# ilovepose/fast-human-pose-estimation.pytorch

Measured on AMD Instinct MI355X. Metric: images/sec FPD train step (4-stack HG student, 8-stack teacher) 256x256, higher is better.
Workload: dtype bf16; 1 GPU; configs[1]: hourglass student S=4 F=128 + teacher S=8 F=256, 256x256, batch 32/GPU, fused FPD step incl. Adam, teacher forward one batch ahead on a 2nd stream; global_batch=32, parallelism=dp1, backend=mfma, launch=one native plan call per phase, kernels launched eagerly on 3 streams, ranks=1, finite=True

## Files before the change

### fast-human-pose-estimation.pytorch_amd/csrc/api.hip

```cpp
#include <cstdarg>
#include <cstdio>
#include <cstdlib>
#include <cstring>
#include <string>
#include <vector>

#include "conv_dispatch.h"

int g_fpd_backend = FPD_BACKEND_MFMA;
static thread_local char g_err[512] = "";

static FILE* g_launch_log_file = nullptr;
static bool launch_log_open() {
    const char* path = getenv("FPD_LAUNCH_LOG");
    if (path == nullptr || path[0] == 0) return false;
    g_launch_log_file = fopen(path, "w");
    if (g_launch_log_file == nullptr) fprintf(stderr, "[fpd_amd] FPD_LAUNCH_LOG: cannot open %s\n", path);
    return g_launch_log_file != nullptr;
}
bool g_fpd_launch_log = launch_log_open();
static thread_local char g_op_tag[256] = "-";
void fpd_log_launch(const char* kernel, const dim3& grid, const dim3& block) {
    if (g_launch_log_file == nullptr) return;
    fprintf(g_launch_log_file, "%s\t%u\t%u\t%s\n", kernel, grid.x * grid.y * grid.z, block.x * block.y * block.z, g_op_tag);
    fflush(g_launch_log_file);
}

int fpd_fail(int code, const char* fmt, ...) {
    va_list ap;
    va_start(ap, fmt);
    vsnprintf(g_err, sizeof(g_err), fmt, ap);
    va_end(ap);
    return code;
}

static int check_launch() {
    hipError_t e = hipGetLastError();
    if (e != hipSuccess) return fpd_fail(-100 - (int)e, "kernel launch failed: %s", hipGetErrorString(e));
    return 0;
}

static int validate_conv_dims(int N, int H, int W, int C, int K, int R, int S, int stride, int pad, int P, int Q) {
    FPD_REQUIRE(N > 0 && H > 0 && W > 0 && C > 0 && K > 0 && R > 0 && S > 0 && stride > 0 && pad >= 0,
                "conv: non-positive dimension");
    FPD_REQUIRE(P == (H + 2 * pad - R) / stride + 1 && Q == (W + 2 * pad - S) / stride + 1,
                "conv: output %dx%d inconsistent with input %dx%d k=%dx%d stride=%d pad=%d", P, Q, H, W, R, S, stride, pad);
    FPD_REQUIRE((int64_t)N * H * W * C < (1ll << 31) && (int64_t)N * P * Q * K < (1ll << 31), "conv: tensor too large for 32-bit indexing");
    return 0;
}

int fpd_bneck_blocks_option(int value);
int fpd_head_blocks_option(int value);

extern "C" {

const char* fpd_last_error(void) { return g_err; }
int fpd_abi_version(void) { return FPD_ABI_VERSION; }
int64_t fpd_stats_words(int32_t channels) { return FPD_STATS_WORDS(channels); }
int fpd_set_backend(int32_t backend) {
    const int prev = g_fpd_backend;
    if (backend == FPD_BACKEND_MFMA || backend == FPD_BACKEND_NAIVE || backend == FPD_BACKEND_MFMA_GENERIC) g_fpd_backend = backend;
    return prev;
}

static int g_wgrad_tile_only = 0;

int fpd_set_option(const char* name, int32_t value) {
    FPD_REQUIRE(name, "set_option: null name");
    if (!strcmp(name, "conv_pp")) return fpd_conv_pp_option(0, value);
    if (!strcmp(name, "conv_pp_blocks")) return fpd_conv_pp_option(1, value);
    if (!strcmp(name, "conv_c1")) return fpd_conv_c1_option(0, value);
    if (!strcmp(name, "conv_c1_blocks")) return fpd_conv_c1_option(1, value);
    if (!strcmp(name, "conv_c1_launches")) return fpd_conv_c1_option(2, value);
    if (!strcmp(name, "conv_skip")) return fpd_conv_c1_option(3, value);
    if (!strcmp(name, "stem_act")) return fpd_stem_s2d_option(0, value);
    if (!strcmp(name, "ew_merge")) return fpd_ew_merge_option(value < 0 ? 0 : value);
    if (!strcmp(name, "ew_merge_blocks")) return fpd_ew_merge_blocks_option(value);
    if (!strcmp(name, "conv_c3")) return fpd_conv_c3_option(0, value);
    if (!strcmp(name, "conv_c3_blocks")) return fpd_conv_c3_option(1, value);
    if (!strcmp(name, "conv_c3_launches")) return fpd_conv_c3_option(2, value);
    if (!strcmp(name, "bneck_blocks")) return fpd_bneck_blocks_option(value);
    if (!strcmp(name, "head_blocks")) return fpd_head_blocks_option(value);
    if (!strcmp(name, "wgrad_tile_only")) { g_wgrad_tile_only = value; return 0; }
    return fpd_fail(-2, "set_option: unknown option '%s'", name);
}

int fpd_abi_sizeof(const char* n) {
#define SZ(T) if (!strcmp(n, #T)) return (int)sizeof(T)
    SZ(fpd_bn_t); SZ(fpd_conv_t); SZ(fpd_wgrad_t); SZ(fpd_stem_t); SZ(fpd_ew_t); SZ(fpd_loss_t); SZ(fpd_adam_t);
    SZ(fpd_wprep_entry_t); SZ(fpd_bnupd_entry_t); SZ(fpd_memset_t); SZ(fpd_table_t); SZ(fpd_wreduce_entry_t); SZ(fpd_bneck_t); SZ(fpd_conv_pair_t); SZ(fpd_bneck_pair_t); SZ(fpd_ew_pair_t); SZ(fpd_pck_t); SZ(fpd_head_t); SZ(fpd_affsum_t); SZ(fpd_layout_t);
    SZ(fpd_conv_f8_t); SZ(fpd_wquant_entry_t); SZ(fpd_flipmerge_t); SZ(fpd_finalpreds_t); SZ(fpd_targets_t); SZ(fpd_warp_src_t); SZ(fpd_warp_t);
    SZ(fpd_loss_ohkm_t); SZ(fpd_sgd_t); SZ(fpd_ew_merge_t);
    SZ(fpd_aug_img_t); SZ(fpd_aug_db_t); SZ(fpd_aug_crop_t); SZ(fpd_augment_t); SZ(fpd_warp_aug_t); SZ(fpd_targets_w_t);
    SZ(fpd_oks_nms_t); SZ(fpd_coco_match_t); SZ(fpd_coco_accum_t);
#undef SZ
    return -1;
}

static int validate_conv(const fpd_conv_t* a) {
    FPD_REQUIRE(a && a->x && a->w && a->y, "conv: null pointer");
    int rc = validate_conv_dims(a->N, a->H, a->W, a->C, a->K, a->R, a->S, a->stride, a->pad, a->P, a->Q);
    if (rc) return rc;
    FPD_REQUIRE(a->dtype == FPD_F32 || a->dtype == FPD_BF16, "conv: bad dtype %d", a->dtype);
    FPD_REQUIRE(a->bn.mode == FPD_BN_NONE || (a->bn.gamma && a->bn.beta), "conv: BN prologue without gamma/beta");
    FPD_REQUIRE(a->bn.mode != FPD_BN_TRAIN || a->bn.stats, "conv: train-mode BN without statistics");
    FPD_REQUIRE(a->bn.mode != FPD_BN_EVAL || (a->bn.running_mean && a->bn.running_var), "conv: eval-mode BN without running stats");
    FPD_REQUIRE(a->epi == FPD_EPI_PLAIN || (a->epi_x && a->epi_stats && a->epi_bn.mode == FPD_BN_TRAIN && a->epi_bn.stats),
                "conv: BNRELU_BWD epilogue needs epi_x, epi_stats and a train-mode epi_bn");
    FPD_REQUIRE(a->x2 == nullptr || (a->w2 != nullptr && a->C2 > 0), "conv: a second source (x2) needs w2 and C2");
    FPD_REQUIRE(a->x2 == nullptr || a->residual == nullptr, "conv: a second source (x2) and a residual exclude each other");
    return 0;
}

constexpr unsigned ON_MFMA = 1u << FPD_BACKEND_MFMA, ON_GENERIC = ON_MFMA | 1u << FPD_BACKEND_MFMA_GENERIC, ON_ANY = ON_GENERIC | 1u << FPD_BACKEND_NAIVE;
struct ConvBackend {
    const char* name;
    unsigned backends;
    int (*route)(const fpd_conv_t& a, const fpd_conv_t* b, ConvAsk ask, ConvRoute& r);
    int (*launch)(const fpd_conv_t& a, const fpd_conv_t* b, hipStream_t st);
};
static const ConvBackend g_conv_backends[] = {
    {"conv_c1", ON_MFMA, fpd_conv_c1_route, fpd_conv_c1_launch},
    {"conv_c3", ON_MFMA, fpd_conv_c3_route, fpd_conv_c3_launch},
    {"conv_pp", ON_MFMA, fpd_conv_pp_route, fpd_conv_pp_launch},
    {"conv_tile", ON_MFMA, fpd_conv_tile_route, fpd_conv_tile_launch},
    {"conv_mfma", ON_GENERIC, nullptr, [](const fpd_conv_t& a, const fpd_conv_t*, hipStream_t st) { return fpd_conv_mfma_launch(a, st); }},
    {"conv_smallc", ON_GENERIC, nullptr, [](const fpd_conv_t& a, const fpd_conv_t*, hipStream_t st) { return fpd_conv_smallc_launch(a, st); }},
    {"conv_naive", ON_ANY, nullptr, [](const fpd_conv_t& a, const fpd_conv_t*, hipStream_t st) { return fpd_conv_naive_launch(a, st); }},
};
static bool eligible(unsigned backends) { return (backends >> g_fpd_backend & 1u) != 0; }

static const ConvBackend* route_conv(const fpd_conv_t& a, const fpd_conv_t* b, ConvAsk ask, ConvRoute& r) {
    r = ConvRoute{false, 0, 0, false};
    for (const ConvBackend& e : g_conv_backends) {
        if (!eligible(e.backends)) continue;
        if (e.route == nullptr ? b == nullptr : e.route(a, b, ask, r) == 0) return &e;
    }
    return nullptr;
}

static int launch_conv(const fpd_conv_t& a, const fpd_conv_t* b, hipStream_t st) {
    ConvRoute r;
    const ConvBackend* e = route_conv(a, b, fpd_conv_ask(a, b), r);
    if (e == nullptr) {
        const int rc = launch_conv(a, nullptr, st);
        return rc ? rc : launch_conv(*b, nullptr, st);
    }
    FPD_REQUIRE(!(a.wg_partial != nullptr && r.slabs_a == 0) && !(b != nullptr && b->wg_partial != nullptr && r.slabs_b == 0),
                "conv: the launch asks for a fused weight gradient (wg_partial), which its route (%s) does not offer; %s() reports 0 for it",
                e->name, b ? "fpd_conv_pair_fused_wgrad_partials" : "fpd_conv_fused_wgrad_partials");
    FPD_REQUIRE(r.folds || (a.fold_x == nullptr && (b == nullptr || b->fold_x == nullptr)),
                "conv: the launch asks for a folded BN-backward apply (fold_x), which its route (%s) does not offer; %s() reports 0 for it",
                e->name, b ? "fpd_conv_pair_fold_supported" : "fpd_conv_fold_supported");
    FPD_REQUIRE(r.skips || (a.x2 == nullptr && (b == nullptr || b->x2 == nullptr)),
                "conv: the launch carries a second 1x1 source (x2), which its route (%s) does not offer; fpd_conv_skip_supported() reports 0 for it", e->name);
    int rc = e->launch(a, b, st);
    for (++e; rc == 1 && e != std::end(g_conv_backends); ++e)
        if (e->route == nullptr && eligible(e->backends)) rc = e->launch(a, b, st);
    return rc;
}

int fpd_conv_forward(const fpd_conv_t* a, fpd_stream_t stream) {
    int rc = validate_conv(a);
    if (rc) return rc;
    rc = launch_conv(*a, nullptr, (hipStream_t)stream);
    return rc ? rc : check_launch();
}

int fpd_conv_fold_supported(const fpd_conv_t* a) {
    ConvRoute r;
    if (!a || validate_conv(a) != 0) return 0;
    route_conv(*a, nullptr, ConvAsk{true, a->wg_partial != nullptr, a->x2 != nullptr}, r);
    return r.folds ? 1 : 0;
}
int fpd_conv_pair_fold_supported(const fpd_conv_pair_t* p) {
    ConvRoute r;
    if (!p || validate_conv(&p->a) != 0 || validate_conv(&p->b) != 0) return 0;
    if (route_conv(p->a, &p->b, ConvAsk{true, fpd_conv_ask(p->a, &p->b).wg, fpd_conv_ask(p->a, &p->b).skip}, r) != nullptr) return r.folds ? 1 : 0;
    return (fpd_conv_fold_supported(&p->a) && fpd_conv_fold_supported(&p->b)) ? 1 : 0;
}

int fpd_conv_skip_supported(const fpd_conv_t* a) {
    ConvRoute r;
    if (!a || validate_conv(a) != 0) return 0;
    route_conv(*a, nullptr, ConvAsk{a->fold_x != nullptr, a->wg_partial != nullptr, true}, r);
    return r.skips ? 1 : 0;
}

int fpd_conv_fused_wgrad_partials(const fpd_conv_t* a) {
    ConvRoute r;
    if (!a || validate_conv(a) != 0) return 0;
    route_conv(*a, nullptr, ConvAsk{a->fold_x != nullptr, true, a->x2 != nullptr}, r);
    return r.slabs_a;
}
int fpd_conv_pair_fused_wgrad_partials(const fpd_conv_pair_t* p, int32_t* n_a, int32_t* n_b) {
    FPD_REQUIRE(p && n_a && n_b, "conv_pair_fused_wgrad_partials: null pointer");
    *n_a = *n_b = 0;
    if (validate_conv(&p->a) != 0 || validate_conv(&p->b) != 0) return 0;
    ConvRoute r;
    route_conv(p->a, &p->b, ConvAsk{fpd_conv_ask(p->a, &p->b).fold, true, fpd_conv_ask(p->a, &p->b).skip}, r);
    *n_a = r.slabs_a; *n_b = r.slabs_b;
    return 0;
}

int fpd_conv_f8_in_domain(const fpd_conv_t* c) { return (c && fpd_conv_f8_domain(*c)) ? 1 : 0; }

int fpd_conv_forward_f8(const fpd_conv_f8_t* a, fpd_stream_t stream) {
    FPD_REQUIRE(a, "conv_f8: null pointer");
    int rc = validate_conv(&a->c);
    if (rc) return rc;
    FPD_REQUIRE(a->w8 && a->w8_scale, "conv_f8: null fp8 weights / scales");
    FPD_REQUIRE(((uintptr_t)a->w8 & 15) == 0, "conv_f8: w8 must be 16-byte aligned");
    rc = 1;
    if (g_fpd_backend == FPD_BACKEND_MFMA) rc = fpd_conv_tile_f8_launch(a->c, a->w8, a->w8_scale, (hipStream_t)stream);
    if (rc == 1) rc = launch_conv(a->c, nullptr, (hipStream_t)stream);
    return rc ? rc : check_launch();
}

int fpd_weight_quant_f8(const fpd_wquant_entry_t* t, int32_t n, fpd_stream_t stream) {
    FPD_REQUIRE(n == 0 || t != nullptr, "weight_quant_f8: null table");
    int rc = fpd_weight_quant_f8_launch(t, n, (hipStream_t)stream);
    return rc ? rc : check_launch();
}

int fpd_conv_forward_pair(const fpd_conv_pair_t* p, fpd_stream_t stream) {
    FPD_REQUIRE(p, "conv_pair: null pointer");
    int rc = validate_conv(&p->a);
    if (rc) return rc;
    rc = validate_conv(&p->b);
    if (rc) return rc;
    FPD_REQUIRE(p->a.x2 == nullptr && p->b.x2 == nullptr, "conv_pair: a pair launch takes no second source (x2)");
    rc = launch_conv(p->a, &p->b, (hipStream_t)stream);
    return rc ? rc : check_launch();
}

static int validate_bneck_bns(const fpd_bneck_t* a) {
    const fpd_bn_t* bns[3] = {&a->bn1, &a->bn2, &a->bn3};
    for (int i = 0; i < 3; ++i)
        FPD_REQUIRE(bns[i]->mode == FPD_BN_EVAL && bns[i]->relu && bns[i]->gamma && bns[i]->beta && bns[i]->running_mean &&
                    bns[i]->running_var, "bottleneck: bn%d must be an eval-mode BN+ReLU with running statistics", i + 1);
    return 0;
}

int fpd_bottleneck_fold(const fpd_bneck_t* a, fpd_stream_t stream) {
    FPD_REQUIRE(a && a->folded, "bottleneck_fold: null pointer");
    int rc = validate_bneck_bns(a);
    if (rc) return rc;
    rc = fpd_bneck_fold_launch(*a, const_cast<float*>(a->folded), (hipStream_t)stream);
    if (rc == 1) return fpd_fail(-3, "bottleneck_fold: C=%d P=%d is outside the fused kernel's domain", a->C, a->P);
    return rc ? rc : check_launch();
}

int fpd_bottleneck_forward_pair(const fpd_bneck_pair_t* p, fpd_stream_t stream) {
    FPD_REQUIRE(p, "bottleneck_pair: null pointer");
    const fpd_bneck_t* ab[2] = {&p->a, &p->b};
    for (const fpd_bneck_t* a : ab) {
        FPD_REQUIRE(a->x && a->y && a->w1 && a->w2 && a->w3 && a->x != a->y, "bottleneck_pair: null pointer or y aliases x");
        FPD_REQUIRE((int64_t)a->N * a->H * a->W * a->C < ((int64_t)1 << 31), "bottleneck_pair: tensor too large for 32-bit indexing");
        int rc = validate_bneck_bns(a);
        if (rc) return rc;
    }
    int rc = fpd_bneck_fused_pair_launch(p->a, p->b, (hipStream_t)stream);
    if (rc == 1) {
        rc = fpd_bottleneck_forward(&p->a, stream);
        return rc ? rc : fpd_bottleneck_forward(&p->b, stream);
    }
    return rc ? rc : check_launch();
}

int fpd_bottleneck_forward(const fpd_bneck_t* a, fpd_stream_t stream) {
    FPD_REQUIRE(a && a->x && a->y && a->w1 && a->w2 && a->w3, "bottleneck: null pointer");
    FPD_REQUIRE(a->x != a->y, "bottleneck: y must not alias x");
    FPD_REQUIRE(a->N > 0 && a->H > 0 && a->W > 0 && a->C > 0 && a->P > 0, "bottleneck: bad dims");
    FPD_REQUIRE((int64_t)a->N * a->H * a->W * a->C < ((int64_t)1 << 31), "bottleneck: tensor too large for 32-bit indexing");
    int rc = validate_bneck_bns(a);
    if (rc) return rc;
    rc = fpd_bneck_fused_launch(*a, (hipStream_t)stream);
    if (rc == 1)
        return fpd_fail(-3, "bottleneck: shape N=%d H=%d W=%d C=%d P=%d dtype=%d is outside the fused kernel's domain",
                        a->N, a->H, a->W, a->C, a->P, a->dtype);
    return rc ? rc : check_launch();
}

struct WgradBackend {
    unsigned backends;
    int (*partials)(const fpd_wgrad_t& a);
    int (*launch)(const fpd_wgrad_t& a, hipStream_t st);
};
static const WgradBackend g_wgrad_backends[] = {
    {ON_MFMA, fpd_wgrad_tile_partials, fpd_wgrad_tile_launch},
    {ON_GENERIC, fpd_wgrad_mfma_partials, fpd_wgrad_mfma_launch},
    {ON_GENERIC, fpd_wgrad_smallc_partials, fpd_wgrad_smallc_launch},
    {ON_ANY, fpd_wgrad_naive_partials, fpd_wgrad_naive_launch},
};

int fpd_conv_wgrad(const fpd_wgrad_t* a, fpd_stream_t stream) {
    FPD_REQUIRE(a && a->x && a->dy && a->dw, "wgrad: null pointer");
    int rc = validate_conv_dims(a->N, a->H, a->W, a->C, a->K, a->R, a->S, a->stride, a->pad, a->P, a->Q);
    if (rc) return rc;
    FPD_REQUIRE(a->dtype == FPD_F32 || a->dtype == FPD_BF16, "wgrad: bad dtype %d", a->dtype);
    FPD_REQUIRE(a->partial == nullptr || a->partial_stride >= (int64_t)a->K * a->R * a->S * a->C + a->K,
                "wgrad: partial_stride %lld smaller than weight + bias", (long long)a->partial_stride);
    rc = 1;
    for (const WgradBackend& e : g_wgrad_backends) {
        FPD_REQUIRE(!(g_wgrad_tile_only && &e != g_wgrad_backends), "wgrad: option wgrad_tile_only is set and the halo-tile kernel declines N=%d H=%d W=%d C=%d K=%d R=%d", a->N, a->H, a->W, a->C, a->K, a->R);
        if (eligible(e.backends)) rc = e.launch(*a, (hipStream_t)stream);
        if (rc != 1) break;
    }
    return rc ? rc : check_launch();
}

int fpd_wgrad_num_partials(const fpd_wgrad_t* a) {
    int n = 0;
    for (const WgradBackend& e : g_wgrad_backends)
        if (a && n == 0 && eligible(e.backends)) n = e.partials(*a);
    return n;
}

struct StemBackend {
    unsigned backends;
    bool (*takes_act)(const fpd_stem_t& a);
    int (*forward)(const fpd_stem_t& a, hipStream_t st);
    int (*wgrad_partials)(const fpd_stem_t& a);
    int (*wgrad)(const fpd_stem_t& a, hipStream_t st);
};
static const StemBackend g_stem_backends[] = {
    {ON_MFMA, fpd_stem_forward_s2d_takes_act, fpd_stem_forward_s2d_launch, fpd_stem_wgrad_s2d_partials, fpd_stem_wgrad_s2d_launch},
    {ON_MFMA, nullptr, fpd_stem_forward_mfma_launch, fpd_stem_wgrad_mfma_partials, fpd_stem_wgrad_mfma_launch},
    {ON_ANY, nullptr, fpd_stem_forward_launch, fpd_stem_wgrad_partials, fpd_stem_wgrad_launch},
};

int fpd_stem_wgrad_num_partials(const fpd_stem_t* a) {
    int n = 0;
    for (const StemBackend& e : g_stem_backends)
        if (a && n == 0 && eligible(e.backends)) n = e.wgrad_partials(*a);
    return n;
}

int fpd_wgrad_reduce(const fpd_wreduce_entry_t* t, int32_t n, int64_t max_elems, fpd_stream_t stream) {
    int rc = fpd_wreduce_launch(t, n, max_elems, (hipStream_t)stream);
    return rc ? rc : check_launch();
}

int fpd_stem_act_supported(const fpd_stem_t* a) {
    if (!a || a->act.mode != FPD_BN_EVAL || !a->act.gamma || !a->act.beta || !a->act.running_mean || !a->act.running_var || a->out_stats != nullptr) return 0;
    for (const StemBackend& e : g_stem_backends)
        if (eligible(e.backends)) return (e.takes_act != nullptr && e.takes_act(*a)) ? 1 : 0;
    return 0;
}

int fpd_stem_forward(const fpd_stem_t* a, fpd_stream_t stream) {
    FPD_REQUIRE(a && a->x && a->w && a->bias && a->y, "stem: null pointer");
    FPD_REQUIRE(a->P == (a->H + 6 - 7) / 2 + 1 && a->Q == (a->W + 6 - 7) / 2 + 1, "stem: bad output size");
    FPD_REQUIRE(a->act.mode == FPD_BN_NONE || fpd_stem_act_supported(a) == 1,
                "stem: the launch asks for BN + ReLU in its epilogue (act), which is not offered for it; fpd_stem_act_supported() reports 0");
    int rc = 1;
    for (const StemBackend& e : g_stem_backends)
        if (rc == 1 && eligible(e.backends)) rc = e.forward(*a, (hipStream_t)stream);
    return rc ? rc : check_launch();
}

int fpd_stem_wgrad(const fpd_stem_t* a, fpd_stream_t stream) {
    FPD_REQUIRE(a && a->x && a->dy && a->dw, "stem wgrad: null pointer");
    FPD_REQUIRE(a->partial == nullptr || a->partial_stride >= (int64_t)a->K * 148, "stem wgrad: partial_stride %lld smaller than weight + bias",
                (long long)a->partial_stride);
    int rc = 1;
    for (const StemBackend& e : g_stem_backends)
        if (rc == 1 && eligible(e.backends)) rc = e.wgrad(*a, (hipStream_t)stream);
    return rc ? rc : check_launch();
}

int fpd_affsum(const fpd_affsum_t* a, fpd_stream_t stream) {
    FPD_REQUIRE(a && a->y, "affsum: null pointer");
    FPD_REQUIRE(a->nterms >= 1 && a->nterms <= FPD_AFFSUM_MAX, "affsum: %d terms (1..%d supported)", a->nterms, FPD_AFFSUM_MAX);
    FPD_REQUIRE(a->dtype == FPD_F32 || a->dtype == FPD_BF16, "affsum: bad dtype %d", a->dtype);
    for (int j = 0; j < a->nterms; ++j) {
        const int up = a->t[j].up;
        FPD_REQUIRE(a->t[j].x, "affsum: term %d has no input", j);
        FPD_REQUIRE((up == 1 || up == 2 || up == 4 || up == 8) && a->H % up == 0 && a->W % up == 0,
                    "affsum: term %d: up-sampling factor %d does not divide %dx%d", j, up, a->H, a->W);
        const fpd_bn_t& bn = a->t[j].bn;
        FPD_REQUIRE(bn.mode == FPD_BN_NONE || (bn.gamma && bn.beta), "affsum: term %d: BN without gamma/beta", j);
        FPD_REQUIRE(bn.mode != FPD_BN_TRAIN || bn.stats, "affsum: term %d: train-mode BN without statistics", j);
        FPD_REQUIRE(bn.mode != FPD_BN_EVAL || (bn.running_mean && bn.running_var), "affsum: term %d: eval-mode BN without running stats", j);
    }
    int rc = fpd_affsum_launch(*a, (hipStream_t)stream);
    return rc ? rc : check_launch();
}

int fpd_elementwise(const fpd_ew_t* a, fpd_stream_t stream) {
    FPD_REQUIRE(a && (a->y || a->op == FPD_EW_BNRELU_BWD_R), "elementwise: null pointer");
    int rc = fpd_elementwise_launch(*a, (hipStream_t)stream);
    return rc ? rc : check_launch();
}

int fpd_ew_merge_supported(const fpd_ew_merge_t* a) { return (a && fpd_ew_merge_why_not(*a) == nullptr) ? 1 : 0; }
int fpd_ew_merge(const fpd_ew_merge_t* a, fpd_stream_t stream) {
    FPD_REQUIRE(a, "ew_merge: null pointer");
    int rc = fpd_ew_merge_launch(*a, (hipStream_t)stream);
    return rc ? rc : check_launch();
}

static int validate_head(const fpd_head_t* a) {
    FPD_REQUIRE(a && a->y0 && a->score && a->w_fc && a->w_score, "head: null pointer");
    FPD_REQUIRE(a->next == nullptr || (a->x && a->w_fc2 && a->w_score2 && a->next != a->x && a->next != a->y0),
                "head: next needs x, w_fc2, w_score2 and must not alias an input");
    FPD_REQUIRE(a->N > 0 && a->H > 0 && a->W > 0 && (int64_t)a->N * a->H * a->W * a->C < ((int64_t)1 << 31), "head: bad dims");
    FPD_REQUIRE(a->bn.mode == FPD_BN_EVAL && a->bn.relu && a->bn.gamma && a->bn.beta && a->bn.running_mean && a->bn.running_var,
                "head: bn must be an eval-mode BN+ReLU with running statistics");
    return 0;
}
int fpd_head_forward(const fpd_head_t* a, fpd_stream_t stream) {
    int rc = validate_head(a);
    if (rc) return rc;
    rc = fpd_head_fused_launch(*a, (hipStream_t)stream);
    if (rc == 1) return fpd_fail(-3, "head: C=%d J=%d dtype=%d is outside the fused kernel's domain", a->C, a->J, a->dtype);
    return rc ? rc : check_launch();
}
int fpd_head_fold(const fpd_head_t* a, fpd_stream_t stream) {
    FPD_REQUIRE(a && a->folded, "head_fold: null pointer");
    FPD_REQUIRE(a->bn.mode == FPD_BN_EVAL && a->bn.gamma && a->bn.beta && a->bn.running_mean && a->bn.running_var, "head_fold: bn");
    int rc = fpd_head_fold_launch(*a, const_cast<float*>(a->folded), (hipStream_t)stream);
    if (rc == 1) return fpd_fail(-3, "head_fold: C=%d is outside the fused kernel's domain", a->C);
    return rc ? rc : check_launch();
}

int fpd_pck(const fpd_pck_t* a, fpd_stream_t stream) {
    FPD_REQUIRE(a && a->out && a->target && a->counts && a->log && a->cursor, "pck: null pointer");
    FPD_REQUIRE(a->B > 0 && a->J > 0 && a->H > 0 && a->W > 0 && a->log_slots > 0, "pck: bad dims");
    FPD_REQUIRE(a->dtype == FPD_F32 || a->dtype == FPD_BF16, "pck: bad dtype %d", a->dtype);
    int rc = fpd_pck_launch(*a, (hipStream_t)stream);
    return rc ? rc : check_launch();
}

int fpd_flip_w(const float* x, float* y, int64_t rows, int32_t W, fpd_stream_t stream) {
// ... 156 lines not shown

int fpd_sgd(const fpd_sgd_t* a, fpd_stream_t stream) {
    FPD_REQUIRE(a && a->param && a->grad, "sgd: null pointer");
    FPD_REQUIRE(a->n >= 0, "sgd: n = %lld is negative", (long long)a->n);
    FPD_REQUIRE(a->momentum >= 0.f, "sgd: invalid momentum value %g", (double)a->momentum);
    FPD_REQUIRE(a->weight_decay >= 0.f, "sgd: invalid weight_decay value %g", (double)a->weight_decay);
    FPD_REQUIRE(a->momentum == 0.f || a->buf, "sgd: momentum %g needs a momentum buffer (buf is null)", (double)a->momentum);
    FPD_REQUIRE(!a->nesterov || a->momentum != 0.f, "sgd: nesterov momentum requires a momentum (and zero dampening)");
    int rc = fpd_sgd_launch(*a, (hipStream_t)stream);
    return rc ? rc : check_launch();
}

int fpd_weight_prep(const fpd_wprep_entry_t* t, int32_t n, int64_t max_elems, int32_t dtype, fpd_stream_t stream) {
    int rc = fpd_weight_prep_launch(t, n, max_elems, dtype, (hipStream_t)stream);
    return rc ? rc : check_launch();
}
int fpd_bn_update_running(const fpd_bnupd_entry_t* t, int32_t n, fpd_stream_t stream) {
    int rc = fpd_bn_update_running_launch(t, n, (hipStream_t)stream);
    return rc ? rc : check_launch();
}
int fpd_cast(const void* src, void* dst, int64_t n, int32_t sd, int32_t dd, fpd_stream_t stream) {
    int rc = fpd_cast_launch(src, dst, n, sd, dd, (hipStream_t)stream);
    return rc ? rc : check_launch();
}
int fpd_nchw_to_nhwc(const float* src, void* dst, int32_t N, int32_t C, int32_t H, int32_t W, int32_t dtype, fpd_stream_t stream) {
    int rc = fpd_nchw_to_nhwc_launch(src, dst, N, C, H, W, dtype, (hipStream_t)stream);
    return rc ? rc : check_launch();
}
int fpd_nhwc_to_nchw(const void* src, float* dst, int32_t N, int32_t C, int32_t H, int32_t W, int32_t dtype, fpd_stream_t stream) {
    int rc = fpd_nhwc_to_nchw_launch(src, dst, N, C, H, W, dtype, (hipStream_t)stream);
    return rc ? rc : check_launch();
}

struct fpd_op {
    int32_t type;
    union {
        fpd_affsum_t affsum; fpd_layout_t layout; fpd_conv_f8_t conv8; fpd_conv_t conv; fpd_conv_pair_t pair; fpd_bneck_t bneck; fpd_bneck_pair_t bpair; fpd_ew_pair_t epair; fpd_pck_t pck; fpd_head_t head; fpd_wgrad_t wgrad; fpd_stem_t stem; fpd_ew_t ew; fpd_loss_t loss; fpd_loss_ohkm_t lossk; fpd_adam_t adam; fpd_sgd_t sgd; fpd_ew_merge_t ewm;
        fpd_memset_t mset; fpd_table_t table;
    } u;
};
struct fpd_sched {
    int32_t lane = 0;
    bool record = false;
    hipEvent_t done = nullptr;
    std::vector<int32_t> waits;
};
struct fpd_plan {
    std::vector<fpd_op> ops;
    std::vector<fpd_sched> sched;
    std::vector<hipGraphExec_t> graphs;
    std::vector<hipGraph_t> graph_defs;
    hipStream_t lanes[FPD_MAX_LANES] = {};
    hipEvent_t lane_done[FPD_MAX_LANES] = {};
    hipEvent_t fork = nullptr;
};

fpd_plan* fpd_plan_create(void) { return new fpd_plan(); }
void fpd_plan_destroy(fpd_plan* p) {
    if (!p) return;
    for (auto g : p->graphs) (void)hipGraphExecDestroy(g);
    for (auto g : p->graph_defs) (void)hipGraphDestroy(g);
    for (auto& s : p->sched) if (s.done) (void)hipEventDestroy(s.done);
    for (int l = 0; l < FPD_MAX_LANES; ++l) {
        if (p->lanes[l]) (void)hipStreamDestroy(p->lanes[l]);
        if (p->lane_done[l]) (void)hipEventDestroy(p->lane_done[l]);
    }
    if (p->fork) (void)hipEventDestroy(p->fork);
    delete p;
}
int fpd_plan_size(const fpd_plan* p) { return p ? (int)p->ops.size() : -1; }

int fpd_plan_add(fpd_plan* p, int32_t op, const void* args, int64_t bytes) {
    FPD_REQUIRE(p && args, "plan_add: null");
    fpd_op o;
    memset(&o, 0, sizeof(o));
    o.type = op;
    size_t want = 0;
    switch (op) {
        case FPD_OP_CONV: want = sizeof(fpd_conv_t); break;
        case FPD_OP_CONV_F8: want = sizeof(fpd_conv_f8_t); break;
        case FPD_OP_WGRAD: want = sizeof(fpd_wgrad_t); break;
        case FPD_OP_CONV_PAIR: want = sizeof(fpd_conv_pair_t); break;
        case FPD_OP_BNECK_PAIR: want = sizeof(fpd_bneck_pair_t); break;
        case FPD_OP_EW_PAIR: want = sizeof(fpd_ew_pair_t); break;
        case FPD_OP_PCK: want = sizeof(fpd_pck_t); break;
        case FPD_OP_HEAD: case FPD_OP_HEAD_FOLD: want = sizeof(fpd_head_t); break;
        case FPD_OP_BNECK: case FPD_OP_BNECK_FOLD: want = sizeof(fpd_bneck_t); break;
        case FPD_OP_STEM_FWD: case FPD_OP_STEM_WGRAD: want = sizeof(fpd_stem_t); break;
        case FPD_OP_EW: want = sizeof(fpd_ew_t); break;
        case FPD_OP_EW_MERGE: want = sizeof(fpd_ew_merge_t); break;
        case FPD_OP_LOSS: want = sizeof(fpd_loss_t); break;
        case FPD_OP_LOSS_OHKM: want = sizeof(fpd_loss_ohkm_t); break;
        case FPD_OP_ADAM: want = sizeof(fpd_adam_t); break;
        case FPD_OP_SGD: want = sizeof(fpd_sgd_t); break;
        case FPD_OP_MEMSET: case FPD_OP_NOP: want = sizeof(fpd_memset_t); break;
        case FPD_OP_AFFSUM: want = sizeof(fpd_affsum_t); break;
        case FPD_OP_NCHW2NHWC: want = sizeof(fpd_layout_t); break;
        case FPD_OP_WPREP: case FPD_OP_BNUPD: case FPD_OP_WREDUCE: case FPD_OP_WQUANT: want = sizeof(fpd_table_t); break;
        default: return fpd_fail(-2, "plan_add: unknown op %d", op);
    }
    FPD_REQUIRE((size_t)bytes == want, "plan_add: op %d expects %zu bytes of args, got %lld", op, want, (long long)bytes);
    memcpy(&o.u, args, want);
    p->ops.push_back(o);
    p->sched.emplace_back();
    return (int)p->ops.size() - 1;
}

int fpd_plan_set_schedule(fpd_plan* p, int32_t op, int32_t lane, const int32_t* wait_ops, int32_t n_waits) {
    FPD_REQUIRE(p && op >= 0 && op < (int)p->ops.size(), "plan_set_schedule: bad op index %d", op);
    FPD_REQUIRE(lane >= 0 && lane < FPD_MAX_LANES, "plan_set_schedule: lane %d outside [0,%d)", lane, FPD_MAX_LANES);
    FPD_REQUIRE(n_waits >= 0 && (n_waits == 0 || wait_ops != nullptr), "plan_set_schedule: bad wait list");
    for (int i = 0; i < n_waits; ++i)
        FPD_REQUIRE(wait_ops[i] >= 0 && wait_ops[i] < op, "plan_set_schedule: op %d may only wait for earlier ops (got %d)", op, wait_ops[i]);
    fpd_sched& s = p->sched[op];
    s.lane = lane;
    s.waits.assign(wait_ops, wait_ops + n_waits);
    for (int i = 0; i < n_waits; ++i) p->sched[wait_ops[i]].record = true;
    return 0;
}

int fpd_plan_mark_event(fpd_plan* p, int32_t op) {
    FPD_REQUIRE(p && op >= 0 && op < (int)p->ops.size(), "plan_mark_event: bad op index %d", op);
    p->sched[op].record = true;
    return 0;
}

int fpd_plan_wait_op(fpd_plan* p, int32_t op, fpd_stream_t stream) {
    FPD_REQUIRE(p && op >= 0 && op < (int)p->ops.size(), "plan_wait_op: bad op index %d", op);
    FPD_REQUIRE(p->sched[op].record && p->sched[op].done, "plan_wait_op: op %d has no recorded event (mark it, then run its range)", op);
    FPD_CHECK_HIP(hipStreamWaitEvent((hipStream_t)stream, p->sched[op].done, 0));
    return 0;
}

static void conv_tag(char* p, size_t n, const char* what, const fpd_conv_t& c) {
    snprintf(p, n, "%s N=%d H=%d W=%d C=%d K=%d R=%d s=%d %s%s%s%s%s", what, c.N, c.H, c.W, c.C, c.K, c.R, c.stride,
             c.epi == FPD_EPI_BNRELU_BWD ? "dgrad" : "fwd", c.bn.mode == FPD_BN_EVAL ? " evalbn" : "", c.wg_partial ? " +wgrad" : "", c.fold_x ? " +fold" : "",
             c.x2 ? " +skip" : "");
}
static void set_op_tag(int idx, const fpd_op& o) {
    char t[200] = "";
    static const char* ew_names[] = {"bnrelu_fwd", "bnrelu_bwd_r", "bn_bwd_apply", "maxpool_fwd", "maxpool_bwd", "upadd_fwd", "sumpool", "add", "relu_mask", "dilate2"};
    auto ewn = [&](int op) { return (op >= 0 && op < 10) ? ew_names[op] : "ew"; };
    switch (o.type) {
        case FPD_OP_CONV: conv_tag(t, sizeof(t), "conv", o.u.conv); break;
        case FPD_OP_CONV_F8: conv_tag(t, sizeof(t), "conv_f8", o.u.conv8.c); break;
        case FPD_OP_CONV_PAIR: {
            char a[90], b[90];
            conv_tag(a, sizeof(a), "conv2", o.u.pair.a);
            snprintf(b, sizeof(b), " | H=%d W=%d", o.u.pair.b.H, o.u.pair.b.W);
            snprintf(t, sizeof(t), "%s%s", a, b);
            break;
        }
        case FPD_OP_WGRAD: snprintf(t, sizeof(t), "wgrad N=%d H=%d W=%d C=%d K=%d R=%d s=%d", o.u.wgrad.N, o.u.wgrad.H, o.u.wgrad.W, o.u.wgrad.C, o.u.wgrad.K, o.u.wgrad.R, o.u.wgrad.stride); break;
        case FPD_OP_BNECK: snprintf(t, sizeof(t), "bneck N=%d H=%d W=%d C=%d P=%d", o.u.bneck.N, o.u.bneck.H, o.u.bneck.W, o.u.bneck.C, o.u.bneck.P); break;
        case FPD_OP_BNECK_PAIR: snprintf(t, sizeof(t), "bneck2 N=%d H=%d W=%d C=%d P=%d | H=%d W=%d", o.u.bpair.a.N, o.u.bpair.a.H, o.u.bpair.a.W, o.u.bpair.a.C, o.u.bpair.a.P, o.u.bpair.b.H, o.u.bpair.b.W); break;
        case FPD_OP_HEAD: snprintf(t, sizeof(t), "head N=%d H=%d W=%d C=%d J=%d", o.u.head.N, o.u.head.H, o.u.head.W, o.u.head.C, o.u.head.J); break;
        case FPD_OP_EW: snprintf(t, sizeof(t), "ew %s N=%d H=%d W=%d C=%d", ewn(o.u.ew.op), o.u.ew.N, o.u.ew.H, o.u.ew.W, o.u.ew.C); break;
        case FPD_OP_EW_PAIR: snprintf(t, sizeof(t), "ew2 %s N=%d H=%d W=%d C=%d | H=%d W=%d", ewn(o.u.epair.a.op), o.u.epair.a.N, o.u.epair.a.H, o.u.epair.a.W, o.u.epair.a.C, o.u.epair.b.H, o.u.epair.b.W); break;
        case FPD_OP_EW_MERGE: {
            const fpd_ew_merge_t& m = o.u.ewm;
            const bool pb = m.kind == FPD_EWM_MAXPOOL_BWD;
            snprintf(t, sizeof(t), "ewm %s N=%d H=%d W=%d C=%d", pb ? (m.has_full ? "apply2+maxpool_bwd" : "apply+maxpool_bwd") : "apply+sumpool", m.pool.N, m.pool.H, m.pool.W, m.pool.C);
            break;
        }
        case FPD_OP_STEM_FWD: case FPD_OP_STEM_WGRAD: snprintf(t, sizeof(t), "%s N=%d H=%d W=%d K=%d%s", o.type == FPD_OP_STEM_FWD ? "stem_fwd" : "stem_wgrad", o.u.stem.N, o.u.stem.H, o.u.stem.W, o.u.stem.K,
                                                              (o.type == FPD_OP_STEM_FWD && o.u.stem.act.mode != FPD_BN_NONE) ? " +act" : ""); break;
        case FPD_OP_AFFSUM: snprintf(t, sizeof(t), "affsum N=%d H=%d W=%d C=%d terms=%d", o.u.affsum.N, o.u.affsum.H, o.u.affsum.W, o.u.affsum.C, o.u.affsum.nterms); break;
        case FPD_OP_LOSS: snprintf(t, sizeof(t), "loss B=%d J=%d H=%d W=%d S=%d", o.u.loss.B, o.u.loss.J, o.u.loss.H, o.u.loss.W, o.u.loss.S); break;
        case FPD_OP_LOSS_OHKM: snprintf(t, sizeof(t), "loss_ohkm B=%d J=%d H=%d W=%d S=%d k=%d,%d", o.u.lossk.base.B, o.u.lossk.base.J, o.u.lossk.base.H, o.u.lossk.base.W, o.u.lossk.base.S, o.u.lossk.topk_pose, o.u.lossk.topk_kd); break;
        case FPD_OP_ADAM: snprintf(t, sizeof(t), "adam n=%lld", (long long)o.u.adam.n); break;
        case FPD_OP_SGD: snprintf(t, sizeof(t), "sgd n=%lld momentum=%g wd=%g%s", (long long)o.u.sgd.n, (double)o.u.sgd.momentum, (double)o.u.sgd.weight_decay, o.u.sgd.nesterov ? " nesterov" : ""); break;
        case FPD_OP_WREDUCE: snprintf(t, sizeof(t), "wreduce entries=%d", o.u.table.n); break;
        case FPD_OP_WPREP: snprintf(t, sizeof(t), "wprep entries=%d", o.u.table.n); break;
        case FPD_OP_BNUPD: snprintf(t, sizeof(t), "bnupd entries=%d", o.u.table.n); break;
        default: snprintf(t, sizeof(t), "op%d", o.type); break;
    }
    snprintf(g_op_tag, sizeof(g_op_tag), "%d\t%s", idx, t);
}

static int run_op(const fpd_op& o, fpd_stream_t s) {
    switch (o.type) {
        case FPD_OP_CONV: return fpd_conv_forward(&o.u.conv, s);
        case FPD_OP_CONV_F8: return fpd_conv_forward_f8(&o.u.conv8, s);
        case FPD_OP_WQUANT: return fpd_weight_quant_f8((const fpd_wquant_entry_t*)o.u.table.table, o.u.table.n, s);
        case FPD_OP_WGRAD: return fpd_conv_wgrad(&o.u.wgrad, s);
        case FPD_OP_CONV_PAIR: return fpd_conv_forward_pair(&o.u.pair, s);
        case FPD_OP_BNECK_PAIR: return fpd_bottleneck_forward_pair(&o.u.bpair, s);
        case FPD_OP_EW_PAIR: return fpd_elementwise_pair(&o.u.epair, s);
        case FPD_OP_PCK: return fpd_pck(&o.u.pck, s);
        case FPD_OP_HEAD: return fpd_head_forward(&o.u.head, s);
        case FPD_OP_HEAD_FOLD: return fpd_head_fold(&o.u.head, s);
        case FPD_OP_BNECK: return fpd_bottleneck_forward(&o.u.bneck, s);
        case FPD_OP_BNECK_FOLD: return fpd_bottleneck_fold(&o.u.bneck, s);
        case FPD_OP_STEM_FWD: return fpd_stem_forward(&o.u.stem, s);
        case FPD_OP_STEM_WGRAD: return fpd_stem_wgrad(&o.u.stem, s);
        case FPD_OP_EW: return fpd_elementwise(&o.u.ew, s);
        case FPD_OP_EW_MERGE: return fpd_ew_merge(&o.u.ewm, s);
        case FPD_OP_LOSS: return fpd_loss(&o.u.loss, s);
        case FPD_OP_LOSS_OHKM: return fpd_loss_ohkm(&o.u.lossk, s);
        case FPD_OP_ADAM: return fpd_adam(&o.u.adam, s);
        case FPD_OP_SGD: return fpd_sgd(&o.u.sgd, s);
        case FPD_OP_MEMSET: {
            FPD_CHECK_HIP(hipMemsetAsync(o.u.mset.ptr, 0, (size_t)o.u.mset.bytes, (hipStream_t)s));
            return 0;
        }
        case FPD_OP_NOP: return 0;
        case FPD_OP_AFFSUM: return fpd_affsum(&o.u.affsum, s);
        case FPD_OP_NCHW2NHWC:
            return fpd_nchw_to_nhwc(o.u.layout.src, o.u.layout.dst, o.u.layout.N, o.u.layout.C, o.u.layout.H, o.u.layout.W, o.u.layout.dtype, s);
        case FPD_OP_WPREP:
            return fpd_weight_prep((const fpd_wprep_entry_t*)o.u.table.table, o.u.table.n, o.u.table.max_elems, o.u.table.dtype, s);
        case FPD_OP_BNUPD: return fpd_bn_update_running((const fpd_bnupd_entry_t*)o.u.table.table, o.u.table.n, s);
        case FPD_OP_WREDUCE: return fpd_wgrad_reduce((const fpd_wreduce_entry_t*)o.u.table.table, o.u.table.n, o.u.table.max_elems, s);
    }
    return fpd_fail(-2, "run_op: unknown op %d", o.type);
}

static int lane_priority() { return 0; }

static int side_streams() { return FPD_MAX_LANES; }

int fpd_plan_run(fpd_plan* p, int32_t begin, int32_t end, fpd_stream_t stream) {
    FPD_REQUIRE(p && begin >= 0 && end <= (int)p->ops.size() && begin <= end, "plan_run: bad range [%d,%d)", begin, end);
    hipStream_t main_s = (hipStream_t)stream;
    bool multi = false;
    for (int i = begin; i < end; ++i) multi |= p->sched[i].lane != 0;
    bool used[FPD_MAX_LANES] = {};
    if (multi) {
        if (!p->fork) FPD_CHECK_HIP(hipEventCreateWithFlags(&p->fork, hipEventDisableTiming));
        FPD_CHECK_HIP(hipEventRecord(p->fork, main_s));
    }
    int rc = 0;
    for (int i = begin; i < end && rc == 0; ++i) {
        fpd_sched& sc = p->sched[i];
        hipStream_t st = main_s;
        if (sc.lane != 0) {
            const int l = 1 + (sc.lane - 1) % side_streams();
            if (!p->lanes[l]) {
                FPD_CHECK_HIP(hipStreamCreateWithPriority(&p->lanes[l], hipStreamNonBlocking, lane_priority()));
                FPD_CHECK_HIP(hipEventCreateWithFlags(&p->lane_done[l], hipEventDisableTiming));
            }
            st = p->lanes[l];
            if (!used[l]) {
                FPD_CHECK_HIP(hipStreamWaitEvent(st, p->fork, 0));
                used[l] = true;
            }
        }
        for (int32_t w : sc.waits)
            if (w >= begin && w < end) FPD_CHECK_HIP(hipStreamWaitEvent(st, p->sched[w].done, 0));
        if (g_fpd_launch_log) set_op_tag(i, p->ops[i]);
        rc = run_op(p->ops[i], (fpd_stream_t)st);
        if (rc) {
            char tmp[400];
            snprintf(tmp, sizeof(tmp), "%s", g_err);
            rc = fpd_fail(rc, "plan op %d (type %d): %s", i, p->ops[i].type, tmp);
            break;
        }
        if (sc.record) {
            if (!sc.done) FPD_CHECK_HIP(hipEventCreateWithFlags(&sc.done, hipEventDisableTiming));
            FPD_CHECK_HIP(hipEventRecord(sc.done, st));
        }
    }
    for (int l = 1; l < FPD_MAX_LANES; ++l)
        if (used[l]) {
            FPD_CHECK_HIP(hipEventRecord(p->lane_done[l], p->lanes[l]));
            FPD_CHECK_HIP(hipStreamWaitEvent(main_s, p->lane_done[l], 0));
        }
    return rc;
}

int fpd_plan_run_op(fpd_plan* p, int32_t op, fpd_stream_t stream) {
    FPD_REQUIRE(p && op >= 0 && op < (int)p->ops.size(), "plan_run_op: bad op index %d", op);
    if (g_fpd_launch_log) set_op_tag(op, p->ops[op]);
    return run_op(p->ops[op], stream);
}

int fpd_plan_capture(fpd_plan* p, int32_t begin, int32_t end, fpd_stream_t stream) {
    FPD_REQUIRE(p, "plan_capture: null");
    FPD_REQUIRE(!g_fpd_launch_log, "plan_capture: FPD_LAUNCH_LOG is set -- the launch log keys a kernel trace 1:1 and cannot follow hipGraph replays; unset one of them");
    hipStream_t st = (hipStream_t)stream;
    FPD_CHECK_HIP(hipStreamBeginCapture(st, hipStreamCaptureModeThreadLocal));
    int rc = fpd_plan_run(p, begin, end, stream);
    hipGraph_t g = nullptr;
    hipError_t e = hipStreamEndCapture(st, &g);
    if (rc) { if (g) (void)hipGraphDestroy(g); return rc; }
    if (e != hipSuccess) return fpd_fail(-100 - (int)e, "hipStreamEndCapture: %s", hipGetErrorString(e));
    hipGraphExec_t ge = nullptr;
    FPD_CHECK_HIP(hipGraphInstantiate(&ge, g, nullptr, nullptr, 0));
    p->graph_defs.push_back(g);
    p->graphs.push_back(ge);
    return (int)p->graphs.size() - 1;
}

int fpd_plan_replay(fpd_plan* p, int32_t gid, fpd_stream_t stream) {
    FPD_REQUIRE(p && gid >= 0 && gid < (int)p->graphs.size(), "plan_replay: bad graph id %d", gid);
    FPD_CHECK_HIP(hipGraphLaunch(p->graphs[gid], (hipStream_t)stream));
    return 0;
}

void* fpd_event_create(void) {
    hipEvent_t e = nullptr;
    if (hipEventCreate(&e) != hipSuccess) return nullptr;
    return (void*)e;
}
int fpd_event_record(void* ev, fpd_stream_t stream) {
    FPD_CHECK_HIP(hipEventRecord((hipEvent_t)ev, (hipStream_t)stream));
    return 0;
// ... 11 lines not shown
```

### fast-human-pose-estimation.pytorch_amd/csrc/bneck_fused.hip

```cpp
#include <algorithm>
#include <atomic>
#include <cstdlib>
#include <type_traits>

#include "common.h"

namespace {

typedef unsigned int u32x4 __attribute__((ext_vector_type(4)));

#ifdef FPD_BNECK_TIMING
#define STAMP(i) do { if (tid == 0 && bid_in == 0) stamps[i] = clock64(); } while (0)
#else
#define STAMP(i) do { } while (0)
#endif

template <int P>
__device__ __forceinline__ void bneck_fold_tables(const fpd_bneck_t& a, float* out, int tid, int nthreads) {
    constexpr int C = 2 * P;
    for (int c = tid; c < C; c += nthreads) {
        float sc, sh;
        bn_coef_eval(a.bn1, c, sc, sh);
        out[c] = sc;
        out[C + c] = sh;
        out[2 * C + 4 * P + c] = a.b3 ? a.b3[c] : 0.f;
    }
    for (int c = tid; c < 2 * P; c += nthreads) {
        const bool second = c >= P;
        const int cc = second ? c - P : c;
        float sc, sh;
        bn_coef_eval(second ? a.bn3 : a.bn2, cc, sc, sh);
        const float* bias = second ? a.b2 : a.b1;
        out[2 * C + (second ? 2 * P : 0) + cc] = sc;
        out[2 * C + (second ? 2 * P : 0) + P + cc] = fmaf(sc, bias ? bias[cc] : 0.f, sh);
    }
}

template <int P>
__global__ void bneck_fold_kernel(const fpd_bneck_t a, float* out) { bneck_fold_tables<P>(a, out, threadIdx.x, blockDim.x); }

template <int P, bool DMA>
__device__ __forceinline__ void bneck_eval_body(const fpd_bneck_t& a, const int logW, const int swz, const int bid_in,
                                                const int nblk, const int ntiles) {
    constexpr int C = 2 * P;
    constexpr int LDW = DMA ? P : P + 8;
    constexpr int LDX = 64 + 8;
    constexpr int LD2 = P + 8;
    constexpr int TNH = P / 64;
    constexpr int CW = 32 * TNH;
    constexpr int NSTEP = 9 + 2;
    constexpr int VPR2 = P / 8;
    constexpr int WV = P * VPR2 / 512;
    constexpr int W1V = P * 8 / 512;
    constexpr int NCH = C / 64;
    constexpr int ASTG = (128 + P) * LDX;
    extern __shared__ __attribute__((aligned(16))) unsigned char smem[];

    const int tid = threadIdx.x, lane = tid & 63, wave = tid >> 6;
#ifdef FPD_BNECK_TIMING
    long long stamps[8];
    long long astamp[10];
    int acnt = 0;
#define ASTAMP() do { if (tid == 0 && bid_in == 0 && acnt < 10) astamp[acnt++] = clock64(); } while (0)
#else
#define ASTAMP() do { } while (0)
#endif
    STAMP(0);
    const int q = wave & 3, hC = wave >> 2;
    const int koff = 8 * (lane >> 5);
    const int H = a.H, W = a.W;
    const int M = a.N * H * W, GR = a.N * H;
    const int nrows = 128 >> logW, hrows = nrows + 2, WP = W + 2;
    const int rrows = 2 * nrows;
    const bool whole = (128 % (H * W)) == 0;
    const int irows = whole ? hrows : rrows;
    const int zero_px = irows * WP;
    int m0 = 0, g0 = 0;
    int vrow0 = 0;

    float* s_sc1 = reinterpret_cast<float*>(smem);
    float* s_sh1 = s_sc1 + C;
    float* s_sc2 = s_sh1 + C;
    float* s_sh2 = s_sc2 + P;
    float* s_sc3 = s_sh2 + P;
    float* s_sh3 = s_sc3 + P;
    float* s_b3 = s_sh3 + P;
    bf16_t* sA2 = reinterpret_cast<bf16_t*>(s_b3 + C);
    bf16_t* sR2 = sA2 + (zero_px + 3) * LD2;
    const bf16_t* __restrict__ x = reinterpret_cast<const bf16_t*>(a.x);
    const bf16_t* __restrict__ w1 = reinterpret_cast<const bf16_t*>(a.w1);
    const bf16_t* __restrict__ w2 = reinterpret_cast<const bf16_t*>(a.w2);
    const bf16_t* __restrict__ w3 = reinterpret_cast<const bf16_t*>(a.w3);

    int hp0 = whole ? W : 0;
    int npass = whole ? 1 : ((hrows * W + 127) >> 7);
    const int xpx = tid >> 3, xcv = (tid & 7) * 8;
    int xo[2];
    bool xok[2];
    auto pass_addr = [&](int p) __attribute__((always_inline)) {
#pragma unroll
        for (int i = 0; i < 2; ++i) {
            const int hp = hp0 + 128 * p + xpx + 64 * i;
            const int hr = hp >> logW, j = hp & (W - 1);
            const int g = g0 - 1 + hr;
            xok[i] = hr < hrows && (unsigned)g < (unsigned)GR;
            xo[i] = xok[i] ? (g * W + j) * C + xcv : 0;
        }
    };
    int w1o[W1V], w1l[W1V];
#pragma unroll
    for (int i = 0; i < W1V; ++i) {
        const int v = tid + i * 512;
        w1o[i] = (v >> 3) * C + (v & 7) * 8;
        w1l[i] = 128 * LDX + (v >> 3) * LDX + (v & 7) * 8;
    }
    const int xl = xpx * LDX + xcv;

    u32x4 rx[NCH][2], rw[NCH][W1V];
    auto a_load = [&](auto kcc) __attribute__((always_inline)) {
        constexpr int kc = decltype(kcc)::value;
        static_for<2>([&](auto ic) {
            constexpr int i = decltype(ic)::value;
            const u32x4 z = {0u, 0u, 0u, 0u};
            rx[kc][i] = z;
            if (xok[i]) rx[kc][i] = *reinterpret_cast<const u32x4*>(x + (xo[i] + kc * 64));
        });
        static_for<W1V>([&](auto ic) {
            constexpr int i = decltype(ic)::value;
            rw[kc][i] = *reinterpret_cast<const u32x4*>(w1 + (w1o[i] + kc * 64));
        });
    };
    constexpr int NSL = 2 + W1V;
    auto a_store_slice = [&](auto kcc, auto slc) __attribute__((always_inline)) {
        constexpr int kc = decltype(kcc)::value, sl = decltype(slc)::value;
        bf16_t* dst = sR2 + (kc & 1) * ASTG;
        if constexpr (sl < 2) {
            f32x4 sc[2], sh[2];
            sc[0] = *reinterpret_cast<const f32x4*>(s_sc1 + kc * 64 + xcv);
            sc[1] = *reinterpret_cast<const f32x4*>(s_sc1 + kc * 64 + xcv + 4);
            sh[0] = *reinterpret_cast<const f32x4*>(s_sh1 + kc * 64 + xcv);
            sh[1] = *reinterpret_cast<const f32x4*>(s_sh1 + kc * 64 + xcv + 4);
            float f[8];
            const u32x4 r = rx[kc][sl];
            DT<bf16_t>::unpack(make_uint4(r[0], r[1], r[2], r[3]), f);
#pragma unroll
            for (int e = 0; e < 8; ++e) f[e] = fmaxf(fmaf(f[e], sc[e >> 2][e & 3], sh[e >> 2][e & 3]), 0.f);
            *reinterpret_cast<uint4*>(dst + xl + 64 * sl * LDX) = DT<bf16_t>::pack(f);
        } else if constexpr (sl < NSL) {
            *reinterpret_cast<u32x4*>(dst + w1l[sl - 2]) = rw[kc][sl - 2];
        }
    };
    auto a_store = [&](auto kcc) __attribute__((always_inline)) {
        static_for<NSL>([&](auto slc) { a_store_slice(kcc, slc); });
    };
    int t2o[WV], t3o[WV], tlo[WV];
#pragma unroll
    for (int i = 0; i < WV; ++i) {
        const int v = tid + i * 512;
        const int row = v / VPR2, col = (v - row * VPR2) * 8;
        t2o[i] = row * 9 * P + col;
        t3o[i] = row * P + col;
        tlo[i] = row * LD2 + col;
    }
    u32x4 rb[DMA ? 1 : 2][DMA ? 1 : WV];
    auto t_load = [&](auto sc_) __attribute__((always_inline)) {
        constexpr int s = decltype(sc_)::value;
        if constexpr (!DMA) {
            static_for<WV>([&](auto ic) {
                constexpr int i = decltype(ic)::value;
                const bf16_t* src = s < 9 ? w2 + (t2o[i] + s * P) : w3 + (t3o[i] + (s - 9) * P * P);
                rb[s & 1][i] = *reinterpret_cast<const u32x4*>(src);
            });
        }
    };
    auto t_store = [&](auto sc_) __attribute__((always_inline)) {
        constexpr int s = decltype(sc_)::value;
        if constexpr (!DMA) {
            bf16_t* dst = sR2 + (s & 1) * P * LDW;
            static_for<WV>([&](auto ic) {
                constexpr int i = decltype(ic)::value;
                *reinterpret_cast<u32x4*>(dst + tlo[i]) = rb[s & 1][i];
            });
        }
    };
    constexpr int CPR = P / 8;
    constexpr int RPI = 64 / CPR;
    constexpr int DPW = P / RPI / 8;
    unsigned dma2[DMA ? DPW : 1], dma3[DMA ? DPW : 1];
    if constexpr (DMA) {
#pragma unroll
        for (int j = 0; j < DPW; ++j) {
            const int row = wave * DPW * RPI + j * RPI + lane / CPR;
            const int sw = (P == 128) ? (row & 15) : ((row >> 1) & 7);
            const int c8 = ((lane % CPR) ^ sw) * 8;
            dma2[j] = (unsigned)(row * 9 * P + c8) * 2u;
            dma3[j] = (unsigned)(row * P + c8) * 2u;
        }
    }
    auto t_dma = [&](auto sc_) __attribute__((always_inline)) {
        constexpr int s = decltype(sc_)::value;
        if constexpr (DMA) {
            unsigned char* ring = reinterpret_cast<unsigned char*>(sR2) + (s & 1) * P * P * 2 + wave * DPW * 1024;
            const char* gbase = s < 9 ? reinterpret_cast<const char*>(w2) + s * P * 2
                                      : reinterpret_cast<const char*>(w3) + (s - 9) * P * P * 2;
            static_for<DPW>([&](auto jc) {
                constexpr int j = decltype(jc)::value;
                unsigned off = s < 9 ? dma2[j] : dma3[j];
                asm volatile("" : "+v"(off));
                __builtin_amdgcn_global_load_lds((const __attribute__((address_space(1))) void*)(gbase + off),
                                                 (__attribute__((address_space(3))) void*)(ring + j * 1024), 16, 0, 0);
            });
        }
    };

    if (a.folded != nullptr) {
        for (int v = tid; v < (3 * C + 4 * P) / 4; v += 512)
            reinterpret_cast<f32x4*>(s_sc1)[v] = reinterpret_cast<const f32x4*>(a.folded)[v];
    } else {
        bneck_fold_tables<P>(a, s_sc1, tid, 512);
    }

    const int t_beg = fpd_cut(bid_in, ntiles, nblk), t_end = fpd_cut(bid_in + 1, ntiles, nblk);
    (void)swz;
    for (int tile = t_beg; tile < t_end; ++tile) {
    {
        m0 = tile * 128;
        g0 = m0 >> logW;
        vrow0 = (tile * nrows) % rrows;
        if (!whole) {
            const bool incr = tile > t_beg && (g0 % H) != 0;
            hp0 = incr ? 2 * W : 0;
            npass = incr ? 1 : ((hrows * W + 127) >> 7);
        }
    }
    pass_addr(0);
    static_for<NCH>([&](auto kcc) { a_load(kcc); });
    if (npass > 1) pass_addr(1);
    __syncthreads();
    {
        constexpr int VR = LD2 / 8;
        const uint4 z = make_uint4(0, 0, 0, 0);
        for (int v = tid; v < (2 * irows + 3) * VR; v += 512) {
            const int pz = v / VR, cv = (v - pz * VR) * 8;
            const int px = pz < 2 * irows ? ((pz >> 1) * WP + ((pz & 1) ? WP - 1 : 0)) : zero_px + (pz - 2 * irows);
            *reinterpret_cast<uint4*>(sA2 + px * LD2 + cv) = z;
        }
    }
    STAMP(1);

    auto refill = [&](auto kcc, int pp) __attribute__((always_inline)) {
        constexpr int kc = decltype(kcc)::value;
        if (pp + 1 < npass) a_load(kcc);
        else if constexpr (kc < 2) t_load(kcc);
    };
#ifdef FPD_BNECK_TIMING
    acnt = 0;
#endif
    ASTAMP();
    a_store(std::integral_constant<int, 0>{});
    refill(std::integral_constant<int, 0>{}, 0);
    __syncthreads();
    ASTAMP();
    for (int p = 0; p < npass; ++p) {
        f32x16 acc[TNH];
#pragma unroll
        for (int tn = 0; tn < TNH; ++tn)
#pragma unroll
            for (int i = 0; i < 16; ++i) acc[tn][i] = 0.f;
        static_for<NCH>([&](auto kcc) {
            constexpr int kc = decltype(kcc)::value;
            auto stage_slice = [&](auto slc) __attribute__((always_inline)) {
                constexpr int sl = decltype(slc)::value;
                if constexpr (kc + 1 < NCH) {
                    a_store_slice(std::integral_constant<int, (kc + 1) % NCH>{}, slc);
                    if constexpr (sl == NSL - 1) refill(std::integral_constant<int, (kc + 1) % NCH>{}, p);
                } else {
                    if (p + 1 < npass) {
                        a_store_slice(std::integral_constant<int, 0>{}, slc);
                        if constexpr (sl == NSL - 1) {
                            if (p + 2 < npass) pass_addr(p + 2);
                            refill(std::integral_constant<int, 0>{}, p + 1);
                        }
                    }
                }
            };
            const bf16_t* xrow = sR2 + (kc & 1) * ASTG + (q * 32 + (lane & 31)) * LDX + koff;
            const bf16_t* wrow = sR2 + (kc & 1) * ASTG + 128 * LDX + (hC * CW + (lane & 31)) * LDX + koff;
            static_for<4>([&](auto kkc) {
                constexpr int kk = decltype(kkc)::value;
                const bf16x8 px = *reinterpret_cast<const bf16x8*>(xrow + kk * 16);
#pragma unroll
                for (int tn = 0; tn < TNH; ++tn) {
                    const bf16x8 wf = *reinterpret_cast<const bf16x8*>(wrow + tn * 32 * LDX + kk * 16);
                    acc[tn] = __builtin_amdgcn_mfma_f32_32x32x16_bf16(wf, px, acc[tn], 0, 0, 0);
                }
                stage_slice(kkc);
            });
            __syncthreads();
            ASTAMP();
        });
        if (p + 1 == npass) {
            t_dma(std::integral_constant<int, 0>{});
            t_dma(std::integral_constant<int, 1>{});
        }
        const int hp = hp0 + 128 * p + q * 32 + (lane & 31);
        const int hr = hp >> logW, j = hp & (W - 1);
        if (hr < hrows) {
            const int rr = whole ? hr : ((vrow0 + hr) & (rrows - 1));
            bf16_t* dst = sA2 + (rr * WP + j + 1) * LD2;
#pragma unroll
            for (int tn = 0; tn < TNH; ++tn)
#pragma unroll
                for (int gi = 0; gi < 4; ++gi) {
                    const int c = hC * CW + tn * 32 + 8 * gi + 4 * (lane >> 5);
                    const f32x4 sc = *reinterpret_cast<const f32x4*>(s_sc2 + c);
                    const f32x4 sh = *reinterpret_cast<const f32x4*>(s_sh2 + c);
                    float v[4];
#pragma unroll
                    for (int e = 0; e < 4; ++e) v[e] = fmaxf(fmaf(acc[tn][4 * gi + e], sc[e], sh[e]), 0.f);
                    *reinterpret_cast<uint2*>(dst + c) = make_uint2(f2bf_pk(v[0], v[1]), f2bf_pk(v[2], v[3]));
                }
        }
    }

    const int ml = q * 32 + (lane & 31);
    const int a3px = whole ? 0 : vrow0 * WP;
    int ab[3];
    {
        const int ti = ml >> logW, tj = ml & (W - 1);
        const int g = g0 + ti;
        const int pr = g % H;
        const bool live = g < GR;
        const int r0 = whole ? ti : ((vrow0 + ti) & (rrows - 1)), r1 = whole ? ti + 1 : ((vrow0 + ti + 1) & (rrows - 1)),
                  r2 = whole ? ti + 2 : ((vrow0 + ti + 2) & (rrows - 1));
        ab[0] = (live && pr - 1 >= 0) ? (r0 * WP + tj) * LD2 : zero_px * LD2;
        ab[1] = live ? (r1 * WP + tj) * LD2 : zero_px * LD2;
        ab[2] = (live && pr + 1 < H) ? (r2 * WP + tj) * LD2 : zero_px * LD2;
    }
    STAMP(2);
    t_store(std::integral_constant<int, 0>{});
    t_load(std::integral_constant<int, 2>{});
    __syncthreads();
    STAMP(3);

    f32x16 accB[TNH], accC[2][TNH];
#pragma unroll
    for (int tn = 0; tn < TNH; ++tn)
#pragma unroll
        for (int i = 0; i < 16; ++i) accB[tn][i] = 0.f;

    const int wsw = (P == 128) ? (lane & 15) : ((lane >> 1) & 7);
    auto mma = [&](const bf16_t* arow, int buf, f32x16* acc) __attribute__((always_inline)) {
        const bf16_t* wbase = sR2 + buf * P * LDW + (hC * CW + (lane & 31)) * LDW;
#pragma unroll
        for (int kk = 0; kk < P / 16; ++kk) {
            const bf16x8 px = *reinterpret_cast<const bf16x8*>(arow + kk * 16);
            const int wo = DMA ? (((2 * kk + (lane >> 5)) ^ wsw) * 8) : (kk * 16 + koff);
#pragma unroll
            for (int tn = 0; tn < TNH; ++tn) {
                const bf16x8 wf = *reinterpret_cast<const bf16x8*>(wbase + tn * 32 * LDW + wo);
                acc[tn] = __builtin_amdgcn_mfma_f32_32x32x16_bf16(wf, px, acc[tn], 0, 0, 0);
            }
        }
    };

    constexpr int VW = CW / 8;
    constexpr int NIT = 32 * VW / 64;
    u32x4 rres[2][NIT];
    auto res_load = [&](auto stc) __attribute__((always_inline)) {
        constexpr int st = decltype(stc)::value;
        static_for<NIT>([&](auto itc) {
            constexpr int it = decltype(itc)::value;
            const int idx = lane + 64 * it;
            const int px = idx / VW, cv = (idx - px * VW) * 8;
            const int m = m0 + q * 32 + px;
            const u32x4 z = {0u, 0u, 0u, 0u};
            rres[st][it] = z;
            if (m < M) rres[st][it] = *reinterpret_cast<const u32x4*>(x + ((size_t)m * C + st * P + hC * CW + cv));
        });
    };

    static_for<NSTEP>([&](auto sc_) {
        constexpr int s = decltype(sc_)::value;
        if constexpr (DMA && s >= 1 && s + 1 < NSTEP) t_dma(std::integral_constant<int, (s + 1 < NSTEP ? s + 1 : 0)>{});
        if constexpr (s < 9) {
            mma(sA2 + ab[s / 3] + (s % 3) * LD2 + koff, s & 1, accB);
        } else {
#pragma unroll
            for (int tn = 0; tn < TNH; ++tn)
#pragma unroll
                for (int i = 0; i < 16; ++i) accC[s - 9][tn][i] = 0.f;
            mma(sA2 + (a3px + ml) * LD2 + koff, s & 1, accC[s - 9]);
        }
        if constexpr (s + 1 < NSTEP) {
            t_store(std::integral_constant<int, s + 1>{});
            if constexpr (s + 3 < NSTEP) t_load(std::integral_constant<int, (s + 3 < NSTEP ? s + 3 : 0)>{});
            if constexpr (s == 8) res_load(std::integral_constant<int, 0>{});
            if constexpr (s == 9) res_load(std::integral_constant<int, 1>{});
            __syncthreads();
        }
        if constexpr (s == 8) {
            STAMP(4);
            bf16_t* dst = sA2 + (a3px + ml) * LD2;
#pragma unroll
            for (int tn = 0; tn < TNH; ++tn)
#pragma unroll
                for (int gi = 0; gi < 4; ++gi) {
                    const int c = hC * CW + tn * 32 + 8 * gi + 4 * (lane >> 5);
                    const f32x4 sc = *reinterpret_cast<const f32x4*>(s_sc3 + c);
                    const f32x4 sh = *reinterpret_cast<const f32x4*>(s_sh3 + c);
                    float v[4];
#pragma unroll
                    for (int e = 0; e < 4; ++e) v[e] = fmaxf(fmaf(accB[tn][4 * gi + e], sc[e], sh[e]), 0.f);
                    *reinterpret_cast<uint2*>(dst + c) = make_uint2(f2bf_pk(v[0], v[1]), f2bf_pk(v[2], v[3]));
                }
            __syncthreads();
        }
    });

    STAMP(5);
    constexpr int LDS_ = CW + 4;
    float* stage = reinterpret_cast<float*>(sR2) + wave * 32 * LDS_;
    bf16_t* __restrict__ y = reinterpret_cast<bf16_t*>(a.y);
    static_for<2>([&](auto stc) {
        constexpr int st = decltype(stc)::value;
        __syncthreads();
#pragma unroll
        for (int tn = 0; tn < TNH; ++tn)
#pragma unroll
            for (int gi = 0; gi < 4; ++gi) {
                f32x4 v;
#pragma unroll
                for (int e = 0; e < 4; ++e) v[e] = accC[st][tn][4 * gi + e];
                *reinterpret_cast<f32x4*>(stage + (lane & 31) * LDS_ + tn * 32 + 8 * gi + 4 * (lane >> 5)) = v;
            }
        __syncthreads();
        static_for<NIT>([&](auto itc) {
            constexpr int it = decltype(itc)::value;
            const int idx = lane + 64 * it;
            const int px = idx / VW, cv = (idx - px * VW) * 8;
            const int m = m0 + q * 32 + px;
            if (m < M) {
                const int c = st * P + hC * CW + cv;
                const f32x4 v0 = *reinterpret_cast<const f32x4*>(stage + px * LDS_ + cv);
                const f32x4 v1 = *reinterpret_cast<const f32x4*>(stage + px * LDS_ + cv + 4);
                const f32x4 b0 = *reinterpret_cast<const f32x4*>(s_b3 + c);
                const f32x4 b1 = *reinterpret_cast<const f32x4*>(s_b3 + c + 4);
                float res[8], o[8];
                const u32x4 r = rres[st][it];
                DT<bf16_t>::unpack(make_uint4(r[0], r[1], r[2], r[3]), res);
#pragma unroll
                for (int e = 0; e < 4; ++e) {
                    o[e] = v0[e] + b0[e] + res[e];
                    o[4 + e] = v1[e] + b1[e] + res[4 + e];
                }
                *reinterpret_cast<uint4*>(y + ((size_t)m * C + c)) = DT<bf16_t>::pack(o);
            }
        });
    });
    }
#ifdef FPD_BNECK_TIMING
    STAMP(6);
    if (tid == 0 && bid_in == 0)
        printf("bneck W=%d: setup %lld | phaseA %lld | tile0 %lld | B(9 taps) %lld | a3+C %lld | epilogue %lld | total %lld cycles\n",
               W, stamps[1] - stamps[0], stamps[2] - stamps[1], stamps[3] - stamps[2], stamps[4] - stamps[3],
               stamps[5] - stamps[4], stamps[6] - stamps[5], stamps[6] - stamps[0]);
    if (tid == 0 && bid_in == 0 && acnt == 10)
        printf("  phase A steps: first-stage %lld | pass0 %lld %lld %lld %lld | pass1 %lld %lld %lld %lld | a2 write %lld\n",
               astamp[1] - astamp[0], astamp[2] - astamp[1], astamp[3] - astamp[2], astamp[4] - astamp[3], astamp[5] - astamp[4],
               astamp[6] - astamp[5], astamp[7] - astamp[6], astamp[8] - astamp[7], astamp[9] - astamp[8], stamps[2] - astamp[9]);
#endif
}

template <int P, bool DMA>
__global__ __launch_bounds__(512, 1) void bneck_eval_kernel(const fpd_bneck_t a, const int logW, const int ntiles) {
    bneck_eval_body<P, DMA>(a, logW, (ntiles & 7) == 0, blockIdx.x, gridDim.x, ntiles);
}

template <int P, bool DMA>
__global__ __launch_bounds__(512, 1) void bneck_eval_pair_kernel(const fpd_bneck_t a, const fpd_bneck_t b, const int logWa,
                                                                 const int logWb, const int nblk_a, const int ntiles_a,
                                                                 const int ntiles_b) {
    if ((int)blockIdx.x < nblk_a) bneck_eval_body<P, DMA>(a, logWa, (ntiles_a & 7) == 0, blockIdx.x, nblk_a, ntiles_a);
    else bneck_eval_body<P, DMA>(b, logWb, (ntiles_b & 7) == 0, (int)blockIdx.x - nblk_a, (int)gridDim.x - nblk_a, ntiles_b);
}


static std::atomic<int> g_bneck_cap{0};
static int bneck_block_cap() {
    int cap = g_bneck_cap.load(std::memory_order_relaxed);
    if (!cap) {
        const char* e = getenv("FPD_BNECK_BLOCKS");
        cap = e ? atoi(e) : 128;
        if (cap < 8) cap = 8;
        int unset = 0;
        if (!g_bneck_cap.compare_exchange_strong(unset, cap, std::memory_order_relaxed)) cap = unset;
    }
    return cap;
}
static int bneck_blocks(int tiles, int cap) {
    if (tiles <= cap) return tiles;
    const int rounds = cdiv(tiles, cap);
    return cdiv(tiles, rounds);
}

template <int P>
size_t bneck_lds_bytes(int H, int W) {
    constexpr int C = 2 * P, LD2 = P + 8, LDX = 72, CW = 32 * (P / 64);
    int logW = 0;
    while ((1 << logW) < W) ++logW;
    const int nrows = 128 >> logW, WP = W + 2;
    const bool whole = (128 % (H * W)) == 0;
    const int irows = whole ? nrows + 2 : 2 * nrows;
    const size_t r2 = std::max({(size_t)2 * P * LD2 * 2, (size_t)2 * (128 + P) * LDX * 2, (size_t)8 * 32 * (CW + 4) * 4});
    return (size_t)(3 * C + 4 * P) * sizeof(float) + (size_t)(irows * WP + 3) * LD2 * 2 + r2;
}

template <int P, bool DMA>
int launch_bneck_pair(const fpd_bneck_t& a, const fpd_bneck_t& b, hipStream_t st) {
    const size_t lds = std::max(bneck_lds_bytes<P>(a.H, a.W), bneck_lds_bytes<P>(b.H, b.W));
    static LdsAttr configured;
    if (int rc_ = configured.ensure(reinterpret_cast<const void*>(&bneck_eval_pair_kernel<P, DMA>), lds)) return rc_;
    int la = 0, lb = 0;
    while ((1 << la) < a.W) ++la;
    while ((1 << lb) < b.W) ++lb;
    const int ta = cdiv(a.N * a.H * a.W, 128), tb = cdiv(b.N * b.H * b.W, 128);
    int na = ta, nb = tb;
    const int cap = bneck_block_cap();
    if (ta + tb > cap) {
        const int capb = std::max(1, (int)((int64_t)cap * tb / (ta + tb)));
        nb = bneck_blocks(tb, capb);
        na = bneck_blocks(ta, std::max(1, cap - nb));
    }
    FPD_LAUNCH((bneck_eval_pair_kernel<P, DMA>), dim3(na + nb), dim3(512), lds, st, a, b, la, lb, na, ta, tb);
    return 0;
}

template <int P, bool DMA>
int launch_bneck(const fpd_bneck_t& a, int logW, hipStream_t st) {
    const size_t lds = bneck_lds_bytes<P>(a.H, a.W);
    static LdsAttr configured;
    if (int rc_ = configured.ensure(reinterpret_cast<const void*>(&bneck_eval_kernel<P, DMA>), lds)) return rc_;
    const int ntiles = cdiv(a.N * a.H * a.W, 128);
    FPD_LAUNCH((bneck_eval_kernel<P, DMA>), dim3(bneck_blocks(ntiles, bneck_block_cap())), dim3(512), lds, st, a, logW, ntiles);
    return 0;
}

}

int fpd_bneck_blocks_option(int value) {
    bneck_block_cap();
    return g_bneck_cap.exchange(value < 1 ? 1 : value, std::memory_order_relaxed);
}

static bool bneck_in_domain(const fpd_bneck_t& a) {
    if (a.dtype != FPD_BF16 || a.C != 2 * a.P || (a.P != 64 && a.P != 128)) return false;
    if (a.W < 4 || a.W > 64 || (a.W & (a.W - 1)) != 0) return false;
    const int hw = a.H * a.W;
    return hw % 128 == 0 || 128 % hw == 0;
}

int fpd_bneck_fused_launch(const fpd_bneck_t& a, hipStream_t st) {
    if (!bneck_in_domain(a)) return 1;
    int logW = 0;
    while ((1 << logW) < a.W) ++logW;
    return a.P == 128 ? launch_bneck<128, true>(a, logW, st) : launch_bneck<64, true>(a, logW, st);
}

int fpd_bneck_fused_pair_launch(const fpd_bneck_t& a, const fpd_bneck_t& b, hipStream_t st) {
    if (!bneck_in_domain(a) || !bneck_in_domain(b) || a.P != b.P) return 1;
    return a.P == 128 ? launch_bneck_pair<128, true>(a, b, st) : launch_bneck_pair<64, true>(a, b, st);
}

int fpd_bneck_fold_launch(const fpd_bneck_t& a, float* out, hipStream_t st) {
    if (a.C != 2 * a.P || (a.P != 64 && a.P != 128)) return 1;
    if (a.P == 128) FPD_LAUNCH((bneck_fold_kernel<128>), dim3(1), dim3(256), 0, st, a, out);
    else FPD_LAUNCH((bneck_fold_kernel<64>), dim3(1), dim3(256), 0, st, a, out);
    return 0;
}
```

### fast-human-pose-estimation.pytorch_amd/csrc/conv_dispatch.h

```cpp
#pragma once
#include <algorithm>
#include <climits>
#include <cstdlib>

#include "common.h"

struct EnvOpt {
    const char* env; int def, lo = INT_MIN, v = -1;
    int get() { if (v < 0) { const char* e = getenv(env); v = e ? atoi(e) : def; } return v < lo ? lo : v; }
    int set(int value) { const int prev = get(); v = value; return prev; }
};

inline bool fpd_split_blocks(int ua, int ub, bool pair, int cap, int& na, int& nb) {
    int total = std::max(1, std::min(cap, ua + ub));
    total = cdiv(ua + ub, cdiv(ua + ub, total));
    nb = 0;
    if (pair) {
        if (total < 2) return false;
        nb = std::max(1, std::min(total - 1, (int)((long long)total * ub / (ua + ub))));
    }
    na = total - nb;
    return true;
}

struct ConvAsk { bool fold, wg, skip; };
struct ConvRoute { bool folds; int slabs_a, slabs_b; bool skips; };
inline ConvAsk fpd_conv_ask(const fpd_conv_t& a, const fpd_conv_t* b) {
    return ConvAsk{a.fold_x != nullptr || (b != nullptr && b->fold_x != nullptr), a.wg_partial != nullptr || (b != nullptr && b->wg_partial != nullptr),
                   a.x2 != nullptr || (b != nullptr && b->x2 != nullptr)};
}
inline int fpd_conv_check_slabs(const fpd_conv_t& c, int slabs, const char* unit) {
    if (c.wg_partial == nullptr) return 0;
    FPD_REQUIRE(c.wg_stride >= (int64_t)c.C * c.K + c.C, "conv: wg_stride %lld smaller than weight + bias", (long long)c.wg_stride);
    FPD_REQUIRE(c.wg_count == slabs, "conv: the launch writes %d weight-gradient slabs but the caller sized its workspace for %d "
                "(fpd_conv_fused_wgrad_partials: has a %s option changed since?)", slabs, c.wg_count, unit);
    return 0;
}
int fpd_conv_c1_route(const fpd_conv_t& a, const fpd_conv_t* b, ConvAsk ask, ConvRoute& r);
int fpd_conv_c1_launch(const fpd_conv_t& a, const fpd_conv_t* b, hipStream_t st);
int fpd_conv_c3_route(const fpd_conv_t& a, const fpd_conv_t* b, ConvAsk ask, ConvRoute& r);
int fpd_conv_c3_launch(const fpd_conv_t& a, const fpd_conv_t* b, hipStream_t st);
int fpd_conv_pp_route(const fpd_conv_t& a, const fpd_conv_t* b, ConvAsk ask, ConvRoute& r);
int fpd_conv_pp_launch(const fpd_conv_t& a, const fpd_conv_t* b, hipStream_t st);
int fpd_conv_tile_route(const fpd_conv_t& a, const fpd_conv_t* b, ConvAsk ask, ConvRoute& r);
int fpd_conv_tile_launch(const fpd_conv_t& a, const fpd_conv_t* b, hipStream_t st);
int fpd_conv_c1_option(int which, int value);
int fpd_conv_c3_option(int which, int value);
int fpd_conv_pp_option(int which, int value);
int fpd_conv_mfma_launch(const fpd_conv_t& a, hipStream_t st);
int fpd_conv_smallc_launch(const fpd_conv_t& a, hipStream_t st);
int fpd_conv_naive_launch(const fpd_conv_t& a, hipStream_t st);
bool fpd_conv_f8_domain(const fpd_conv_t& a);
int fpd_conv_tile_f8_launch(const fpd_conv_t& a, const void* w8, const float* wscale, hipStream_t st);
int fpd_weight_quant_f8_launch(const fpd_wquant_entry_t* table, int n, hipStream_t st);

int fpd_wgrad_tile_partials(const fpd_wgrad_t& a);
int fpd_wgrad_tile_launch(const fpd_wgrad_t& a, hipStream_t st);
int fpd_wgrad_mfma_partials(const fpd_wgrad_t& a);
int fpd_wgrad_mfma_launch(const fpd_wgrad_t& a, hipStream_t st);
int fpd_wgrad_smallc_partials(const fpd_wgrad_t& a);
int fpd_wgrad_smallc_launch(const fpd_wgrad_t& a, hipStream_t st);
int fpd_wgrad_naive_partials(const fpd_wgrad_t& a);
int fpd_wgrad_naive_launch(const fpd_wgrad_t& a, hipStream_t st);
int fpd_wreduce_launch(const fpd_wreduce_entry_t* table, int n, int64_t max_elems, hipStream_t st);

int fpd_stem_forward_s2d_launch(const fpd_stem_t& a, hipStream_t st);
bool fpd_stem_forward_s2d_takes_act(const fpd_stem_t& a);
int fpd_stem_s2d_option(int which, int value);
int fpd_stem_wgrad_s2d_partials(const fpd_stem_t& a);
int fpd_stem_wgrad_s2d_launch(const fpd_stem_t& a, hipStream_t st);
int fpd_stem_forward_mfma_launch(const fpd_stem_t& a, hipStream_t st);
int fpd_stem_wgrad_mfma_partials(const fpd_stem_t& a);
int fpd_stem_wgrad_mfma_launch(const fpd_stem_t& a, hipStream_t st);
int fpd_stem_forward_launch(const fpd_stem_t& a, hipStream_t st);
int fpd_stem_wgrad_partials(const fpd_stem_t& a);
int fpd_stem_wgrad_launch(const fpd_stem_t& a, hipStream_t st);

int fpd_bneck_fused_launch(const fpd_bneck_t& a, hipStream_t st);
int fpd_bneck_fused_pair_launch(const fpd_bneck_t& a, const fpd_bneck_t& b, hipStream_t st);
int fpd_bneck_fold_launch(const fpd_bneck_t& a, float* out, hipStream_t st);
int fpd_head_fused_launch(const fpd_head_t& a, hipStream_t st);
int fpd_head_fold_launch(const fpd_head_t& a, float* out, hipStream_t st);
int fpd_pck_launch(const fpd_pck_t& a, hipStream_t st);
int fpd_flip_w_launch(const float* x, float* y, int64_t rows, int W, hipStream_t st);
int fpd_flip_merge_launch(const fpd_flipmerge_t& p, hipStream_t st);
int fpd_final_preds_launch(const fpd_finalpreds_t& p, hipStream_t st);
int fpd_render_targets_launch(const fpd_targets_t& a, hipStream_t st);
int fpd_warp_affine_launch(const fpd_warp_t& a, hipStream_t st);
int fpd_render_targets_w_launch(const fpd_targets_w_t& a, hipStream_t st);
int fpd_warp_affine_aug_launch(const fpd_warp_aug_t& a, hipStream_t st);
int fpd_augment_params_launch(const fpd_augment_t& a, hipStream_t st);
int fpd_oks_nms_launch(const fpd_oks_nms_t& a, hipStream_t st);
int fpd_coco_match_launch(const fpd_coco_match_t& a, hipStream_t st);
int fpd_coco_accumulate_launch(const fpd_coco_accum_t& a, hipStream_t st);
int fpd_elementwise_launch(const fpd_ew_t& a, hipStream_t st);
int fpd_elementwise_pair_launch(const fpd_ew_t& a, const fpd_ew_t& b, hipStream_t st);
int fpd_affsum_launch(const fpd_affsum_t& a, hipStream_t st);
const char* fpd_ew_merge_why_not(const fpd_ew_merge_t& m);
int fpd_ew_merge_launch(const fpd_ew_merge_t& m, hipStream_t st);
int fpd_ew_merge_option(int value);
int fpd_ew_merge_blocks_option(int value);
int fpd_loss_launch(const fpd_loss_t& a, hipStream_t st);
int fpd_loss_ohkm_launch(const fpd_loss_ohkm_t& a, hipStream_t st);
int64_t fpd_loss_ohkm_scratch_size(const fpd_loss_t& a);
int fpd_adam_launch(const fpd_adam_t& a, hipStream_t st);
int fpd_sgd_launch(const fpd_sgd_t& a, hipStream_t st);
int fpd_weight_prep_launch(const fpd_wprep_entry_t* table, int n, int64_t max_elems, int dtype, hipStream_t st);
int fpd_bn_update_running_launch(const fpd_bnupd_entry_t* table, int n, hipStream_t st);
int fpd_cast_launch(const void* src, void* dst, int64_t n, int sd, int dd, hipStream_t st);
int fpd_nchw_to_nhwc_launch(const float* src, void* dst, int N, int C, int H, int W, int dtype, hipStream_t st);
int fpd_nhwc_to_nchw_launch(const void* src, float* dst, int N, int C, int H, int W, int dtype, hipStream_t st);
```

### fast-human-pose-estimation.pytorch_amd/executor.py

```python
import ctypes as C
import os

import torch

from . import graph as G
from . import runtime as R
from .schedule import PhaseSchedule

_EW = {'bnrelu_fwd': R.EW_BNRELU_FWD, 'bnrelu_bwd_r': R.EW_BNRELU_BWD_R, 'bn_bwd_apply': R.EW_BN_BWD_APPLY,
       'maxpool_fwd': R.EW_MAXPOOL_FWD, 'maxpool_bwd': R.EW_MAXPOOL_BWD, 'upadd_fwd': R.EW_UPADD_FWD,
       'sumpool': R.EW_SUMPOOL, 'add': R.EW_ADD, 'relu_mask': R.EW_RELU_MASK, 'dilate2': R.EW_DILATE2}
_ARENA_DTYPE = {'param': torch.float32, 'grad': torch.float32, 'rstat': torch.float32, 'nbt': torch.int64,
                'stats': torch.int64, 'losses': torch.float64, 'image': torch.float32, 'target': torch.float32,
                'weight': torch.float32, 'adam_m': torch.float32, 'adam_v': torch.float32, 'fold': torch.float32,
                'w8': torch.uint8, 'w8s': torch.float32, 'ohkm_scratch': torch.float64, 'ohkm_masks': torch.int32}


def act_torch_dtype(dtype):
    return torch.bfloat16 if dtype == R.BF16 else torch.float32


_STAT_HI, _STAT_LO = float(2 ** 20), float(2 ** 60)


# ... 154 lines not shown
                    for o in members_of(top):
                        if id(o) in own or not any(_abuf(t) is y for t in o.acts_in()):
                            continue
                        if j < i:
                            early = True
                        m.fold_other_readers = True
            if early:
                continue
            if op.kind == 'conv2':
                ps = R.ConvPairT()
                ps.a, ps.b = self.conv(op.a, plain=True)[1], self.conv(op.b, plain=True)[1]
                ok = l.fpd_conv_pair_fold_supported(C.byref(ps)) == 1
            else:
                ok = l.fpd_conv_fold_supported(C.byref(self.conv(op, plain=True)[1])) == 1
            if ok:
                for m in cands:
                    m.fold_active = True
                    m.fold_apply.folded = True

    def plan_ew_merge(self, ops):
        if os.environ.get('FPD_EW_MERGE', '1') == '0':
            return
        l = R.lib()
        members_of = lambda top: [m for m in ((top.a, top.b) if top.kind in ('conv2', 'ew2', 'bneck2') else (top,)) if m is not None]
        iv = lambda b: (b.arena, b.off, b.off + b.numel)
        hit = lambda p, q: p[0] == q[0] and p[1] < q[2] and q[1] < p[2]
        is_apply = lambda m: (m is not None and m.kind == 'ew' and m.op == 'bn_bwd_apply' and not getattr(m, 'folded', False)
                              and not getattr(m, 'ewm_absorbed', False))
        lane0 = [i for i, op in enumerate(ops) if op is not None and (op.lane or 0) == 0]
        for k in range(1, len(lane0)):
            i, j = lane0[k - 1], lane0[k]
            prev, op = ops[i], ops[j]
            if op.kind != 'ew' or op.op not in ('maxpool_bwd', 'sumpool') or getattr(op, 'ewm_kind', None) is not None:
                continue
            full = half = None
            if op.op == 'maxpool_bwd':
                cands = [m for m in members_of(prev) if is_apply(m)] if prev.kind in ('ew', 'ew2') else []
                if len(cands) != len(members_of(prev)):
                    continue
                half = next((m for m in cands if _abuf(m.y) is _abuf(op.dy)), None)
                full = next((m for m in cands if m is not half), None)
                n, h, w, c = op.dims
                if half is None or tuple(half.dims) != (n, h // 2, w // 2, c):
                    continue
                if full is not None and not (_abuf(op.add) is _abuf(full.y) and _abuf(op.x) is _abuf(full.x) and tuple(full.dims) == tuple(op.dims)):
                    continue
                hidden = [m.y for m in (full, half) if m is not None]
                if any(o is not op and any(_abuf(t) is _abuf(y) for t in o.acts_in() for y in hidden)
                       for top in ops if top is not None for o in members_of(top)):
                    continue
            else:
                if prev.kind != 'ew' or not is_apply(prev) or _abuf(prev.y) is not _abuf(op.x) or tuple(prev.dims) != tuple(op.dims):
                    continue
                full = prev
                if any(any(_abuf(t) is _abuf(full.y) for t in o.acts_in()) for top in ops[i + 1:j] if top is not None for o in members_of(top)):
                    continue
            group = [m for m in (full, half) if m is not None]
            if not self._ew_merge_intervals_ok(op, full, half, ops[i + 1:j], iv, hit):
                continue
            op.ewm_kind, op.ewm_full, op.ewm_half = op.op, full, half
            if l.fpd_ew_merge_supported(C.byref(self.ew_merge(op)[1])) == 1:
                for m in group:
                    m.ewm_absorbed = True
            else:
                op.ewm_kind = op.ewm_full = op.ewm_half = None

    @staticmethod
    def _ew_merge_intervals_ok(op, full, half, between, iv, hit):
        group = [m for m in (full, half) if m is not None]
        pool_bwd = op.op == 'maxpool_bwd'
        moved_rd, moved_wr = [], []
        for m in group:
            r, w = m.accesses()
            moved_rd += r + [m.bstats]
            moved_wr += [b for b in w if b is not m.bstats and not (pool_bwd and b is _abuf(m.y))]
        ins = moved_rd + [_abuf(t) for t in ((op.x, op.add if full is None else None) if pool_bwd else (op.add,)) if t is not None]
        outs = moved_wr + [_abuf(op.y)]
        if any(hit(iv(o), iv(b)) for o in outs for b in ins):
            return False
        if any(hit(iv(a), iv(b)) for x, a in enumerate(outs) for b in outs[x + 1:]):
            return False
        for top in between:
            if top is None:
                continue
            acc = top.accesses()
            if acc is None:
                return False
            r, w = acc
            if any(hit(iv(a), iv(b)) for a in w for b in moved_rd + moved_wr) or any(hit(iv(a), iv(b)) for a in r for b in moved_wr):
                return False
        return True

    def ew_merge(self, op):
        s = R.EwMergeT()
        s.kind = R.EWM_MAXPOOL_BWD if op.ewm_kind == 'maxpool_bwd' else R.EWM_SUMPOOL
        s.has_full = 1 if op.ewm_full is not None else 0
        if op.ewm_full is not None:
            s.full = self.ew(op.ewm_full, plain=True)[1]
        if op.ewm_half is not None:
            s.half = self.ew(op.ewm_half, plain=True)[1]
        s.pool = self.ew(op, plain=True)[1]
        return R.OP_EW_MERGE, s

    def _fill_skip(self, op, s):
        sc, p = op.skip_conv, self.A.ptr
        assert _abuf(sc.y) is _abuf(op.residual) and sc.bn is None, 'skip: the downsample convolution must produce exactly this residual'
        s.x2, s.w2, s.bias2, s.C2 = p(_abuf(sc.x)), p(sc.w), p(sc.bias), sc.dims[3]
        s.residual = None

    def plan_skips(self, ops, readers=None):
        if os.environ.get('FPD_FUSE_SKIP', '1') == '0':
            return
        l = R.lib()
        readers = ops if readers is None else readers
        members_of = lambda top: [m for m in ((top.a, top.b) if top.kind in ('conv2', 'ew2', 'bneck2') else (top,)) if m is not None]
        for op in ops:
            sc = getattr(op, 'skip_conv', None) if op is not None and op.kind == 'conv' else None
            if sc is None or not any(o is sc for o in ops) or (op.lane or 0) != (sc.lane or 0):
                continue
            if getattr(op, 'w8', None) is not None or getattr(sc, 'w8', None) is not None or sc.bn is not None:
                continue
            if _abuf(sc.y) is not _abuf(op.residual) or sc.out_stats is not None:
                continue
            y = _abuf(sc.y)
            if any(o is not op and any(_abuf(t) is y for t in o.acts_in()) for top in readers if top is not None for o in members_of(top)):
                continue
            s = self.conv(op, plain=True)[1]
            self._fill_skip(op, s)
            if l.fpd_conv_skip_supported(C.byref(s)) == 1:
                op.skip_active = True
                sc.skip_fused = True

    def plan_stem_act(self, ops, readers=None):
        if os.environ.get('FPD_STEM_ACT', '1') == '0':
            return
        readers = ops if readers is None else readers
        members_of = lambda top: [m for m in ((top.a, top.b) if top.kind in ('conv2', 'ew2', 'bneck2') else (top,)) if m is not None]
        for op in ops:
            ae = getattr(op, 'act_ew', None) if op is not None and op.kind == 'stem_fwd' else None
            if ae is None or not any(o is ae for o in ops) or (op.lane or 0) != (ae.lane or 0):
                continue
            if ae.op != 'bnrelu_fwd' or ae.bn is None or ae.bn.mode != 'eval' or _abuf(ae.x) is not _abuf(op.y):
                continue
            if op.out_stats is not None or ae.out_stats is not None:
                continue
            y = _abuf(op.y)
            if any(o is not ae and any(_abuf(t) is y for t in o.acts_in()) for top in readers if top is not None for o in members_of(top)):
                continue
            op.act_active = True
            ok = R.lib().fpd_stem_act_supported(C.byref(self.stem(op)[1])) == 1
            op.act_active = ok
            ae.stem_fused = ok

    def _fill_fold(self, op, s):
        if not getattr(op, 'fold_active', False):
            return
        ap, p = op.fold_apply, self.A.ptr
        assert ap.add is None and _abuf(ap.y) is _abuf(op.x), 'fold: the apply must produce exactly this operand'
        s.x = p(_abuf(ap.dy))
        s.fold_x, s.fold_bn, s.fold_stats = p(_abuf(ap.x)), self.bn(ap.bn), p(ap.bstats)
        s.fold_dgamma, s.fold_dbeta = p(ap.dgamma), p(ap.dbeta)
        skip = getattr(op, 'fused_active', False) and not getattr(op, 'fold_other_readers', False)
        s.fold_out = None if skip else p(_abuf(ap.y))

    def _fuse_wgrad(self, op, s, n):
        fw = op.fused_wgrad
        numel = fw.dw.numel
        assert numel == s.C * s.K, (numel, s.C, s.K)
        stride = (numel + s.C + 63) // 64 * 64
        self.partials[id(fw)] = [s, fw.dw, numel, stride, n, self.partial_elems, fw.dbias, s.C]
        self.partial_elems += n * stride
        s.wg_bias = 1 if fw.dbias is not None else 0
        s.wg_count = n
        self.fused.add(id(fw))
        op.fused_active = True

    def wquant(self, entries):
        ents = []
        for w, q, sc in entries:
            e = R.WquantEntryT()
            e.w, e.w8, e.scale = self.A.ptr(w), self.A.ptr(q), self.A.ptr(sc)
            e.K, e.RSC = w.shape[0], w.numel // w.shape[0]
            ents.append(e)
        s = R.TableT()
        s.table, s.n, s.dtype, s.max_elems = self._table(ents, R.WquantEntryT), len(ents), self.dtype, 0
        return R.OP_WQUANT, s

    def bneck(self, op):
        s = R.BneckT()
        (s.N, s.H, s.W, s.C, s.P) = op.dims
        s.dtype = self.dtype
        p = self.A.ptr
        s.x, s.y = p(_abuf(op.x)), p(_abuf(op.y))
        s.w1, s.b1, s.w2, s.b2, s.w3, s.b3 = p(op.w1), p(op.b1), p(op.w2), p(op.b2), p(op.w3), p(op.b3)
        s.bn1, s.bn2, s.bn3 = self.bn(op.bn1), self.bn(op.bn2), self.bn(op.bn3)
        s.folded = p(getattr(op, 'folded', None))
        return R.OP_BNECK, s

    def head(self, op):
        s = R.HeadT()
        (s.N, s.H, s.W, s.C, s.J) = op.dims
        s.dtype = self.dtype
        p = self.A.ptr
        s.y0, s.x, s.score, s.next = p(_abuf(op.y0)), p(_abuf(op.x)), p(_abuf(op.score)), p(_abuf(op.next))
        s.w_fc, s.b_fc, s.w_score, s.b_score = p(op.w_fc), p(op.b_fc), p(op.w_score), p(op.b_score)
        s.w_fc2, s.b_fc2, s.w_score2, s.b_score2 = p(op.w_fc2), p(op.b_fc2), p(op.w_score2), p(op.b_score2)
        s.bn = self.bn(op.bn)
        s.folded = p(getattr(op, 'folded', None))
        return R.OP_HEAD, s

    def wgrad(self, op):
        if id(op) in self.fused:
            return R.OP_NOP, R.MemsetT()
        s = R.WgradT()
        (s.N, s.H, s.W, s.C, s.K, s.R, s.S, s.stride, s.pad, s.P, s.Q) = op.dims
        s.dtype = self.dtype
        p = self.A.ptr
        s.x, s.dy, s.dw, s.dbias = p(_abuf(op.x)), p(_abuf(op.dy)), p(op.dw), p(op.dbias)
        s.bn = self.bn(op.bn)
        s.partial, s.partial_stride = None, 0
        if self.use_partials:
            n = R.lib().fpd_wgrad_num_partials(C.byref(s))
            if n > 0:
                numel = op.dw.numel
                stride = (numel + s.K + 63) // 64 * 64
                self.partials[id(op)] = [s, op.dw, numel, stride, n, self.partial_elems, op.dbias, s.K]
                self.partial_elems += n * stride
        return R.OP_WGRAD, s

    def wreduce(self, op):
        if not any(id(w) in self.partials for w in op.wgrads):
            return R.OP_NOP, R.MemsetT()
        t = R.TableT()
        self.reduces.append((op, t))
        return R.OP_WREDUCE, t

    def finish_partials(self):
        if not self.partials:
            return
        ws = torch.empty(self.partial_elems, dtype=torch.float32, device=self.A.device)
        self.keep.append(ws)
        for s, dw, numel, stride, n, off, dbias, nbias in self.partials.values():
            if isinstance(s, R.ConvT):
                s.wg_partial, s.wg_stride = ws.data_ptr() + 4 * off, stride
            else:
                s.partial, s.partial_stride = ws.data_ptr() + 4 * off, stride
        for op, t in self.reduces:
            ents, mx = [], 0
            for w in op.wgrads:
                rec = self.partials.get(id(w))
                if rec is None:
                    continue
                s, dw, numel, stride, n, off, dbias, nbias = rec
                base = ws.data_ptr() + 4 * off
                e = R.WreduceEntryT()
                e.partial, e.dw, e.n, e.stride, e.count = base, self.A.ptr(dw), numel, stride, n
                ents.append(e)
                if dbias is not None:
                    e = R.WreduceEntryT()
                    e.partial, e.dw, e.n, e.stride, e.count = base + 4 * numel, self.A.ptr(dbias), nbias, stride, n
                    ents.append(e)
                mx = max(mx, numel)
            t.table, t.n, t.dtype, t.max_elems = self._table(ents, R.WreduceEntryT), len(ents), self.dtype, mx

    def stem(self, op):
        s = R.StemT()
        (s.N, s.H, s.W, s.K, s.P, s.Q) = op.dims
        s.dtype = self.dtype
        p = self.A.ptr
        s.x = p(op.image)
        if op.kind == 'stem_fwd':
            s.w, s.bias, s.y, s.out_stats = p(op.w), p(op.bias), p(_abuf(op.y)), p(op.out_stats)
            if getattr(op, 'act_active', False):
                s.act, s.y = self.bn(op.act_ew.bn), p(_abuf(op.act_ew.y))
            return R.OP_STEM_FWD, s
        s.dy, s.dw, s.dbias = p(_abuf(op.dy)), p(op.dw), p(op.dbias)
        s.partial, s.partial_stride = None, 0
        if self.use_partials:
            n = R.lib().fpd_stem_wgrad_num_partials(C.byref(s))
            if n > 0:
                numel = op.dw.numel
                stride = (numel + s.K + 63) // 64 * 64
                self.partials[id(op)] = [s, op.dw, numel, stride, n, self.partial_elems, op.dbias, s.K]
                self.partial_elems += n * stride
        return R.OP_STEM_WGRAD, s

    def ew(self, op, plain=False):
        if not plain and getattr(op, 'ewm_absorbed', False):
            return R.OP_NOP, R.MemsetT()
        if not plain and getattr(op, 'ewm_kind', None) is not None:
            return self.ew_merge(op)
        if getattr(op, 'folded', False):
            return R.OP_NOP, R.MemsetT()
        if getattr(op, 'stem_fused', False):
            return R.OP_NOP, R.MemsetT()
        s = R.EwT()
        s.op, s.dtype = _EW[op.op], self.dtype
        (s.N, s.H, s.W, s.C) = op.dims
        p = self.A.ptr
        s.x, s.x2, s.dy, s.add, s.y = p(_abuf(op.x)), p(_abuf(op.x2)), p(_abuf(op.dy)), p(_abuf(op.add)), p(_abuf(op.y))
        s.out_stats, s.bstats, s.dgamma, s.dbeta = p(op.out_stats), p(op.bstats), p(op.dgamma), p(op.dbeta)
        s.bn = self.bn(op.bn)
        return R.OP_EW, s

    def _table(self, entries, cls):
        arr = (cls * len(entries))(*entries)
        raw = torch.frombuffer(bytearray(bytes(arr)), dtype=torch.uint8).to(self.A.device)
        self.keep.append(raw)
        return raw.data_ptr()

    def bnupd(self, op):
        ents = []
        for bn in op.bns:
            e = R.BnupdEntryT()
            e.stats, e.running_mean, e.running_var = self.A.ptr(bn.stats), self.A.ptr(bn.rmean), self.A.ptr(bn.rvar)
            e.num_batches_tracked = self.A.ptr(bn.nbt)
            e.count, e.momentum, e.C = float(bn.count), G.BN_MOMENTUM, bn.C
            ents.append(e)
        s = R.TableT()
        s.table, s.n, s.dtype, s.max_elems = self._table(ents, R.BnupdEntryT), len(ents), self.dtype, 0
        return R.OP_BNUPD, s

    def wprep(self, entries):
        ents, mx = [], 0
        for w, wf, wb in entries:
            e = R.WprepEntryT()
            e.w, e.w_fwd, e.w_bwd = self.A.ptr(w), self.A.ptr(wf), self.A.ptr(wb)
            (e.K, e.R, e.S, e.C) = w.shape
            mx = max(mx, w.numel)
            ents.append(e)
        s = R.TableT()
        s.table, s.n, s.dtype, s.max_elems = self._table(ents, R.WprepEntryT), len(ents), self.dtype, mx
        return R.OP_WPREP, s

    def memset(self, arena_name, off=0, n=None):
        t = self.A.tensor(arena_name)
        n = t.numel() - off if n is None else n
        s = R.MemsetT()
        s.ptr, s.bytes = t.data_ptr() + off * t.element_size(), n * t.element_size()
        return R.OP_MEMSET, s

    def op(self, op):
        if _WHATIF and _whatif_drop(op, getattr(self, 'train', True)):
            return R.OP_NOP, R.MemsetT()
        if op.kind == 'conv2':
            s = R.ConvPairT()
            s.a, s.b = self.conv(op.a, plain=True)[1], self.conv(op.b, plain=True)[1]
            if (self.use_partials and getattr(op.a, 'fused_wgrad', None) is not None and
                    getattr(op.b, 'fused_wgrad', None) is not None):
                na, nb = C.c_int32(0), C.c_int32(0)
                R.check(R.lib().fpd_conv_pair_fused_wgrad_partials(C.byref(s), C.byref(na), C.byref(nb)), 'fpd_conv_pair_fused_wgrad_partials')
                if na.value > 0 and nb.value > 0:
                    self._fuse_wgrad(op.a, s.a, na.value)
                    self._fuse_wgrad(op.b, s.b, nb.value)
            self._fill_fold(op.a, s.a)
            self._fill_fold(op.b, s.b)
            return R.OP_CONV_PAIR, s
        if op.kind == 'ew2':
            if getattr(op.a, 'ewm_absorbed', False) and getattr(op.b, 'ewm_absorbed', False):
                return R.OP_NOP, R.MemsetT()
            fa, fb = getattr(op.a, 'folded', False), getattr(op.b, 'folded', False)
            if fa or fb:
                return (R.OP_NOP, R.MemsetT()) if (fa and fb) else self.ew(op.b if fa else op.a)
            s = R.EwPairT()
            s.a, s.b = self.ew(op.a)[1], self.ew(op.b)[1]
            return R.OP_EW_PAIR, s
        if op.kind == 'bneck2':
            s = R.BneckPairT()
            s.a, s.b = self.bneck(op.a)[1], self.bneck(op.b)[1]
            return R.OP_BNECK_PAIR, s
        if op.kind == 'head':
            return self.head(op)
        if op.kind == 'head_fold':
            return R.OP_HEAD_FOLD, self.head(op.target)[1]
        if op.kind == 'bneck_fold':
            return R.OP_BNECK_FOLD, self.bneck(op.target)[1]
        if op.kind == 'affsum':
            s = R.AffsumT()
            (s.N, s.H, s.W, s.C) = op.dims
            s.dtype, s.relu, s.nterms = self.dtype, 1 if op.relu else 0, len(op.terms)
            assert len(op.terms) <= R.AFFSUM_MAX and op.out_stats is None
            for j, (t, bn, up) in enumerate(op.terms):
                s.t[j].x, s.t[j].bn, s.t[j].up = self.A.ptr(_abuf(t)), self.bn(bn), up
            s.y = self.A.ptr(_abuf(op.y))
            return R.OP_AFFSUM, s
        if op.kind == 'nchw2nhwc':
            s = R.LayoutT()
            (s.N, s.C, s.H, s.W) = op.dims
            s.src, s.dst, s.dtype = self.A.ptr(op.image), self.A.ptr(_abuf(op.y)), self.dtype
            return R.OP_NCHW2NHWC, s
        if op.kind == 'wreduce':
            return self.wreduce(op)
        if op.kind == 'grad_ready':
            return R.OP_NOP, R.MemsetT()
        return {'conv': self.conv, 'bneck': self.bneck, 'wgrad': self.wgrad, 'stem_fwd': self.stem, 'stem_wgrad': self.stem, 'ew': self.ew,
                'bnupd': self.bnupd}[op.kind](op)


class ModelState:

    def __init__(self, table, device, dtype):
        self.table, self.device, self.dtype = table, device, dtype
        self.A = Arenas(device, dtype)
        for name in ('param', 'rstat', 'nbt'):
            self.A.alloc(name, table.sizes[name])
        self.A.alloc('grad', table.sizes['param'])


class GraphInstance:

    def __init__(self, state, cfg, batch, height, width, train, image=None, share_weights_with=None):
        self.state, self.train = state, train
        self._wlp_owner = share_weights_with
        self.dtype = state.dtype
        env = os.environ.get
        if cfg.get('arch') == 'hrnet':
            self.g = G.HRNetGraph(state.table, cfg['extra'], cfg['J'], batch, height, width, train,
                                  wlp_is_master=(self.dtype == R.F32),
                                  wgrad_batch=int(env('FPD_WGRAD_BATCH')) if env('FPD_WGRAD_BATCH') else None,
                                  fp8=bool(cfg.get('fp8', False)))
        else:
            self.g = G.HourglassGraph(state.table, cfg['F'], cfg['S'], cfg['J'], batch, height, width, train,
                                      num_blocks=cfg.get('num_blocks', 1), wlp_is_master=(self.dtype == R.F32),
                                      fuse_bneck=(self.dtype == R.BF16 and not train and env('FPD_FUSE_BNECK', '1') != '0'),
                                      pair_branches=env('FPD_PAIR', '1') != '0', fuse_head=env('FPD_FUSE_HEAD', '1') != '0',
                                      fuse_skip=(self.dtype == R.BF16 and env('FPD_FUSE_SKIP', '1') != '0'),
                                      fuse_stem_act=(self.dtype == R.BF16 and env('FPD_STEM_ACT', '1') != '0'),
                                      wgrad_batch=int(env('FPD_WGRAD_BATCH')) if env('FPD_WGRAD_BATCH') else None)
        self.A = Arenas(state.device, self.dtype, parent=state.A)
        self.low = Lowering(self.A, self.dtype)
        self.low.train = train
        self.plan = R.Plan()
        self.rng = {}
        self.graphs = {}
        self._image_ext = image
        self._finalized = False
        self.mid_ops = []
        self.mid_native = []

    def _schedule(self, name, ir_ops):
        b, e = self.rng[name]
        assert e - b == len(ir_ops), (name, b, e, len(ir_ops))
        if not self.lanes_enabled or not any(o is not None and o.lane for o in ir_ops):
            return
        sch = PhaseSchedule([((o.lane or 0), o.accesses()) if o is not None else (0, None) for o in ir_ops], self.g.n_lanes)
        for k in range(len(ir_ops)):
            if sch.lanes[k] or sch.waits[k]:
                self.plan.set_schedule(b + k, sch.lanes[k], [b + w for w in sch.waits[k]])
        self.schedules[name] = sch

    def finalize(self):
        g = self.g
        ops = g.fwd + self.mid_ops + g.bwd
        self.lanes_enabled = os.environ.get('FPD_LANES', '1') != '0'
        self.schedules = {}
        delay = int(os.environ.get('FPD_REUSE_DELAY', '400')) if self.lanes_enabled else 0
        if not self.train:
            delay = 0
        act = G.plan_memory(ops, reuse_delay=delay)
        self.act_elems = act
        self.A.alloc('act', act)
        self.A.alloc('stats', g.stats_size)
        if self._wlp_owner is not None:
            o = self._wlp_owner
            assert o.g.wlp_size == g.wlp_size and o.g.fold_size == g.fold_size and not self.train
            self.A.t['wlp'] = o.A.t['wlp']
            self.A.t['fold'] = o.A.t['fold']
        else:
            self.A.alloc('wlp', g.wlp_size)
            self.A.alloc('fold', g.fold_size)
        if self._image_ext is not None:
            self.A.t['image'] = self._image_ext
        else:
            self.A.alloc('image', g.N * 3 * g.H * g.W)
        p = self.plan
        b = len(p)
        p.add(*self.low.memset('stats'))
        entries = []
        for k in self.state.table.conv_keys():
            if k in g.MASTER_ONLY:
                continue
            wf, wb = g.wfwd.get(k), g.wbwd.get(k)
            if wf is not None or wb is not None:
                entries.append((self.state.table[k], wf, wb))
        if entries:
            p.add(*self.low.wprep(entries))
        w8 = getattr(g, 'w8', None)
        if w8:
            self.A.alloc('w8', g.w8_size)
            self.A.alloc('w8s', g.w8s_size)
            p.add(*self.low.wquant([(self.state.table[k], q, sc) for k, (q, sc) in w8.items()]))
        for op in g.fwd:
            for sub in ((op.a, op.b) if op.kind == 'bneck2' else (op,)):
                if sub.kind == 'bneck' and getattr(sub, 'folded', None) is not None:
                    p.add(*self.low.op(G.Op('bneck_fold', target=sub)))
                if sub.kind == 'head' and getattr(sub, 'folded', None) is not None:
                    p.add(*self.low.op(G.Op('head_fold', target=sub)))
        self.rng['prep'] = (b, len(p))
        b = len(p)
        self.op_index = {}
        self.low.plan_skips(g.fwd, readers=ops)
        self.low.plan_stem_act(g.fwd, readers=ops)
        for op in g.fwd:
            self.op_index[id(op)] = p.add(*self.low.op(op))
        self.rng['fwd'] = (b, len(p))
        self._schedule('fwd', list(g.fwd))
        b = len(p)
        for fn in self.mid_native:
            fn(p)
        self.rng['mid'] = (b, len(p))
        if self.train:
            b = len(p)
            p.add(*self.low.memset('grad'))
            self.low.use_partials = True
            bwd_ir = [op for op in g.bwd if op.kind != 'seed']
            self.low.plan_folds(bwd_ir)
            if not isinstance(g, G.HRNetGraph):
                self.low.plan_ew_merge(bwd_ir)
            lowered = [self.low.op(op) for op in bwd_ir]
            self.low.finish_partials()
            self.bucket_ops = {}
            for ir, (code, st) in zip(bwd_ir, lowered):
                k = self.op_index[id(ir)] = p.add(code, st)
                if ir.kind == 'grad_ready':
                    self.bucket_ops[ir.bucket] = k
                    p.mark_event(k)
            self.rng['bwd'] = (b, len(p))
            self._schedule('bwd', [None] + bwd_ir)
        self._finalized = True
        return self

    def run(self, name, stream=None):
        gid = self.graphs.get(name)
        if gid is not None:
            self.plan.replay(gid, stream)
            return
        b, e = self.rng[name]
        self.plan.run(b, e, stream)

    def capture(self, names, cap_stream):
        torch.cuda.synchronize()
        with torch.cuda.stream(cap_stream):
            for n in names:
                b, e = self.rng[n]
                self.graphs[n] = self.plan.capture(b, e, C.c_void_p(cap_stream.cuda_stream))
        torch.cuda.synchronize()

    def image(self):
        return self.A.tensor('image').view(self.g.N, 3, self.g.H, self.g.W)

    def calibrate_running_stats(self):
        assert self.train
        torch.cuda.synchronize()
        for bn in self.g.bns:
            st = self.A.stats_read(bn.stats).sum(0)
            mean = st[0] / bn.count
            var = (st[1] / bn.count - mean * mean).clamp_min(0) * (bn.count / max(bn.count - 1, 1))
            self.A.view(bn.rmean).copy_(mean.float())
            self.A.view(bn.rvar).copy_(var.float())

    def output_view(self, i):
        return self.A.view(self.g.outputs[i].buf)

    def out_grad_view(self, i):
        return self.A.view(self.g.out_grads[i].buf)


class FusedFPDStep:

    def __init__(self, student_state, student_cfg, teacher_state, teacher_cfg, batch, height, width, alpha,
                 lr=2.5e-4, betas=(0.9, 0.999), eps=1e-8, world_size=1, adam=None, teacher_chunks=None,
                 use_target_weight=(True, True), ohkm=None, sgd=None):
        dev = student_state.device
        if adam is not None and sgd is not None:
            raise R.FpdError('FusedFPDStep: adam= and sgd= are mutually exclusive')
        self.use_w = (bool(use_target_weight[0]), bool(use_target_weight[1]))
        self.dtype = student_state.dtype
        self.alpha, self.world_size = alpha, world_size
        self.B, self.J = batch, student_cfg['J']
        self.ohkm = None
        if ohkm is not None:
            self.ohkm = tuple(self.J if k is None else int(k) for k in ohkm)
            if len(self.ohkm) != 2 or not all(1 <= k <= self.J for k in self.ohkm):
                raise R.FpdError('FusedFPDStep: ohkm=%r: topk must lie in [1, J=%d]' % (ohkm, self.J))
        self.teacher = None
        self.teachers = []
        self.tmap = [None, None]
        if teacher_state is not None:
            assert teacher_state.dtype == self.dtype
            if teacher_chunks is None:
                teacher_chunks = 1
            while batch % teacher_chunks:
                teacher_chunks -= 1
            cb = batch // teacher_chunks
            self.teacher = GraphInstance(teacher_state, teacher_cfg, cb, height, width, train=False).finalize()
            self.teachers = [self.teacher] + [
                GraphInstance(teacher_state, teacher_cfg, cb, height, width, train=False,
                              share_weights_with=self.teacher).finalize() for _ in range(1, teacher_chunks)]
            self.teacher.run('prep')
            nt = self.teacher.g.outputs[-1].numel * teacher_chunks
            self.tmap = [torch.zeros(nt, dtype=act_torch_dtype(self.dtype), device=dev) for _ in range(2)]
            self.t_streams = [torch.cuda.Stream(device=dev) for _ in range(teacher_chunks)]
            self.t_stream = self.t_streams[0]
            self.ev_t = [torch.cuda.Event(), torch.cuda.Event()]
            self.ev_chunk = [torch.cuda.Event() for _ in range(teacher_chunks)]
        self._k_t = self._k_s = 0
        self._late_teacher_wait = True
        self.student = GraphInstance(student_state, student_cfg, batch, height, width, train=True)
        g = self.student.g
        self.hh, self.hw = g.outputs[0].shape[1:3]
        A = self.student.A
# ... 239 lines not shown
```

### fast-human-pose-estimation.pytorch_amd/graph.py

```python
import os
from collections import OrderedDict

BN_EPS = 1e-5
BN_MOMENTUM = 0.1
STATS_REPLICAS = int(os.environ.get('FPD_STATS_REPLICAS', '4'))
WGRAD_LANES = 1
LANE_LEVELS = 0
FOLD_APPLY = os.environ.get('FPD_FOLD_APPLY', '1') != '0'
WREDUCE_MODE = os.environ.get('FPD_WREDUCE_MODE', 'lag')
WGRAD_BATCH = 8


class Buf:
    __slots__ = ('arena', 'off', 'shape', 'name')

    def __init__(self, arena, off, shape, name=''):
        self.arena, self.off, self.shape, self.name = arena, off, tuple(shape), name

    @property
    def numel(self):
        n = 1
        for s in self.shape:
            n *= s
        return n

    def __repr__(self):
        return 'Buf(%s+%s %s %s)' % (self.arena, self.off, self.shape, self.name)


class Act:
    __slots__ = ('shape', 'buf', 'stats', 'producer', 'grad', 'name', 'persistent', 'needs_grad', 'apply_op')

    def __init__(self, shape, name=''):
        self.shape = tuple(shape)
        self.buf = None
        self.stats = None
        self.producer = None
        self.grad = None
        self.name = name
        self.persistent = False
        self.needs_grad = True
        self.apply_op = None

    @property
    def numel(self):
        n, h, w, c = self.shape
        return n * h * w * c


class BN:
    __slots__ = ('name', 'mode', 'relu', 'C', 'gamma', 'beta', 'rmean', 'rvar', 'nbt', 'stats', 'count')

    def __init__(self, name, mode, C, gamma, beta, rmean, rvar, nbt, stats=None, relu=True):
        self.name, self.mode, self.C, self.relu = name, mode, C, relu
        self.gamma, self.beta, self.rmean, self.rvar, self.nbt, self.stats = gamma, beta, rmean, rvar, nbt, stats
        self.count = 0


def f8_conv_domain(dims):
    n, h, w, C, K, R, S, stride, pad, P, Q = dims
    if stride != 1 or R != S or R not in (1, 3) or pad != (R - 1) // 2 or w > 128 or w < 2:
        return False
    if C % 32 or K % 8 or C > 512:
        return False
    bk = 64 if C % 64 == 0 else 32
    return (max(1, 128 // w) + R - 1) * w * (bk // 8) <= 2048


class Op:

    def __init__(self, kind, **kw):
        self.kind = kind
        self.lane = None
        self.__dict__.update(kw)

    def accesses(self):
        def b(a):
            return a.buf if isinstance(a, Act) else a

        def bn_bufs(bn):
            if bn is None:
                return []
            return [bn.gamma, bn.beta] + ([bn.stats] if bn.mode == 'train' else [bn.rmean, bn.rvar])
        k = self.kind
        if k in ('conv2', 'bneck2', 'ew2'):
            (ra, wa), (rb, wb) = self.a.accesses(), self.b.accesses()
            return ra + rb, wa + wb
        if k == 'conv':
            rd = [b(self.x), self.w, self.bias, b(self.residual), b(self.epi_x)] + bn_bufs(self.bn) + bn_bufs(self.epi_bn)
            rd += [getattr(self, 'w8', None), getattr(self, 'w8s', None)]
            wr = [b(self.y), self.out_stats, self.epi_stats]
            fw = getattr(self, 'fused_wgrad', None)
            if fw is not None and getattr(self, 'fused_active', False):
                wr += [fw.dw, fw.dbias]
            fa = getattr(self, 'fold_apply', None)
            if fa is not None and getattr(self, 'fold_active', False):
                rd += [b(fa.x), b(fa.dy), fa.bstats] + bn_bufs(fa.bn)
                wr += [b(fa.y), fa.dgamma, fa.dbeta]
            sc = getattr(self, 'skip_conv', None)
            if sc is not None and getattr(self, 'skip_active', False):
                rd += [b(sc.x), sc.w, sc.bias]
        elif k == 'head':
            rd = [b(self.y0), b(self.x), self.w_fc, self.b_fc, self.w_score, self.b_score, self.w_fc2, self.b_fc2,
                  self.w_score2, self.b_score2] + bn_bufs(self.bn)
            wr = [b(self.score), b(self.next)]
        elif k == 'bneck':
            rd = [b(self.x), self.w1, self.b1, self.w2, self.b2, self.w3, self.b3] + bn_bufs(self.bn1) + \
                bn_bufs(self.bn2) + bn_bufs(self.bn3)
            wr = [b(self.y)]
        elif k == 'wgrad':
            rd = [b(self.x), b(self.dy)] + bn_bufs(self.bn)
            wr = [self.dw, self.dbias]
        elif k == 'affsum':
            rd = [b(t) for t, _, _ in self.terms]
            for _, bn, _ in self.terms:
                rd += bn_bufs(bn)
            wr = [b(self.y), self.out_stats]
        elif k == 'nchw2nhwc':
            rd, wr = [self.image], [b(self.y)]
        elif k == 'wreduce':
            rd, wr = list(self.bufs), list(self.bufs)
        elif k == 'grad_ready':
            rd, wr = [self.region], []
        elif k == 'stem_fwd':
            rd, wr = [self.image, self.w, self.bias], [b(self.y), self.out_stats]
            ae = getattr(self, 'act_ew', None)
            if ae is not None and getattr(self, 'act_active', False):
                rd += bn_bufs(ae.bn)
                wr += [b(ae.y)]
        elif k == 'stem_wgrad':
            rd, wr = [self.image, b(self.dy)], [self.dw, self.dbias]
        elif k == 'ew':
            rd = [b(self.x), b(self.x2), b(self.dy), b(self.add)] + bn_bufs(self.bn)
            wr = [b(self.y), self.out_stats, self.bstats, self.dgamma, self.dbeta]
            if getattr(self, 'ewm_kind', None) is not None:
                for m in (self.ewm_full, self.ewm_half):
                    if m is not None:
                        rd += [b(m.x), b(m.dy), b(m.add)] + bn_bufs(m.bn)
                        wr += [b(m.y), m.bstats, m.dgamma, m.dbeta]
        else:
            return None
        return [x for x in rd if x is not None], [x for x in wr if x is not None]

    def acts_in(self):
        if self.kind in ('conv2', 'bneck2', 'ew2'):
            return self.a.acts_in() + self.b.acts_in()
        if self.kind == 'head':
            return [t for t in (self.y0, self.x) if t is not None]
        fa = getattr(self, 'fold_apply', None)
        folded = [t for t in (fa.x, fa.dy) if isinstance(t, Act)] if fa is not None else []
        sc = getattr(self, 'skip_conv', None)
        if sc is not None and isinstance(sc.x, Act):
            folded = folded + [sc.x]
        return [getattr(self, f) for f in ('x', 'x2', 'dy', 'add', 'residual', 'epi_x') if
                isinstance(getattr(self, f, None), Act)] + [a for a in getattr(self, 'extra_in', []) if a is not None] + folded

    def acts_out(self):
        if self.kind in ('conv2', 'bneck2', 'ew2'):
            return self.a.acts_out() + self.b.acts_out()
        if self.kind == 'head':
            return [t for t in (self.score, self.next) if t is not None]
        ae = getattr(self, 'act_ew', None)
        return [getattr(self, f) for f in ('y',) if isinstance(getattr(self, f, None), Act)] + \
               [a for a in getattr(self, 'extra_out', []) if a is not None] + ([ae.y] if ae is not None else [])


class ParamTable:

    def __init__(self, keys, bucket_of=None):
        self.keys = list(keys)
        self.entries = OrderedDict()
        self.logical = dict(self.keys)
        self.sizes = {'param': 0, 'rstat': 0, 'nbt': 0}
        self.bucket = {k: (bucket_of(k) if bucket_of else 0) for k, _ in self.keys}
        placed = {}
        self.buckets = []
        for k, shp in sorted(self.keys, key=lambda ks: self.bucket[ks[0]]):
            if k.endswith('num_batches_tracked'):
                arena = 'nbt'
            elif k.endswith('running_mean') or k.endswith('running_var'):
                arena = 'rstat'
            else:
                arena = 'param'
            n = 1
            for s in shp:
                n *= s
            phys = (shp[0], shp[2], shp[3], shp[1]) if len(shp) == 4 else tuple(shp)
            off = self.sizes[arena]
            placed[k] = Buf(arena, off, phys, k)
            step = 4 if arena != 'nbt' else 2
            self.sizes[arena] = off + (n + step - 1) // step * step
            if arena == 'param':
                b = self.bucket[k]
                while len(self.buckets) <= b:
                    self.buckets.append([off, off])
                self.buckets[b][1] = self.sizes[arena]
        for k, _ in self.keys:
            self.entries[k] = placed[k]
        self.buckets = [tuple(b) for b in self.buckets]

    def __getitem__(self, k):
        return self.entries[k]

    def grad(self, k):
        b = self.entries[k]
        return Buf('grad', b.off, b.shape, 'grad:' + k)

    def conv_keys(self):
        return [k for k, shp in self.keys if len(shp) == 4]

    def trainable_keys(self):
        return [k for k, b in self.entries.items() if b.arena == 'param']

    def grad_bucket(self, b):
        lo, hi = self.buckets[b]
        return Buf('grad', lo, (hi - lo,), 'grad:bucket%d' % b)


def hourglass_bucket_of(num_stacks):
    def f(key):
        p = key.split('.')
        if p[0] in ('hg', 'res', 'fc', 'score', 'fc_', 'score_'):
            return num_stacks - 1 - int(p[1])
        return num_stacks - 1
    return f


def plan_memory(ops, align=64, reuse_delay=0):
    last = {}
    for i, op in enumerate(ops):
        for a in op.acts_in() + op.acts_out():
            last[id(a)] = i
    free = []
    limbo = []
    top = 0

    def alloc(n):
        nonlocal top
        n = (n + align - 1) // align * align
        best = None
        for j, (o, s) in enumerate(free):
            if s >= n and (best is None or s < free[best][1]):
                best = j
        if best is not None:
            o, s = free.pop(best)
            if s > n:
                free.append((o + n, s - n))
            return o, n
        o = top
        top += n
        return o, n

    def release(o, n):
        free.append((o, n))
        free.sort()
        merged = []
        for o2, s2 in free:
            if merged and merged[-1][0] + merged[-1][1] == o2:
                merged[-1] = (merged[-1][0], merged[-1][1] + s2)
            else:
                merged.append((o2, s2))
        free[:] = merged

    sizes = {}
    for i, op in enumerate(ops):
        while limbo and limbo[0][0] + reuse_delay <= i:
            _, o, n = limbo.pop(0)
            release(o, n)
        for a in op.acts_in() + op.acts_out():
            if a.buf is None:
                o, n = alloc(a.numel)
                a.buf = Buf('act', o, a.shape, a.name)
                sizes[id(a)] = n
        seen = set()
        for a in op.acts_in() + op.acts_out():
            if id(a) in seen:
                continue
            seen.add(id(a))
            if last[id(a)] == i and not a.persistent and id(a) in sizes:
                limbo.append((i, a.buf.off, sizes.pop(id(a))))
    return top


class _OpList(list):

    def __init__(self, owner):
        super().__init__()
        self.owner = owner

    def append(self, op):
        if op.lane is None:
            op.lane = self.owner._lane
        super().append(op)


class HourglassGraph:

    def __init__(self, params, num_feats, num_stacks, num_joints, batch, height, width, train, num_blocks=1,
                 depth=4, wlp_is_master=True, lane_levels=None, wgrad_batch=None, fuse_bneck=False, pair_branches=True, fuse_head=True,
                 fuse_skip=False, fuse_stem_act=False):
        self.p = params
        self.F, self.S, self.J = num_feats, num_stacks, num_joints
        self.N, self.H, self.W = batch, height, width
        self.train, self.num_blocks, self.depth = train, num_blocks, depth
        self.wlp_is_master = wlp_is_master
        self.fuse_bneck = fuse_bneck and not train
        self.fuse_head = fuse_head and self.fuse_bneck
        self.pair_branches = pair_branches
        self.fuse_skip, self.fuse_stem_act = fuse_skip, fuse_stem_act and not train
        self._pair_op = None
        self._pair_ew = None
        self.stats_size = 0
        self.fold_size = 0
        self.wlp_size = 0
# ... 635 lines not shown
```

### fast-human-pose-estimation.pytorch_amd/runtime.py

```python
import ctypes as C
import os

_HERE = os.path.dirname(os.path.abspath(__file__))
LIB_PATH = os.environ.get('FPD_AMD_LIB') or os.path.join(_HERE, 'csrc', 'libfpd_amd.so')

F32, BF16 = 0, 1
BN_NONE, BN_TRAIN, BN_EVAL = 0, 1, 2
EPI_PLAIN, EPI_BNRELU_BWD = 0, 1
BACKEND_MFMA, BACKEND_NAIVE, BACKEND_MFMA_GENERIC = 0, 1, 2
(EW_BNRELU_FWD, EW_BNRELU_BWD_R, EW_BN_BWD_APPLY, EW_MAXPOOL_FWD, EW_MAXPOOL_BWD, EW_UPADD_FWD, EW_SUMPOOL,
 EW_ADD, EW_RELU_MASK, EW_DILATE2) = range(10)
(OP_CONV, OP_WGRAD, OP_STEM_FWD, OP_STEM_WGRAD, OP_EW, OP_LOSS, OP_ADAM, OP_MEMSET, OP_WPREP, OP_BNUPD,
 OP_WREDUCE, OP_BNECK, OP_BNECK_FOLD, OP_CONV_PAIR, OP_BNECK_PAIR, OP_EW_PAIR, OP_PCK, OP_HEAD, OP_HEAD_FOLD,
 OP_NOP, OP_AFFSUM, OP_NCHW2NHWC, OP_CONV_F8, OP_WQUANT, OP_LOSS_OHKM, OP_SGD, OP_EW_MERGE) = range(27)
EWM_MAXPOOL_BWD, EWM_SUMPOOL = 0, 1
AFFSUM_MAX = 4
MAX_STACKS = 8
MAXC = 512

_i32, _i64, _f32, _f64, _vp = C.c_int32, C.c_int64, C.c_float, C.c_double, C.c_void_p


class BnT(C.Structure):
    _fields_ = [('mode', _i32), ('relu', _i32), ('eps', _f32), ('_pad', _i32), ('stats', _vp), ('gamma', _vp),
                ('beta', _vp), ('running_mean', _vp), ('running_var', _vp)]


class ConvT(C.Structure):
    _fields_ = [('N', _i32), ('H', _i32), ('W', _i32), ('C', _i32), ('K', _i32), ('R', _i32), ('S', _i32),
                ('stride', _i32), ('pad', _i32), ('P', _i32), ('Q', _i32), ('dtype', _i32), ('epi', _i32),
                ('_pad', _i32), ('x', _vp), ('w', _vp), ('bias', _vp), ('residual', _vp), ('y', _vp),
                ('out_stats', _vp), ('bn', BnT), ('epi_x', _vp), ('epi_bn', BnT), ('epi_stats', _vp),
                ('wg_partial', _vp), ('wg_stride', _i64), ('wg_bias', _i32), ('wg_count', _i32),
                ('fold_x', _vp), ('fold_bn', BnT), ('fold_stats', _vp), ('fold_out', _vp), ('fold_dgamma', _vp), ('fold_dbeta', _vp),
                ('x2', _vp), ('w2', _vp), ('bias2', _vp), ('C2', _i32), ('_pad2', _i32)]


class ConvF8T(C.Structure):
    _fields_ = [('c', ConvT), ('w8', _vp), ('w8_scale', _vp)]


class WquantEntryT(C.Structure):
    _fields_ = [('w', _vp), ('w8', _vp), ('scale', _vp), ('K', _i32), ('RSC', _i32)]


class ConvPairT(C.Structure):
    _fields_ = [('a', ConvT), ('b', ConvT)]


class BneckT(C.Structure):
    _fields_ = [('N', _i32), ('H', _i32), ('W', _i32), ('C', _i32), ('P', _i32), ('dtype', _i32), ('_pad', _i32 * 2),
                ('x', _vp), ('y', _vp), ('w1', _vp), ('b1', _vp), ('w2', _vp), ('b2', _vp), ('w3', _vp), ('b3', _vp),
                ('bn1', BnT), ('bn2', BnT), ('bn3', BnT), ('folded', _vp)]


class BneckPairT(C.Structure):
    _fields_ = [('a', BneckT), ('b', BneckT)]


class WgradT(C.Structure):
    _fields_ = [('N', _i32), ('H', _i32), ('W', _i32), ('C', _i32), ('K', _i32), ('R', _i32), ('S', _i32),
                ('stride', _i32), ('pad', _i32), ('P', _i32), ('Q', _i32), ('dtype', _i32), ('x', _vp), ('dy', _vp),
                ('dw', _vp), ('dbias', _vp), ('bn', BnT), ('partial', _vp), ('partial_stride', _i64)]


class StemT(C.Structure):
    _fields_ = [('N', _i32), ('H', _i32), ('W', _i32), ('K', _i32), ('P', _i32), ('Q', _i32), ('dtype', _i32),
                ('_pad', _i32), ('x', _vp), ('w', _vp), ('bias', _vp), ('y', _vp), ('out_stats', _vp), ('dy', _vp),
                ('dw', _vp), ('dbias', _vp), ('partial', _vp), ('partial_stride', _i64), ('act', BnT)]


class EwT(C.Structure):
    _fields_ = [('op', _i32), ('dtype', _i32), ('N', _i32), ('H', _i32), ('W', _i32), ('C', _i32), ('x', _vp),
                ('x2', _vp), ('dy', _vp), ('add', _vp), ('y', _vp), ('out_stats', _vp), ('bstats', _vp),
                ('dgamma', _vp), ('dbeta', _vp), ('bn', BnT)]


class EwPairT(C.Structure):
    _fields_ = [('a', EwT), ('b', EwT)]


class EwMergeT(C.Structure):
    _fields_ = [('kind', _i32), ('has_full', _i32), ('full', EwT), ('half', EwT), ('pool', EwT)]


class HeadT(C.Structure):
    _fields_ = [('N', _i32), ('H', _i32), ('W', _i32), ('C', _i32), ('J', _i32), ('dtype', _i32), ('_pad', _i32 * 2),
                ('y0', _vp), ('x', _vp), ('score', _vp), ('next', _vp), ('w_fc', _vp), ('b_fc', _vp), ('w_score', _vp),
                ('b_score', _vp), ('w_fc2', _vp), ('b_fc2', _vp), ('w_score2', _vp), ('b_score2', _vp), ('bn', BnT),
                ('folded', _vp)]


class AffTermT(C.Structure):
    _fields_ = [('x', _vp), ('bn', BnT), ('up', _i32), ('_pad', _i32)]


class AffsumT(C.Structure):
    _fields_ = [('N', _i32), ('H', _i32), ('W', _i32), ('C', _i32), ('dtype', _i32), ('relu', _i32), ('nterms', _i32),
                ('_pad', _i32), ('t', AffTermT * 4), ('y', _vp)]


class LayoutT(C.Structure):
    _fields_ = [('src', _vp), ('dst', _vp), ('N', _i32), ('C', _i32), ('H', _i32), ('W', _i32), ('dtype', _i32), ('_pad', _i32)]


class PckT(C.Structure):
    _fields_ = [('B', _i32), ('J', _i32), ('H', _i32), ('W', _i32), ('dtype', _i32), ('log_slots', _i32), ('thr', C.c_float),
                ('_pad', _i32), ('out', _vp), ('target', _vp), ('counts', _vp), ('log', _vp), ('cursor', _vp), ('losses', _vp)]


class FlipMergeT(C.Structure):
    _fields_ = [('N', _i32), ('J', _i32), ('H', _i32), ('W', _i32), ('shift', _i32), ('_pad', _i32), ('a', _vp), ('b', _vp),
                ('y', _vp), ('src', _i32 * 32)]


class FinalPredsT(C.Structure):
    _fields_ = [('N', _i32), ('J', _i32), ('H', _i32), ('W', _i32), ('post_process', _i32), ('_pad', _i32), ('hm', _vp),
                ('trans', _vp), ('coords', _vp), ('preds', _vp), ('maxvals', _vp)]


class TargetsT(C.Structure):
    _fields_ = [('B', _i32), ('J', _i32), ('H', _i32), ('W', _i32), ('patch', _i32), ('_pad', _i32), ('stride_x', _f64),
                ('stride_y', _f64), ('joints', _vp), ('vis', _vp), ('g', _vp), ('target', _vp), ('weight', _vp)]


class WarpSrcT(C.Structure):
    _fields_ = [('img', _vp), ('h', _i32), ('w', _i32), ('row_bytes', _i64), ('minv', _f64 * 6)]


class WarpT(C.Structure):
    _fields_ = [('B', _i32), ('H', _i32), ('W', _i32), ('_pad', _i32), ('src', _vp), ('mean', _f32 * 3), ('std', _f32 * 3),
                ('out', _vp)]


class AugImgT(C.Structure):
    _fields_ = [('img', _vp), ('h', _i32), ('w', _i32), ('row_bytes', _i64)]


class AugDbT(C.Structure):
    _fields_ = [('N', _i32), ('J', _i32), ('box_f32', _i32), ('_pad', _i32), ('images', _vp), ('joints', _vp), ('vis', _vp),
                ('center', _vp), ('scale', _vp), ('flip_src', _vp), ('upper', _vp), ('aspect_ratio', _f64), ('pixel_std', _f64)]


class AugCropT(C.Structure):
    _fields_ = [('src', _i32), ('flip', _i32), ('minv', _f64 * 6)]


class AugmentT(C.Structure):
    _fields_ = [('db', AugDbT), ('B', _i32), ('is_train', _i32), ('flip', _i32), ('num_joints_half_body', _i32),
                ('idx_stride', _i32), ('draw_stride', _i32), ('out_w', _i32), ('out_h', _i32), ('sf', _f64), ('rf', _f64),
                ('prob_half_body', _f64), ('idx', _vp), ('draws', _vp), ('crop', _vp), ('trans', _vp), ('joints', _vp),
                ('vis', _vp), ('center', _vp), ('scale', _vp), ('rotation', _vp), ('flipped', _vp)]


class WarpAugT(C.Structure):
    _fields_ = [('B', _i32), ('H', _i32), ('W', _i32), ('N', _i32), ('images', _vp), ('crop', _vp), ('mean', _f32 * 3),
                ('std', _f32 * 3), ('out', _vp)]


class TargetsWT(C.Structure):
    _fields_ = [('t', TargetsT), ('joints_weight', _vp)]


class OksNmsT(C.Structure):
    _fields_ = [('P_total', _i32), ('n_img', _i32), ('J', _i32), ('soft', _i32), ('rescore', _i32), ('grid', _i32),
                ('in_vis_thre', _f64), ('oks_thre', _f64), ('kpts', _vp), ('area', _vp), ('box_score', _vp), ('offsets', _vp),
                ('sigmas', _vp), ('score', _vp), ('work', _vp), ('keep', _vp), ('n_keep', _vp), ('oks_first', _vp)]


class CocoMatchT(C.Structure):
    _fields_ = [('n_img', _i32), ('J', _i32), ('G_total', _i32), ('D_total', _i32), ('grid', _i32), ('_pad', _i32),
                ('oks_total', _i64), ('area_lo', _f64 * 3), ('area_hi', _f64 * 3), ('oks_thrs', _f64 * 10), ('gt_kpts', _vp),
                ('gt_area', _vp), ('gt_bbox', _vp), ('gt_flags', _vp), ('dt_kpts', _vp), ('gt_offsets', _vp), ('dt_offsets', _vp),
                ('oks_offsets', _vp), ('sigmas', _vp), ('oks', _vp), ('scratch', _vp), ('matched', _vp), ('dt_ignored', _vp),
                ('gt_counted', _vp), ('dt_area', _vp), ('status', _vp)]


class CocoAccumT(C.Structure):
    _fields_ = [('D_total', _i32), ('n_rec', _i32), ('matched', _vp), ('dt_ignored', _vp), ('order', _vp), ('npig', _vp),
                ('rec_thrs', _vp), ('tp', _vp), ('env', _vp), ('precision', _vp), ('recall', _vp), ('status', _vp)]


class LossT(C.Structure):
    _fields_ = [('B', _i32), ('J', _i32), ('H', _i32), ('W', _i32), ('S', _i32), ('dtype', _i32),
                ('target_nchw', _i32), ('alpha', _f32), ('out', _vp * MAX_STACKS), ('dout', _vp * MAX_STACKS),
                ('teacher', _vp), ('target', _vp), ('weight', _vp), ('losses', _vp), ('grad_scale', _f32),
                ('_pad', _i32), ('weight_kd', _vp)]


class LossOhkmT(C.Structure):
    _fields_ = [('base', LossT), ('topk_pose', _i32), ('topk_kd', _i32), ('scratch', _vp), ('scratch_bytes', _i64),
                ('masks', _vp)]


class AdamT(C.Structure):
    _fields_ = [('n', _i64), ('param', _vp), ('grad', _vp), ('m', _vp), ('v', _vp), ('param_lp', _vp),
                ('lr', _f32), ('beta1', _f32), ('beta2', _f32), ('eps', _f32), ('bias_corr1', _f32),
                ('bias_corr2', _f32), ('grad_scale', _f32), ('_pad', _i32), ('lr_dev', _vp), ('step_dev', _vp)]


class SgdT(C.Structure):
    _fields_ = [('n', _i64), ('param', _vp), ('grad', _vp), ('buf', _vp), ('param_lp', _vp), ('lr', _f32),
                ('momentum', _f32), ('weight_decay', _f32), ('grad_scale', _f32), ('nesterov', _i32), ('_pad', _i32),
                ('lr_dev', _vp), ('step_dev', _vp)]


class WprepEntryT(C.Structure):
    _fields_ = [('w', _vp), ('w_fwd', _vp), ('w_bwd', _vp), ('K', _i32), ('R', _i32), ('S', _i32), ('C', _i32)]


class BnupdEntryT(C.Structure):
    _fields_ = [('stats', _vp), ('running_mean', _vp), ('running_var', _vp), ('num_batches_tracked', _vp),
                ('count', _f64), ('momentum', _f32), ('C', _i32)]


class WreduceEntryT(C.Structure):
    _fields_ = [('partial', _vp), ('dw', _vp), ('n', _i64), ('stride', _i64), ('count', _i32), ('_pad', _i32)]


class MemsetT(C.Structure):
    _fields_ = [('ptr', _vp), ('bytes', _i64)]


class TableT(C.Structure):
    _fields_ = [('table', _vp), ('n', _i32), ('dtype', _i32), ('max_elems', _i64)]


_STRUCTS = {'fpd_bn_t': BnT, 'fpd_conv_t': ConvT, 'fpd_wgrad_t': WgradT, 'fpd_stem_t': StemT, 'fpd_ew_t': EwT,
            'fpd_loss_t': LossT, 'fpd_adam_t': AdamT, 'fpd_wprep_entry_t': WprepEntryT,
            'fpd_bnupd_entry_t': BnupdEntryT, 'fpd_memset_t': MemsetT, 'fpd_table_t': TableT,
            'fpd_wreduce_entry_t': WreduceEntryT, 'fpd_bneck_t': BneckT, 'fpd_conv_pair_t': ConvPairT, 'fpd_bneck_pair_t': BneckPairT, 'fpd_ew_pair_t': EwPairT, 'fpd_pck_t': PckT, 'fpd_head_t': HeadT, 'fpd_affsum_t': AffsumT, 'fpd_layout_t': LayoutT,
            'fpd_conv_f8_t': ConvF8T, 'fpd_wquant_entry_t': WquantEntryT, 'fpd_flipmerge_t': FlipMergeT, 'fpd_finalpreds_t': FinalPredsT, 'fpd_targets_t': TargetsT,
            'fpd_warp_src_t': WarpSrcT, 'fpd_warp_t': WarpT, 'fpd_loss_ohkm_t': LossOhkmT, 'fpd_sgd_t': SgdT,
            'fpd_aug_img_t': AugImgT, 'fpd_aug_db_t': AugDbT, 'fpd_aug_crop_t': AugCropT, 'fpd_augment_t': AugmentT,
            'fpd_warp_aug_t': WarpAugT, 'fpd_targets_w_t': TargetsWT, 'fpd_ew_merge_t': EwMergeT, 'fpd_oks_nms_t': OksNmsT,
            'fpd_coco_match_t': CocoMatchT, 'fpd_coco_accum_t': CocoAccumT}

ABI_VERSION = 2

SYMBOLS = {
    'fpd_conv_forward': (C.c_int, [C.POINTER(ConvT), _vp]),
    'fpd_conv_forward_pair': (C.c_int, [C.POINTER(ConvPairT), _vp]),
    'fpd_conv_forward_f8': (C.c_int, [C.POINTER(ConvF8T), _vp]),
    'fpd_conv_f8_in_domain': (C.c_int, [C.POINTER(ConvT)]),
    'fpd_weight_quant_f8': (C.c_int, [_vp, _i32, _vp]),
    'fpd_bottleneck_forward': (C.c_int, [C.POINTER(BneckT), _vp]),
    'fpd_bottleneck_fold': (C.c_int, [C.POINTER(BneckT), _vp]),
    'fpd_bottleneck_forward_pair': (C.c_int, [C.POINTER(BneckPairT), _vp]),
    'fpd_conv_fused_wgrad_partials': (C.c_int, [C.POINTER(ConvT)]),
    'fpd_conv_fold_supported': (C.c_int, [_vp]),
    'fpd_conv_pair_fold_supported': (C.c_int, [_vp]),
    'fpd_conv_skip_supported': (C.c_int, [_vp]),
    'fpd_stem_act_supported': (C.c_int, [_vp]),
    'fpd_conv_pair_fused_wgrad_partials': (C.c_int, [C.POINTER(ConvPairT), C.POINTER(C.c_int32), C.POINTER(C.c_int32)]),
    'fpd_conv_wgrad': (C.c_int, [C.POINTER(WgradT), _vp]),
    'fpd_wgrad_num_partials': (C.c_int, [C.POINTER(WgradT)]),
    'fpd_wgrad_reduce': (C.c_int, [_vp, _i32, _i64, _vp]),
    'fpd_stem_forward': (C.c_int, [C.POINTER(StemT), _vp]),
    'fpd_stem_wgrad': (C.c_int, [C.POINTER(StemT), _vp]),
    'fpd_stem_wgrad_num_partials': (C.c_int, [C.POINTER(StemT)]),
    'fpd_elementwise': (C.c_int, [C.POINTER(EwT), _vp]),
    'fpd_elementwise_pair': (C.c_int, [C.POINTER(EwPairT), _vp]),
    'fpd_ew_merge': (C.c_int, [C.POINTER(EwMergeT), _vp]),
    'fpd_ew_merge_supported': (C.c_int, [_vp]),
    'fpd_pck': (C.c_int, [C.POINTER(PckT), _vp]),
    'fpd_affsum': (C.c_int, [C.POINTER(AffsumT), _vp]),
    'fpd_flip_w': (C.c_int, [_vp, _vp, _i64, _i32, _vp]),
    'fpd_flip_merge': (C.c_int, [C.POINTER(FlipMergeT), _vp]),
    'fpd_final_preds': (C.c_int, [C.POINTER(FinalPredsT), _vp]),
    'fpd_render_targets': (C.c_int, [C.POINTER(TargetsT), _vp]),
    'fpd_warp_affine': (C.c_int, [C.POINTER(WarpT), _vp]),
    'fpd_augment_params': (C.c_int, [C.POINTER(AugmentT), _vp]),
    'fpd_warp_affine_aug': (C.c_int, [C.POINTER(WarpAugT), _vp]),
    'fpd_render_targets_w': (C.c_int, [C.POINTER(TargetsWT), _vp]),
    'fpd_oks_nms': (C.c_int, [C.POINTER(OksNmsT), _vp]),
    'fpd_coco_match': (C.c_int, [C.POINTER(CocoMatchT), _vp]),
    'fpd_coco_accumulate': (C.c_int, [C.POINTER(CocoAccumT), _vp]),
    'fpd_head_forward': (C.c_int, [C.POINTER(HeadT), _vp]),
    'fpd_head_fold': (C.c_int, [C.POINTER(HeadT), _vp]),
    'fpd_loss': (C.c_int, [C.POINTER(LossT), _vp]),
    'fpd_loss_ohkm': (C.c_int, [C.POINTER(LossOhkmT), _vp]),
    'fpd_loss_ohkm_scratch_bytes': (C.c_int64, [C.POINTER(LossT)]),
    'fpd_adam': (C.c_int, [C.POINTER(AdamT), _vp]),
    'fpd_sgd': (C.c_int, [C.POINTER(SgdT), _vp]),
    'fpd_weight_prep': (C.c_int, [_vp, _i32, _i64, _i32, _vp]),
    'fpd_bn_update_running': (C.c_int, [_vp, _i32, _vp]),
    'fpd_cast': (C.c_int, [_vp, _vp, _i64, _i32, _i32, _vp]),
    'fpd_nchw_to_nhwc': (C.c_int, [_vp, _vp, _i32, _i32, _i32, _i32, _i32, _vp]),
    'fpd_nhwc_to_nchw': (C.c_int, [_vp, _vp, _i32, _i32, _i32, _i32, _i32, _vp]),
    'fpd_plan_create': (_vp, []),
    'fpd_plan_destroy': (None, [_vp]),
    'fpd_plan_add': (C.c_int, [_vp, _i32, _vp, _i64]),
    'fpd_plan_size': (C.c_int, [_vp]),
    'fpd_plan_set_schedule': (C.c_int, [_vp, _i32, _i32, C.POINTER(C.c_int32), _i32]),
    'fpd_plan_mark_event': (C.c_int, [_vp, _i32]),
    'fpd_plan_wait_op': (C.c_int, [_vp, _i32, _vp]),
    'fpd_plan_run': (C.c_int, [_vp, _i32, _i32, _vp]),
    'fpd_plan_run_op': (C.c_int, [_vp, _i32, _vp]),
    'fpd_plan_capture': (C.c_int, [_vp, _i32, _i32, _vp]),
    'fpd_plan_replay': (C.c_int, [_vp, _i32, _vp]),
    'fpd_last_error': (C.c_char_p, []),
    'fpd_set_backend': (C.c_int, [_i32]),
    'fpd_set_option': (C.c_int, [C.c_char_p, _i32]),
    'fpd_abi_sizeof': (C.c_int, [C.c_char_p]),
    'fpd_abi_version': (C.c_int, []),
    'fpd_stats_words': (C.c_int64, [C.c_int32]),
    'fpd_event_create': (_vp, []),
    'fpd_event_record': (C.c_int, [_vp, _vp]),
    'fpd_event_elapsed_ms': (C.c_float, [_vp, _vp]),
    'fpd_event_destroy': (None, [_vp]),
}

_lib = None


class FpdError(RuntimeError):
    pass


def lib_sha16():
    import hashlib
    with open(LIB_PATH, 'rb') as f:
        return hashlib.sha256(f.read()).hexdigest()[:16]


def lib():
    global _lib
    if _lib is not None:
        return _lib
    if not os.path.exists(LIB_PATH):
        raise FpdError('HIP extension %s is missing: run `python __graft_entry__.py` (build()) first; '
                       'there is no CPU fallback for the FPD path' % LIB_PATH)
    import torch
    try:
        torch.cuda.is_available()
    except Exception:
        pass
    l = C.CDLL(LIB_PATH)
    for name, (res, args) in SYMBOLS.items():
        fn = getattr(l, name)
        fn.restype = res
        fn.argtypes = args
    if l.fpd_abi_version() != ABI_VERSION:
        raise FpdError('ABI version mismatch: library %d, python host %d' % (l.fpd_abi_version(), ABI_VERSION))
    for name, st in _STRUCTS.items():
        got = l.fpd_abi_sizeof(name.encode())
        if got != C.sizeof(st):
            raise FpdError('ABI mismatch for %s: library %d bytes, python %d bytes' % (name, got, C.sizeof(st)))
    _lib = l
    return l


def check(rc, what=''):
    if rc != 0:
        raise FpdError('%s failed (rc=%d): %s' % (what or 'fpd call', rc, lib().fpd_last_error().decode()))


def set_backend(backend):
    return lib().fpd_set_backend(backend)


def set_option(name, value):
    prev = lib().fpd_set_option(name.encode(), int(value))
    if prev < 0:
        check(prev, 'fpd_set_option(%s)' % name)
    return prev


def current_stream():
    import torch
    return C.c_void_p(torch.cuda.current_stream().cuda_stream)


class Plan:

    def __init__(self):
        self._l = lib()
        self._p = C.c_void_p(self._l.fpd_plan_create())
        self._graphs = {}
        self._types = []

    def add(self, op, args):
        rc = self._l.fpd_plan_add(self._p, op, C.byref(args), C.sizeof(args))
        if rc < 0:
            check(rc, 'fpd_plan_add')
        self._types.append(op)
        return rc

    def op_type(self, k):
        return self._types[k]

    def __len__(self):
        return self._l.fpd_plan_size(self._p)

    def set_schedule(self, op, lane, waits=()):
        arr = (C.c_int32 * max(len(waits), 1))(*waits)
        check(self._l.fpd_plan_set_schedule(self._p, op, lane, arr, len(waits)), 'fpd_plan_set_schedule')

    def mark_event(self, op):
        check(self._l.fpd_plan_mark_event(self._p, op), 'fpd_plan_mark_event')

# ... 29 lines not shown
```

### include/fpd_amd.h

```cpp
#ifndef FPD_AMD_H
#define FPD_AMD_H

#include <stddef.h>
#include <stdint.h>

#ifdef __cplusplus
extern "C" {
#endif

typedef void* fpd_stream_t;

enum { FPD_F32 = 0, FPD_BF16 = 1 };
#ifndef FPD_STATS_REPLICAS
#define FPD_STATS_REPLICAS 4
#endif
typedef int64_t fpd_stat_t;
#define FPD_STATS_WORDS(C) ((int64_t)FPD_STATS_REPLICAS * 4 * (C))
enum { FPD_BN_NONE = 0, FPD_BN_TRAIN = 1, FPD_BN_EVAL = 2 };
enum { FPD_EPI_PLAIN = 0, FPD_EPI_BNRELU_BWD = 1 };
enum { FPD_BACKEND_MFMA = 0, FPD_BACKEND_NAIVE = 1, FPD_BACKEND_MFMA_GENERIC = 2 };

typedef struct {
    int32_t mode;
    int32_t relu;
    float eps;
    int32_t _pad;
    const fpd_stat_t* stats;
    const float* gamma;
    const float* beta;
    const float* running_mean;
    const float* running_var;
} fpd_bn_t;

typedef struct {
    int32_t N, H, W, C;
    int32_t K, R, S;
    int32_t stride, pad;
    int32_t P, Q;
    int32_t dtype;
    int32_t epi;
    int32_t _pad;
    const void* x;
    const void* w;
    const float* bias;
    const void* residual;
    void* y;
    fpd_stat_t* out_stats;
    fpd_bn_t bn;
    const void* epi_x;
    fpd_bn_t epi_bn;
    fpd_stat_t* epi_stats;
    float* wg_partial;
    int64_t wg_stride;
    int32_t wg_bias;
    int32_t wg_count;
    const void* fold_x;
    fpd_bn_t fold_bn;
    const fpd_stat_t* fold_stats;
    void* fold_out;
    float* fold_dgamma;
    float* fold_dbeta;
    const void* x2;
    const void* w2;
    const float* bias2;
    int32_t C2;
    int32_t _pad2;
} fpd_conv_t;

typedef struct {
    int32_t N, H, W, C, P, dtype;
    int32_t _pad[2];
    const void* x;
    void* y;
    const void* w1;
    const float* b1;
    const void* w2;
    const float* b2;
    const void* w3;
    const float* b3;
    fpd_bn_t bn1, bn2, bn3;
    const float* folded;
} fpd_bneck_t;

typedef struct {
    int32_t N, H, W, C, J, dtype;
    int32_t _pad[2];
    const void* y0;
    const void* x;
    void* score;
    void* next;
    const void* w_fc;
    const float* b_fc;
    const void* w_score;
    const float* b_score;
    const void* w_fc2;
    const float* b_fc2;
    const void* w_score2;
    const float* b_score2;
    fpd_bn_t bn;
    const float* folded;
} fpd_head_t;
int fpd_head_forward(const fpd_head_t* a, fpd_stream_t stream);
int fpd_head_fold(const fpd_head_t* a, fpd_stream_t stream);

typedef struct { fpd_conv_t a, b; } fpd_conv_pair_t;

typedef struct { fpd_bneck_t a, b; } fpd_bneck_pair_t;

typedef struct {
    int32_t N, H, W, C, K, R, S, stride, pad, P, Q, dtype;
    const void* x;
    const void* dy;
    float* dw;
    float* dbias;
    fpd_bn_t bn;
    float* partial;
    int64_t partial_stride;
} fpd_wgrad_t;

typedef struct {
    int32_t N, H, W, K, P, Q, dtype, _pad;
    const float* x;
    const float* w;
    const float* bias;
    void* y;
    fpd_stat_t* out_stats;
    const void* dy;
    float* dw;
    float* dbias;
    float* partial;
    int64_t partial_stride;
    fpd_bn_t act;
} fpd_stem_t;

enum {
    FPD_EW_BNRELU_FWD = 0, FPD_EW_BNRELU_BWD_R = 1, FPD_EW_BN_BWD_APPLY = 2, FPD_EW_MAXPOOL_FWD = 3,
    FPD_EW_MAXPOOL_BWD = 4, FPD_EW_UPADD_FWD = 5, FPD_EW_SUMPOOL = 6, FPD_EW_ADD = 7, FPD_EW_RELU_MASK = 8,
    FPD_EW_DILATE2 = 9
};
typedef struct {
    int32_t op, dtype;
    int32_t N, H, W, C;
    const void* x;
    const void* x2;
    const void* dy;
    const void* add;
    void* y;
    fpd_stat_t* out_stats;
    fpd_stat_t* bstats;
    float* dgamma;
    float* dbeta;
    fpd_bn_t bn;
} fpd_ew_t;

enum { FPD_EWM_MAXPOOL_BWD = 0, FPD_EWM_SUMPOOL = 1 };
typedef struct {
    int32_t kind;
    int32_t has_full;
    fpd_ew_t full;
    fpd_ew_t half;
    fpd_ew_t pool;
} fpd_ew_merge_t;
int fpd_ew_merge(const fpd_ew_merge_t* a, fpd_stream_t stream);
int fpd_ew_merge_supported(const fpd_ew_merge_t* a);

#define FPD_AFFSUM_MAX 4
typedef struct { const void* x; fpd_bn_t bn; int32_t up; int32_t _pad; } fpd_affterm_t;
typedef struct {
    int32_t N, H, W, C;
    int32_t dtype, relu, nterms, _pad;
    fpd_affterm_t t[FPD_AFFSUM_MAX];
    void* y;
} fpd_affsum_t;
int fpd_affsum(const fpd_affsum_t* a, fpd_stream_t stream);

typedef struct { const float* src; void* dst; int32_t N, C, H, W, dtype, _pad; } fpd_layout_t;

#define FPD_MAX_STACKS 8
typedef struct {
    int32_t B, J, H, W, S, dtype;
    int32_t target_nchw;
    float alpha;
    const void* out[FPD_MAX_STACKS];
    void* dout[FPD_MAX_STACKS];
    const void* teacher;
    const float* target;
    const float* weight;
    double* losses;
    float grad_scale;
    int32_t _pad;
    const float* weight_kd;
} fpd_loss_t;

typedef struct {
    fpd_loss_t base;
    int32_t topk_pose, topk_kd;
    void* scratch;
    int64_t scratch_bytes;
    uint32_t* masks;
} fpd_loss_ohkm_t;

typedef struct {
    int64_t n;
    float* param; const float* grad; float* m; float* v;
    void* param_lp;
    float lr, beta1, beta2, eps;
    float bias_corr1, bias_corr2;
    float grad_scale;
    int32_t _pad;
    const float* lr_dev;
    int64_t* step_dev;
} fpd_adam_t;

typedef struct {
    int64_t n;
    float* param; const float* grad; float* buf;
    void* param_lp;
    float lr, momentum, weight_decay;
    float grad_scale;
    int32_t nesterov;
    int32_t _pad;
    const float* lr_dev;
    int64_t* step_dev;
} fpd_sgd_t;

typedef struct {
    const float* w;
    void* w_fwd;
    void* w_bwd;
    int32_t K, R, S, C;
} fpd_wprep_entry_t;

typedef struct {
    const fpd_stat_t* stats;
    float* running_mean; float* running_var; int64_t* num_batches_tracked;
    double count; float momentum; int32_t C;
} fpd_bnupd_entry_t;

typedef struct {
    const float* partial; float* dw; int64_t n; int64_t stride; int32_t count; int32_t _pad;
} fpd_wreduce_entry_t;

int fpd_conv_forward(const fpd_conv_t* a, fpd_stream_t stream);
int fpd_conv_forward_pair(const fpd_conv_pair_t* p, fpd_stream_t stream);
int fpd_bottleneck_forward(const fpd_bneck_t* a, fpd_stream_t stream);
int fpd_bottleneck_fold(const fpd_bneck_t* a, fpd_stream_t stream);
int fpd_bottleneck_forward_pair(const fpd_bneck_pair_t* p, fpd_stream_t stream);
int fpd_conv_fused_wgrad_partials(const fpd_conv_t* a);
int fpd_conv_fold_supported(const fpd_conv_t* a);
int fpd_conv_pair_fold_supported(const fpd_conv_pair_t* p);
int fpd_conv_skip_supported(const fpd_conv_t* a);
int fpd_conv_pair_fused_wgrad_partials(const fpd_conv_pair_t* p, int32_t* n_a, int32_t* n_b);
int fpd_conv_wgrad(const fpd_wgrad_t* a, fpd_stream_t stream);
int fpd_wgrad_num_partials(const fpd_wgrad_t* a);
int fpd_wgrad_reduce(const fpd_wreduce_entry_t* table_dev, int32_t n_entries, int64_t max_elems, fpd_stream_t stream);
int fpd_stem_forward(const fpd_stem_t* a, fpd_stream_t stream);
int fpd_stem_act_supported(const fpd_stem_t* a);
int fpd_stem_wgrad(const fpd_stem_t* a, fpd_stream_t stream);
int fpd_stem_wgrad_num_partials(const fpd_stem_t* a);
int fpd_elementwise(const fpd_ew_t* a, fpd_stream_t stream);
typedef struct { fpd_ew_t a, b; } fpd_ew_pair_t;
int fpd_elementwise_pair(const fpd_ew_pair_t* p, fpd_stream_t stream);
int fpd_loss(const fpd_loss_t* a, fpd_stream_t stream);
int fpd_loss_ohkm(const fpd_loss_ohkm_t* a, fpd_stream_t stream);
int64_t fpd_loss_ohkm_scratch_bytes(const fpd_loss_t* a);
int fpd_adam(const fpd_adam_t* a, fpd_stream_t stream);
int fpd_sgd(const fpd_sgd_t* a, fpd_stream_t stream);
int fpd_weight_prep(const fpd_wprep_entry_t* table_dev, int32_t n_entries, int64_t max_elems, int32_t dtype,
                    fpd_stream_t stream);
int fpd_bn_update_running(const fpd_bnupd_entry_t* table_dev, int32_t n_entries, fpd_stream_t stream);
int fpd_cast(const void* src, void* dst, int64_t n, int32_t src_dtype, int32_t dst_dtype, fpd_stream_t stream);
int fpd_nchw_to_nhwc(const float* src, void* dst, int32_t N, int32_t C, int32_t H, int32_t W, int32_t dtype,
                     fpd_stream_t stream);
int fpd_nhwc_to_nchw(const void* src, float* dst, int32_t N, int32_t C, int32_t H, int32_t W, int32_t dtype,
                     fpd_stream_t stream);

typedef struct {
    int32_t B, J, H, W, dtype, log_slots;
    float thr;
    int32_t _pad;
    const void* out;
    const float* target;
    float* counts;
    double* log;
    long long* cursor;
    const double* losses;
} fpd_pck_t;
int fpd_pck(const fpd_pck_t* a, fpd_stream_t stream);

typedef struct {
    fpd_conv_t c;
    const void* w8;
    const float* w8_scale;
} fpd_conv_f8_t;
int fpd_conv_forward_f8(const fpd_conv_f8_t* a, fpd_stream_t stream);
int fpd_conv_f8_in_domain(const fpd_conv_t* c);

typedef struct {
    const float* w;
    void* w8;
    float* scale;
    int32_t K, RSC;
} fpd_wquant_entry_t;
int fpd_weight_quant_f8(const fpd_wquant_entry_t* table_dev, int32_t n_entries, fpd_stream_t stream);

int fpd_flip_w(const float* x, float* y, int64_t rows, int32_t W, fpd_stream_t stream);

#define FPD_MAX_JOINTS 32
typedef struct {
    int32_t N, J, H, W;
    int32_t shift, _pad;
    const float* a;
    const float* b;
    float* y;
    int32_t src[FPD_MAX_JOINTS];
} fpd_flipmerge_t;
int fpd_flip_merge(const fpd_flipmerge_t* a, fpd_stream_t stream);

typedef struct {
    int32_t N, J, H, W;
    int32_t post_process, _pad;
    const float* hm;
    const double* trans;
    float* coords;
    float* preds;
    float* maxvals;
} fpd_finalpreds_t;
int fpd_final_preds(const fpd_finalpreds_t* a, fpd_stream_t stream);

typedef struct {
    int32_t B, J, H, W;
    int32_t patch, _pad;
    double stride_x, stride_y;
    const double* joints;
    const float* vis;
    const float* g;
    float* target;
    float* weight;
} fpd_targets_t;
int fpd_render_targets(const fpd_targets_t* a, fpd_stream_t stream);

typedef struct {
    const uint8_t* img;
    int32_t h, w;
    int64_t row_bytes;
    double minv[6];
} fpd_warp_src_t;
typedef struct {
    int32_t B, H, W, _pad;
    const fpd_warp_src_t* src;
    float mean[3], std[3];
    float* out;
} fpd_warp_t;
int fpd_warp_affine(const fpd_warp_t* a, fpd_stream_t stream);

typedef struct {
    const uint8_t* img;
    int32_t h, w;
    int64_t row_bytes;
} fpd_aug_img_t;
typedef struct {
    int32_t N, J;
    int32_t box_f32, _pad;
    const fpd_aug_img_t* images;
    const double* joints;
    const float* vis;
    const double* center;
    const double* scale;
    const int32_t* flip_src;
    const int32_t* upper;
    double aspect_ratio;
    double pixel_std;
} fpd_aug_db_t;
typedef struct {
    int32_t src;
    int32_t flip;
    double minv[6];
} fpd_aug_crop_t;
typedef struct {
    fpd_aug_db_t db;
    int32_t B, is_train;
    int32_t flip, num_joints_half_body;
    int32_t idx_stride, draw_stride;
    int32_t out_w, out_h;
    double sf, rf, prob_half_body;
    const int32_t* idx;
    const double* draws;
    fpd_aug_crop_t* crop;
    double* trans;
    double* joints;
    float* vis;
    double* center;
    double* scale;
    double* rotation;
    int32_t* flipped;
} fpd_augment_t;
int fpd_augment_params(const fpd_augment_t* a, fpd_stream_t stream);

typedef struct {
    int32_t B, H, W, N;
// ... 119 lines not shown
```

Baseline: 3632 images/s.

## Fuse hourglass upsample-add into the following eval bottleneck kernel

Adds an optional low-branch source (x2) to the fused eval bottleneck kernel. The kernel reads the nearest-upsampled x2 alongside x and sums them in registers, both for the conv1 input and for the residual. The planner absorbs a preceding upadd_fwd elementwise op into the bottleneck when it is the sole reader, which removes one kernel launch and one full activation write and read. In exchange it adds extra loads and register pressure inside an already tuned pipelined kernel, and it applies only to non-train BF16 plans such as the teacher forward.

```diff
diff --git a/fast-human-pose-estimation.pytorch_amd/csrc/api.hip b/fast-human-pose-estimation.pytorch_amd/csrc/api.hip
--- a/fast-human-pose-estimation.pytorch_amd/csrc/api.hip
+++ b/fast-human-pose-estimation.pytorch_amd/csrc/api.hip
@@ -80,6 +80,7 @@
     if (!strcmp(name, "conv_c3_blocks")) return fpd_conv_c3_option(1, value);
     if (!strcmp(name, "conv_c3_launches")) return fpd_conv_c3_option(2, value);
     if (!strcmp(name, "bneck_blocks")) return fpd_bneck_blocks_option(value);
+    if (!strcmp(name, "bneck_upadd")) return fpd_bneck_upadd_option(value);
     if (!strcmp(name, "head_blocks")) return fpd_head_blocks_option(value);
     if (!strcmp(name, "wgrad_tile_only")) { g_wgrad_tile_only = value; return 0; }
     return fpd_fail(-2, "set_option: unknown option '%s'", name);
@@ -256,6 +257,7 @@
     const fpd_bneck_t* ab[2] = {&p->a, &p->b};
     for (const fpd_bneck_t* a : ab) {
         FPD_REQUIRE(a->x && a->y && a->w1 && a->w2 && a->w3 && a->x != a->y, "bottleneck_pair: null pointer or y aliases x");
+        FPD_REQUIRE(a->x2 == nullptr, "bottleneck_pair: a pair launch takes no low-branch source (x2)");
         FPD_REQUIRE((int64_t)a->N * a->H * a->W * a->C < ((int64_t)1 << 31), "bottleneck_pair: tensor too large for 32-bit indexing");
         int rc = validate_bneck_bns(a);
         if (rc) return rc;
@@ -275,12 +277,20 @@
     FPD_REQUIRE((int64_t)a->N * a->H * a->W * a->C < ((int64_t)1 << 31), "bottleneck: tensor too large for 32-bit indexing");
     int rc = validate_bneck_bns(a);
     if (rc) return rc;
+    if (a->x2 != nullptr) {
+        const char* why = fpd_bneck_upadd_why_not(*a);
+        if (why) return fpd_fail(-3, "bottleneck: low-branch source (x2) with N=%d H=%d W=%d C=%d P=%d: %s; fpd_bneck_upadd_supported() reports 0 for it",
+                                 a->N, a->H, a->W, a->C, a->P, why);
+        FPD_REQUIRE(a->x2 != a->y, "bottleneck: y must not alias x2");
+    }
     rc = fpd_bneck_fused_launch(*a, (hipStream_t)stream);
     if (rc == 1)
         return fpd_fail(-3, "bottleneck: shape N=%d H=%d W=%d C=%d P=%d dtype=%d is outside the fused kernel's domain",
                         a->N, a->H, a->W, a->C, a->P, a->dtype);
     return rc ? rc : check_launch();
 }
+
+int fpd_bneck_upadd_supported(const fpd_bneck_t* a) { return (a && fpd_bneck_upadd_why_not(*a) == nullptr) ? 1 : 0; }
 
 struct WgradBackend {
     unsigned backends;
@@ -743,7 +753,7 @@
             break;
         }
         case FPD_OP_WGRAD: snprintf(t, sizeof(t), "wgrad N=%d H=%d W=%d C=%d K=%d R=%d s=%d", o.u.wgrad.N, o.u.wgrad.H, o.u.wgrad.W, o.u.wgrad.C, o.u.wgrad.K, o.u.wgrad.R, o.u.wgrad.stride); break;
-        case FPD_OP_BNECK: snprintf(t, sizeof(t), "bneck N=%d H=%d W=%d C=%d P=%d", o.u.bneck.N, o.u.bneck.H, o.u.bneck.W, o.u.bneck.C, o.u.bneck.P); break;
+        case FPD_OP_BNECK: snprintf(t, sizeof(t), "bneck N=%d H=%d W=%d C=%d P=%d%s", o.u.bneck.N, o.u.bneck.H, o.u.bneck.W, o.u.bneck.C, o.u.bneck.P, o.u.bneck.x2 ? "+upadd" : ""); break;
         case FPD_OP_BNECK_PAIR: snprintf(t, sizeof(t), "bneck2 N=%d H=%d W=%d C=%d P=%d | H=%d W=%d", o.u.bpair.a.N, o.u.bpair.a.H, o.u.bpair.a.W, o.u.bpair.a.C, o.u.bpair.a.P, o.u.bpair.b.H, o.u.bpair.b.W); break;
         case FPD_OP_HEAD: snprintf(t, sizeof(t), "head N=%d H=%d W=%d C=%d J=%d", o.u.head.N, o.u.head.H, o.u.head.W, o.u.head.C, o.u.head.J); break;
         case FPD_OP_EW: snprintf(t, sizeof(t), "ew %s N=%d H=%d W=%d C=%d", ewn(o.u.ew.op), o.u.ew.N, o.u.ew.H, o.u.ew.W, o.u.ew.C); break;
diff --git a/fast-human-pose-estimation.pytorch_amd/csrc/bneck_fused.hip b/fast-human-pose-estimation.pytorch_amd/csrc/bneck_fused.hip
--- a/fast-human-pose-estimation.pytorch_amd/csrc/bneck_fused.hip
+++ b/fast-human-pose-estimation.pytorch_amd/csrc/bneck_fused.hip
@@ -3,7 +3,7 @@
 #include <cstdlib>
 #include <type_traits>
 
-#include "common.h"
+#include "conv_dispatch.h"
 
 namespace {
 
@@ -39,7 +39,7 @@
 template <int P>
 __global__ void bneck_fold_kernel(const fpd_bneck_t a, float* out) { bneck_fold_tables<P>(a, out, threadIdx.x, blockDim.x); }
 
-template <int P, bool DMA>
+template <int P, bool DMA, bool UPADD>
 __device__ __forceinline__ void bneck_eval_body(const fpd_bneck_t& a, const int logW, const int swz, const int bid_in,
                                                 const int nblk, const int ntiles) {
     constexpr int C = 2 * P;
@@ -88,6 +88,7 @@
     bf16_t* sA2 = reinterpret_cast<bf16_t*>(s_b3 + C);
     bf16_t* sR2 = sA2 + (zero_px + 3) * LD2;
     const bf16_t* __restrict__ x = reinterpret_cast<const bf16_t*>(a.x);
+    const bf16_t* __restrict__ x2 = reinterpret_cast<const bf16_t*>(UPADD ? a.x2 : nullptr);
     const bf16_t* __restrict__ w1 = reinterpret_cast<const bf16_t*>(a.w1);
     const bf16_t* __restrict__ w2 = reinterpret_cast<const bf16_t*>(a.w2);
     const bf16_t* __restrict__ w3 = reinterpret_cast<const bf16_t*>(a.w3);
@@ -96,6 +97,7 @@
     int npass = whole ? 1 : ((hrows * W + 127) >> 7);
     const int xpx = tid >> 3, xcv = (tid & 7) * 8;
     int xo[2];
+    int xo2[UPADD ? 2 : 1];
     bool xok[2];
     auto pass_addr = [&](int p) __attribute__((always_inline)) {
 #pragma unroll
@@ -105,6 +107,7 @@
             const int g = g0 - 1 + hr;
             xok[i] = hr < hrows && (unsigned)g < (unsigned)GR;
             xo[i] = xok[i] ? (g * W + j) * C + xcv : 0;
+            if constexpr (UPADD) xo2[i] = xok[i] ? ((((g >> 1) << logW) >> 1) + (j >> 1)) * C + xcv : 0;
         }
     };
     int w1o[W1V], w1l[W1V];
@@ -117,6 +120,7 @@
     const int xl = xpx * LDX + xcv;
 
     u32x4 rx[NCH][2], rw[NCH][W1V];
+    u32x4 rx2[UPADD ? NCH : 1][2];
     auto a_load = [&](auto kcc) __attribute__((always_inline)) {
         constexpr int kc = decltype(kcc)::value;
         static_for<2>([&](auto ic) {
@@ -124,11 +128,29 @@
             const u32x4 z = {0u, 0u, 0u, 0u};
             rx[kc][i] = z;
             if (xok[i]) rx[kc][i] = *reinterpret_cast<const u32x4*>(x + (xo[i] + kc * 64));
+            if constexpr (UPADD) {
+                rx2[kc][i] = z;
+                if (xok[i]) rx2[kc][i] = *reinterpret_cast<const u32x4*>(x2 + (xo2[i] + kc * 64));
+            }
         });
         static_for<W1V>([&](auto ic) {
             constexpr int i = decltype(ic)::value;
             rw[kc][i] = *reinterpret_cast<const u32x4*>(w1 + (w1o[i] + kc * 64));
         });
+    };
+    auto a_sum = [&](auto kcc, auto ic) __attribute__((always_inline)) {
+        constexpr int kc = decltype(kcc)::value, i = decltype(ic)::value;
+        if constexpr (UPADD) {
+            float v[8], u[8];
+            const u32x4 r = rx[kc][i], r2 = rx2[kc][i];
+            DT<bf16_t>::unpack(make_uint4(r[0], r[1], r[2], r[3]), v);
+            DT<bf16_t>::unpack(make_uint4(r2[0], r2[1], r2[2], r2[3]), u);
+#pragma unroll
+            for (int e = 0; e < 8; ++e) v[e] = v[e] + u[e];
+            const uint4 o = DT<bf16_t>::pack(v);
+            const u32x4 ov = {o.x, o.y, o.z, o.w};
+            rx[kc][i] = ov;
+        }
     };
     constexpr int NSL = 2 + W1V;
     auto a_store_slice = [&](auto kcc, auto slc) __attribute__((always_inline)) {
@@ -246,6 +268,8 @@
             *reinterpret_cast<uint4*>(sA2 + px * LD2 + cv) = z;
         }
     }
+    a_sum(std::integral_constant<int, 0>{}, std::integral_constant<int, 0>{});
+    a_sum(std::integral_constant<int, 0>{}, std::integral_constant<int, 1>{});
     STAMP(1);
 
     auto refill = [&](auto kcc, int pp) __attribute__((always_inline)) {
@@ -269,15 +293,15 @@
             for (int i = 0; i < 16; ++i) acc[tn][i] = 0.f;
         static_for<NCH>([&](auto kcc) {
             constexpr int kc = decltype(kcc)::value;
-            auto stage_slice = [&](auto slc) __attribute__((always_inline)) {
-                constexpr int sl = decltype(slc)::value;
+            auto stage_slice = [&](auto slc, auto lastc) __attribute__((always_inline)) {
+                constexpr bool last = decltype(lastc)::value;
                 if constexpr (kc + 1 < NCH) {
                     a_store_slice(std::integral_constant<int, (kc + 1) % NCH>{}, slc);
-                    if constexpr (sl == NSL - 1) refill(std::integral_constant<int, (kc + 1) % NCH>{}, p);
+                    if constexpr (last) refill(std::integral_constant<int, (kc + 1) % NCH>{}, p);
                 } else {
                     if (p + 1 < npass) {
                         a_store_slice(std::integral_constant<int, 0>{}, slc);
-                        if constexpr (sl == NSL - 1) {
+                        if constexpr (last) {
                             if (p + 2 < npass) pass_addr(p + 2);
                             refill(std::integral_constant<int, 0>{}, p + 1);
                         }
@@ -294,7 +318,19 @@
                     const bf16x8 wf = *reinterpret_cast<const bf16x8*>(wrow + tn * 32 * LDX + kk * 16);
                     acc[tn] = __builtin_amdgcn_mfma_f32_32x32x16_bf16(wf, px, acc[tn], 0, 0, 0);
                 }
-                stage_slice(kkc);
+                if constexpr (!UPADD) {
+                    stage_slice(kkc, std::integral_constant<bool, kk == NSL - 1>{});
+                } else {
+                    if constexpr (kk < 2) {
+                        if constexpr (kc + 1 < NCH) {
+                            if (p == 0) a_sum(std::integral_constant<int, (kc + 1) % NCH>{}, kkc);
+                        }
+                        stage_slice(std::integral_constant<int, (kk + 2 < NSL ? kk + 2 : NSL)>{}, std::false_type{});
+                    } else {
+                        stage_slice(std::integral_constant<int, kk - 2>{}, std::integral_constant<bool, kk == 3>{});
+                        if (p + 1 < npass) a_sum(kcc, std::integral_constant<int, kk - 2>{});
+                    }
+                }
             });
             __syncthreads();
             ASTAMP();
@@ -367,6 +403,7 @@
     constexpr int VW = CW / 8;
     constexpr int NIT = 32 * VW / 64;
     u32x4 rres[2][NIT];
+    u32x4 rres2[UPADD ? NIT : 1];
     auto res_load = [&](auto stc) __attribute__((always_inline)) {
         constexpr int st = decltype(stc)::value;
         static_for<NIT>([&](auto itc) {
@@ -377,6 +414,40 @@
             const u32x4 z = {0u, 0u, 0u, 0u};
             rres[st][it] = z;
             if (m < M) rres[st][it] = *reinterpret_cast<const u32x4*>(x + ((size_t)m * C + st * P + hC * CW + cv));
+            if constexpr (UPADD) {
+                const int g = m >> logW, j = m & (W - 1);
+                const int m2 = (((g >> 1) << logW) >> 1) + (j >> 1);
+                rres2[it] = z;
+                if (m < M) rres2[it] = *reinterpret_cast<const u32x4*>(x2 + ((size_t)m2 * C + st * P + hC * CW + cv));
+            }
+        });
+    };
+    auto res_sum = [&](auto stc, auto itc) __attribute__((always_inline)) {
+        constexpr int st = decltype(stc)::value, it = decltype(itc)::value;
+        if constexpr (UPADD && it < NIT) {
+            float v[8], u[8];
+            const u32x4 r = rres[st][it], r2 = rres2[it];
+            DT<bf16_t>::unpack(make_uint4(r[0], r[1], r[2], r[3]), v);
+            DT<bf16_t>::unpack(make_uint4(r2[0], r2[1], r2[2], r2[3]), u);
+#pragma unroll
+            for (int e = 0; e < 8; ++e) v[e] = v[e] + u[e];
+            const uint4 o = DT<bf16_t>::pack(v);
+            const u32x4 ov = {o.x, o.y, o.z, o.w};
+            rres[st][it] = ov;
+        }
+    };
+    auto mma_sum = [&](const bf16_t* arow, int buf, f32x16* acc, auto stc) __attribute__((always_inline)) {
+        const bf16_t* wbase = sR2 + buf * P * LDW + (hC * CW + (lane & 31)) * LDW;
+        static_for<P / 16>([&](auto kkc) {
+            constexpr int kk = decltype(kkc)::value;
+            const bf16x8 px = *reinterpret_cast<const bf16x8*>(arow + kk * 16);
+            const int wo = DMA ? (((2 * kk + (lane >> 5)) ^ wsw) * 8) : (kk * 16 + koff);
+#pragma unroll
+            for (int tn = 0; tn < TNH; ++tn) {
+                const bf16x8 wf = *reinterpret_cast<const bf16x8*>(wbase + tn * 32 * LDW + wo);
+                acc[tn] = __builtin_amdgcn_mfma_f32_32x32x16_bf16(wf, px, acc[tn], 0, 0, 0);
+            }
+            res_sum(stc, kkc);
         });
     };
 
@@ -390,7 +461,8 @@
             for (int tn = 0; tn < TNH; ++tn)
 #pragma unroll
                 for (int i = 0; i < 16; ++i) accC[s - 9][tn][i] = 0.f;
-            mma(sA2 + (a3px + ml) * LD2 + koff, s & 1, accC[s - 9]);
+            if constexpr (UPADD) mma_sum(sA2 + (a3px + ml) * LD2 + koff, s & 1, accC[s - 9], std::integral_constant<int, s - 9>{});
+            else mma(sA2 + (a3px + ml) * LD2 + koff, s & 1, accC[s - 9]);
         }
         if constexpr (s + 1 < NSTEP) {
             t_store(std::integral_constant<int, s + 1>{});
@@ -472,17 +544,17 @@
 #endif
 }
 
-template <int P, bool DMA>
+template <int P, bool DMA, bool UPADD>
 __global__ __launch_bounds__(512, 1) void bneck_eval_kernel(const fpd_bneck_t a, const int logW, const int ntiles) {
-    bneck_eval_body<P, DMA>(a, logW, (ntiles & 7) == 0, blockIdx.x, gridDim.x, ntiles);
+    bneck_eval_body<P, DMA, UPADD>(a, logW, (ntiles & 7) == 0, blockIdx.x, gridDim.x, ntiles);
 }
 
 template <int P, bool DMA>
 __global__ __launch_bounds__(512, 1) void bneck_eval_pair_kernel(const fpd_bneck_t a, const fpd_bneck_t b, const int logWa,
                                                                  const int logWb, const int nblk_a, const int ntiles_a,
                                                                  const int ntiles_b) {
-    if ((int)blockIdx.x < nblk_a) bneck_eval_body<P, DMA>(a, logWa, (ntiles_a & 7) == 0, blockIdx.x, nblk_a, ntiles_a);
-    else bneck_eval_body<P, DMA>(b, logWb, (ntiles_b & 7) == 0, (int)blockIdx.x - nblk_a, (int)gridDim.x - nblk_a, ntiles_b);
+    if ((int)blockIdx.x < nblk_a) bneck_eval_body<P, DMA, false>(a, logWa, (ntiles_a & 7) == 0, blockIdx.x, nblk_a, ntiles_a);
+    else bneck_eval_body<P, DMA, false>(b, logWb, (ntiles_b & 7) == 0, (int)blockIdx.x - nblk_a, (int)gridDim.x - nblk_a, ntiles_b);
 }
 
 
@@ -536,13 +608,13 @@
     return 0;
 }
 
-template <int P, bool DMA>
+template <int P, bool DMA, bool UPADD>
 int launch_bneck(const fpd_bneck_t& a, int logW, hipStream_t st) {
     const size_t lds = bneck_lds_bytes<P>(a.H, a.W);
     static LdsAttr configured;
-    if (int rc_ = configured.ensure(reinterpret_cast<const void*>(&bneck_eval_kernel<P, DMA>), lds)) return rc_;
+    if (int rc_ = configured.ensure(reinterpret_cast<const void*>(&bneck_eval_kernel<P, DMA, UPADD>), lds)) return rc_;
     const int ntiles = cdiv(a.N * a.H * a.W, 128);
-    FPD_LAUNCH((bneck_eval_kernel<P, DMA>), dim3(bneck_blocks(ntiles, bneck_block_cap())), dim3(512), lds, st, a, logW, ntiles);
+    FPD_LAUNCH((bneck_eval_kernel<P, DMA, UPADD>), dim3(bneck_blocks(ntiles, bneck_block_cap())), dim3(512), lds, st, a, logW, ntiles);
     return 0;
 }
 
@@ -560,15 +632,30 @@
     return hw % 128 == 0 || 128 % hw == 0;
 }
 
+static EnvOpt g_bneck_upadd{"FPD_BNECK_UPADD", 1};
+int fpd_bneck_upadd_option(int value) { return g_bneck_upadd.set(value < 0 ? 0 : value); }
+
+const char* fpd_bneck_upadd_why_not(const fpd_bneck_t& a) {
+    if (g_bneck_upadd.get() == 0) return "switched off (FPD_BNECK_UPADD=0 / option bneck_upadd)";
+    if (!bneck_in_domain(a)) return "the shape is outside the fused kernel's domain";
+    if (a.W < 8) return "W must be one of 8, 16, 32, 64";
+    if (a.H & 1) return "H must be even";
+    return nullptr;
+}
+
 int fpd_bneck_fused_launch(const fpd_bneck_t& a, hipStream_t st) {
     if (!bneck_in_domain(a)) return 1;
     int logW = 0;
     while ((1 << logW) < a.W) ++logW;
-    return a.P == 128 ? launch_bneck<128, true>(a, logW, st) : launch_bneck<64, true>(a, logW, st);
+    if (a.x2 != nullptr) {
+        if (fpd_bneck_upadd_why_not(a) != nullptr) return 1;
+        return a.P == 128 ? launch_bneck<128, true, true>(a, logW, st) : launch_bneck<64, true, true>(a, logW, st);
+    }
+    return a.P == 128 ? launch_bneck<128, true, false>(a, logW, st) : launch_bneck<64, true, false>(a, logW, st);
 }
 
 int fpd_bneck_fused_pair_launch(const fpd_bneck_t& a, const fpd_bneck_t& b, hipStream_t st) {
-    if (!bneck_in_domain(a) || !bneck_in_domain(b) || a.P != b.P) return 1;
+    if (!bneck_in_domain(a) || !bneck_in_domain(b) || a.P != b.P || a.x2 != nullptr || b.x2 != nullptr) return 1;
     return a.P == 128 ? launch_bneck_pair<128, true>(a, b, st) : launch_bneck_pair<64, true>(a, b, st);
 }
 
diff --git a/fast-human-pose-estimation.pytorch_amd/csrc/conv_dispatch.h b/fast-human-pose-estimation.pytorch_amd/csrc/conv_dispatch.h
--- a/fast-human-pose-estimation.pytorch_amd/csrc/conv_dispatch.h
+++ b/fast-human-pose-estimation.pytorch_amd/csrc/conv_dispatch.h
@@ -79,6 +79,8 @@
 int fpd_bneck_fused_launch(const fpd_bneck_t& a, hipStream_t st);
 int fpd_bneck_fused_pair_launch(const fpd_bneck_t& a, const fpd_bneck_t& b, hipStream_t st);
 int fpd_bneck_fold_launch(const fpd_bneck_t& a, float* out, hipStream_t st);
+const char* fpd_bneck_upadd_why_not(const fpd_bneck_t& a);
+int fpd_bneck_upadd_option(int value);
 int fpd_head_fused_launch(const fpd_head_t& a, hipStream_t st);
 int fpd_head_fold_launch(const fpd_head_t& a, float* out, hipStream_t st);
 int fpd_pck_launch(const fpd_pck_t& a, hipStream_t st);
diff --git a/fast-human-pose-estimation.pytorch_amd/executor.py b/fast-human-pose-estimation.pytorch_amd/executor.py
--- a/fast-human-pose-estimation.pytorch_amd/executor.py
+++ b/fast-human-pose-estimation.pytorch_amd/executor.py
@@ -330,6 +330,33 @@
             op.act_active = ok
             ae.stem_fused = ok
 
+    @staticmethod
+    def plan_upadd(ops, readers=None, dtype=R.BF16):
+        if os.environ.get('FPD_BNECK_UPADD', '1') == '0':
+            return 0
+        readers = ops if readers is None else readers
+        members_of = lambda top: [m for m in ((top.a, top.b) if top.kind in ('conv2', 'ew2', 'bneck2') else (top,)) if m is not None]
+        n = 0
+        for op in ops:
+            if op is None or op.kind != 'bneck' or getattr(op, 'x2', None) is not None:
+                continue
+            ua = getattr(op.x, 'producer', None)
+            if ua is None or ua.kind != 'ew' or ua.op != 'upadd_fwd' or ua.out_stats is not None or op.x.stats is not None:
+                continue
+            if ua.y is not op.x or op.x.persistent or not any(o is ua for o in ops) or (op.lane or 0) != (ua.lane or 0):
+                continue
+            rd = [o for top in readers if top is not None for o in members_of(top) if any(t is op.x for t in o.acts_in())]
+            if len(rd) != 1 or rd[0] is not op:
+                continue
+            s = R.BneckT()
+            (s.N, s.H, s.W, s.C, s.P), s.dtype = op.dims, dtype
+            if R.lib().fpd_bneck_upadd_supported(C.byref(s)) != 1:
+                continue
+            op.upadd_op, op.x, op.x2 = ua, ua.x, ua.x2
+            ua.upadd_absorbed = True
+            n += 1
+        return n
+
     def _fill_fold(self, op, s):
         if not getattr(op, 'fold_active', False):
             return
@@ -373,6 +400,12 @@
         s.w1, s.b1, s.w2, s.b2, s.w3, s.b3 = p(op.w1), p(op.b1), p(op.w2), p(op.b2), p(op.w3), p(op.b3)
         s.bn1, s.bn2, s.bn3 = self.bn(op.bn1), self.bn(op.bn2), self.bn(op.bn3)
         s.folded = p(getattr(op, 'folded', None))
+        x2 = getattr(op, 'x2', None)
+        if x2 is not None:
+            yb = _abuf(op.y)
+            for t in (_abuf(op.x), _abuf(x2)):
+                assert t.arena != yb.arena or t.off + t.numel <= yb.off or yb.off + yb.numel <= t.off, 'bneck: y overlaps a source of its up-add'
+            s.x2 = p(_abuf(x2))
         return R.OP_BNECK, s
 
     def head(self, op):
@@ -465,6 +498,8 @@
 
     def ew(self, op, plain=False):
         if not plain and getattr(op, 'ewm_absorbed', False):
+            return R.OP_NOP, R.MemsetT()
+        if getattr(op, 'upadd_absorbed', False):
             return R.OP_NOP, R.MemsetT()
         if not plain and getattr(op, 'ewm_kind', None) is not None:
             return self.ew_merge(op)
@@ -635,6 +670,8 @@
         delay = int(os.environ.get('FPD_REUSE_DELAY', '400')) if self.lanes_enabled else 0
         if not self.train:
             delay = 0
+        if not self.train and self.dtype == R.BF16:
+            self.low.plan_upadd(g.fwd, readers=ops, dtype=self.dtype)
         act = G.plan_memory(ops, reuse_delay=delay)
         self.act_elems = act
         self.A.alloc('act', act)
diff --git a/fast-human-pose-estimation.pytorch_amd/graph.py b/fast-human-pose-estimation.pytorch_amd/graph.py
--- a/fast-human-pose-estimation.pytorch_amd/graph.py
+++ b/fast-human-pose-estimation.pytorch_amd/graph.py
@@ -105,7 +105,7 @@
                   self.w_score2, self.b_score2] + bn_bufs(self.bn)
             wr = [b(self.score), b(self.next)]
         elif k == 'bneck':
-            rd = [b(self.x), self.w1, self.b1, self.w2, self.b2, self.w3, self.b3] + bn_bufs(self.bn1) + \
+            rd = [b(self.x), b(getattr(self, 'x2', None)), self.w1, self.b1, self.w2, self.b2, self.w3, self.b3] + bn_bufs(self.bn1) + \
                 bn_bufs(self.bn2) + bn_bufs(self.bn3)
             wr = [b(self.y)]
         elif k == 'wgrad':
@@ -131,6 +131,8 @@
         elif k == 'stem_wgrad':
             rd, wr = [self.image, b(self.dy)], [self.dw, self.dbias]
         elif k == 'ew':
+            if getattr(self, 'upadd_absorbed', False):
+                return [], []
             rd = [b(self.x), b(self.x2), b(self.dy), b(self.add)] + bn_bufs(self.bn)
             wr = [b(self.y), self.out_stats, self.bstats, self.dgamma, self.dbeta]
             if getattr(self, 'ewm_kind', None) is not None:
@@ -147,6 +149,8 @@
             return self.a.acts_in() + self.b.acts_in()
         if self.kind == 'head':
             return [t for t in (self.y0, self.x) if t is not None]
+        if getattr(self, 'upadd_absorbed', False):
+            return []
         fa = getattr(self, 'fold_apply', None)
         folded = [t for t in (fa.x, fa.dy) if isinstance(t, Act)] if fa is not None else []
         sc = getattr(self, 'skip_conv', None)
@@ -160,6 +164,8 @@
             return self.a.acts_out() + self.b.acts_out()
         if self.kind == 'head':
             return [t for t in (self.score, self.next) if t is not None]
+        if getattr(self, 'upadd_absorbed', False):
+            return []
         ae = getattr(self, 'act_ew', None)
         return [getattr(self, f) for f in ('y',) if isinstance(getattr(self, f, None), Act)] + \
                [a for a in getattr(self, 'extra_out', []) if a is not None] + ([ae.y] if ae is not None else [])
diff --git a/fast-human-pose-estimation.pytorch_amd/runtime.py b/fast-human-pose-estimation.pytorch_amd/runtime.py
--- a/fast-human-pose-estimation.pytorch_amd/runtime.py
+++ b/fast-human-pose-estimation.pytorch_amd/runtime.py
@@ -51,7 +51,7 @@
 class BneckT(C.Structure):
     _fields_ = [('N', _i32), ('H', _i32), ('W', _i32), ('C', _i32), ('P', _i32), ('dtype', _i32), ('_pad', _i32 * 2),
                 ('x', _vp), ('y', _vp), ('w1', _vp), ('b1', _vp), ('w2', _vp), ('b2', _vp), ('w3', _vp), ('b3', _vp),
-                ('bn1', BnT), ('bn2', BnT), ('bn3', BnT), ('folded', _vp)]
+                ('bn1', BnT), ('bn2', BnT), ('bn3', BnT), ('folded', _vp), ('x2', _vp)]
 
 
 class BneckPairT(C.Structure):
@@ -247,6 +247,7 @@
     'fpd_bottleneck_forward': (C.c_int, [C.POINTER(BneckT), _vp]),
     'fpd_bottleneck_fold': (C.c_int, [C.POINTER(BneckT), _vp]),
     'fpd_bottleneck_forward_pair': (C.c_int, [C.POINTER(BneckPairT), _vp]),
+    'fpd_bneck_upadd_supported': (C.c_int, [C.POINTER(BneckT)]),
     'fpd_conv_fused_wgrad_partials': (C.c_int, [C.POINTER(ConvT)]),
     'fpd_conv_fold_supported': (C.c_int, [_vp]),
     'fpd_conv_pair_fold_supported': (C.c_int, [_vp]),
diff --git a/include/fpd_amd.h b/include/fpd_amd.h
--- a/include/fpd_amd.h
+++ b/include/fpd_amd.h
@@ -80,6 +80,7 @@
     const float* b3;
     fpd_bn_t bn1, bn2, bn3;
     const float* folded;
+    const void* x2;
 } fpd_bneck_t;
 
 typedef struct {
@@ -246,6 +247,7 @@
 int fpd_bottleneck_forward(const fpd_bneck_t* a, fpd_stream_t stream);
 int fpd_bottleneck_fold(const fpd_bneck_t* a, fpd_stream_t stream);
 int fpd_bottleneck_forward_pair(const fpd_bneck_pair_t* p, fpd_stream_t stream);
+int fpd_bneck_upadd_supported(const fpd_bneck_t* a);
 int fpd_conv_fused_wgrad_partials(const fpd_conv_t* a);
 int fpd_conv_fold_supported(const fpd_conv_t* a);
 int fpd_conv_pair_fold_supported(const fpd_conv_pair_t* p);
```

After: 3698 images/s (median of 6 runs). 1.8% higher.
